# NVIDIA/flowtron

Measured on AMD Instinct MI355X. Metric: mel-frames/sec training (2-flow, 80-mel), higher is better.
Workload: dtype bf16; 1 GPU; BASELINE configs[1]: 2-flow LJS config.json model, per-GPU batch 32, T_max=862, L_max=157, attn-prior + CTC on, fwd+loss+bwd+clip+RAdam; global_batch=32, parallelism=dp1, mfma_operands=bf16, storage=fp32, skipped_steps=0

## Files before the change

flowtron_amd/_lib.py:

```python
from __future__ import annotations

import ctypes as C
import os

import torch

_HERE = os.path.dirname(os.path.abspath(__file__))
LIB_PATH = os.path.join(_HERE, "libflowtron_hip.so")

FT_F32, FT_BF16, FT_F16 = 0, 1, 2
GEMM_SPLITK = 1
GEMM_SPLITK_DET = 2
GEMM_C16 = 4
ACT_NONE, ACT_TANH, ACT_RELU, ACT_SIGMOID = 0, 1, 2, 3

_p, _i, _l, _f, _sz, _d = C.c_void_p, C.c_int, C.c_int64, C.c_float, C.c_size_t, C.c_double


class GemmArgs(C.Structure):
    _fields_ = [("A", _p), ("B", _p), ("C", _p), ("bias", _p),
                ("M", _i), ("N", _i), ("K", _i), ("batch", _i),
                ("sAm", _l), ("sAk", _l), ("sBk", _l), ("sBn", _l), ("ldc", _l),
                ("bsA", _l), ("bsB", _l), ("bsC", _l),
                ("alpha", _f), ("beta", _f), ("act", _i), ("mode", _i), ("flags", _i),
                ("work", _p), ("work_bytes", _sz)]


class GemmImgArgs(C.Structure):
    _fields_ = [("A", _p), ("B", _p), ("C", _p), ("bias", _p), ("M", _i), ("N", _i), ("K", _i),
                ("lda", _l), ("ldb", _l), ("ldc", _l), ("a_kmajor", _i), ("b_kmajor", _i),
                ("alpha", _f), ("beta", _f), ("act", _i), ("flags", _i),
                ("rowmap", _p), ("rows_dev", _p), ("compact", _i), ("k_shift", _i), ("r1_row", _p), ("r1_col", _p),
                ("split_work", _p), ("split_work_bytes", _sz), ("a_rows", _p)]


class LstmFwdRole(C.Structure):
    _fields_ = [("gx", _p), ("lens", _p), ("y", _p), ("ldy", _l), ("gates", _p), ("cell", _p), ("wimg", _p), ("state_h", _p), ("state_c", _p),
                ("B", C.c_int32), ("ldb", C.c_int32), ("t0", C.c_int32), ("t1", C.c_int32), ("gx16", C.c_int32)]


class LstmBwdRole(C.Structure):
    _fields_ = [("dy", _p), ("ldy", _l), ("lens", _p), ("gates", _p), ("cell", _p), ("dgx", _p), ("wimg", _p),
                ("dimg", _p), ("dimg_ld", _l), ("dimg_rows", _l), ("dbias", _p), ("state_da", _p), ("state_dc", _p),
                ("B", C.c_int32), ("ldb", C.c_int32), ("t0", C.c_int32), ("t1", C.c_int32), ("carry_in", C.c_int32)]


class ImgDesc(C.Structure):
    _fields_ = [("src", _p), ("ld", _l), ("rows", _l), ("cols", _l), ("dst", _p), ("kind", _i)]


class CummAttnArgs(C.Structure):
    _fields_ = [(n, _p) for n in ("text", "Q", "V", "w_key", "v", "w1", "b1", "w2", "b2", "in_lens", "ctx", "attn", "logprob",
                                  "cumm_all", "kproj_all", "work")] + [("work_bytes", _sz)] + [
        (n, _i) for n in ("T", "B", "L", "E", "A", "NF", "K1", "K2")] + [("temperature", _f), ("mode", _i), ("persist_status", _p)]


class DecodeArgs(C.Structure):
    _fields_ = [(n, _p) for n in (
        "att_w_ih", "att_w_hh", "att_b_ih", "att_b_hh", "w_query", "v", "K", "V",
        "l0_w_ih", "l0_w_hh", "l0_b_ih", "l0_b_hh", "l1_w_ih", "l1_w_hh", "l1_b_ih", "l1_b_hh",
        "d0_w", "d0_b", "d1_w", "d1_b", "conv_w", "conv_b", "gate_w", "gate_b",
        "residual", "mel_out", "attn_out", "n_done_dev", "work")] + [
        ("work_bytes", _sz), ("N", _i), ("L", _i), ("H", _i), ("A", _i), ("M", _i),
        ("temperature", _f), ("gate_threshold", _f), ("use_graph", _i)] + [
        (n, _p) for n in ("cond_w1", "cond_b1", "cond_w2", "cond_b2", "w_key", "enc")] + [("E", _i), ("prior", _p), ("forced", _p),
                                                                                         ("wimg", _p), ("wimg_bytes", _sz), ("persist_gran", _p), ("persist_status", _p),
                                                                                         ("n_layers", _i), ("extra_layers", _p)]


class DecodeBatchArgs(C.Structure):
    _fields_ = [("a", DecodeArgs), ("nb", _i), ("n_lim", _p), ("wimg_ready", _i)]


SUMSQ_PARTIALS = 1024
RESAMPLE_MAX_PHASES, RESAMPLE_MAX_TAPS = 2048, 20480

SIGNATURES = {
    "ft_abi_version": ([], _i),
    "ft_last_error": ([], C.c_char_p),
    "ft_debug_hold_cus": ([_i, _l, _p], _i),
    "ft_gemm": ([C.POINTER(GemmArgs), _p], _i),
    "ft_gemm_workspace_bytes": ([C.POINTER(GemmArgs)], _sz),
    "ft_bf16_image_bytes": ([_l, _l], _sz),
    "ft_bf16_image": ([_p, _l, _l, _l, _p, _p], _i),
    "ft_bf16_image_colsum": ([_p, _l, _l, _l, _p, _p, _p], _i),
    "ft_bf16_image_colsum_acc": ([_p, _l, _l, _l, _p, _p, _p], _i),
    "ft_gemm_img": ([C.POINTER(GemmImgArgs), _p], _i),
    "ft_gemm_img_split_work_bytes": ([_i, _i, _i], _sz),
    "ft_bf16_image_split3": ([_p, _l, _l, _l, _p, _i, _p], _i),
    "ft_bf16_image_split3_im2col": ([_p, _p, _i, _i, _i, _i, _p, _p], _i),
    "ft_bf16_image_split3_im2col_f16": ([_p, _p, _i, _i, _i, _i, _p, _p], _i),
    "ft_bf16_image_table": ([C.POINTER(ImgDesc), _i, _p], _i),
    "ft_bf16_image_table_f16": ([C.POINTER(ImgDesc), _i, _p], _i),
    "ft_bf16_image_split3_f16": ([_p, _l, _l, _l, _p, _i, _p], _i),
    "ft_rowmap_build": ([_p, _p, _p, _i, _i, _p], _i),
    "ft_chunk_gather_rows": ([_p, _p, _p, _i, _i, _i, _i, _p], _i),
    "ft_bf16_image_rows": ([_p, _l, _l, _l, _p, _p, _p, _p, _p], _i),
    "ft_bf16_image_rows_acc": ([_p, _l, _l, _l, _p, _p, _p, _p, _p], _i),
    "ft_bf16_image_rows_into": ([_p, _l, _l, _l, _p, _l, _l, _l, _p, _p, _p], _i),
    "ft_img_gemv_rows": ([_p, _l, _i, _p, _p, _p, _l, _p, _p, _p, _i, _i, _p], _i),
    "ft_img_gemv_rows_bwd": ([_p, _l, _i, _p, _l, _p, _p, _p, _p, _l, _p], _i),
    "ft_bf16_image_rows_act_bwd": ([_p, _l, _p, _l, _i, _l, _l, _p, _p, _p, _p, _p], _i),
    "ft_bf16_image_rows_act_bwd_acc": ([_p, _l, _p, _l, _i, _l, _l, _p, _p, _p, _p, _p], _i),
    "ft_pad_rows_fill": ([_p, _l, _i, _p, _i, _i, _i, _p], _i),
    "ft_embedding_fwd": ([_p, _p, _p, _i, _i, _l, _p], _i),
    "ft_embedding_bwd": ([_p, _p, _p, _i, _i, _l, _p], _i),
    "ft_embedding_bwd_runs": ([_p, _p, _p, _i, _i, _l, _i, _p], _i),
    "ft_im2col": ([_p, _p, _p, _i, _i, _i, _i, _p], _i),
    "ft_col2im": ([_p, _p, _p, _i, _i, _i, _i, _p], _i),
    "ft_instnorm_relu_fwd": ([_p] * 8 + [_i, _i, _i, _f, _p], _i),
    "ft_instnorm_relu_bwd": ([_p] * 11 + [_i, _i, _i, _p], _i),
    "ft_lstm_workspace_bytes": ([_i, _i], _sz),
    "ft_lstm_seq_fwd": ([_p, _p, _p, _p, _l, _p, _p, _p, _i, _i, _i, _i, _i, _p], _i),
    "ft_lstm_seq_bwd": ([_p, _l, _p, _p, _p, _p, _p, _p, _i, _i, _i, _i, _i, _p], _i),
    "ft_lstm_persist_supported": ([_i, _i], _i),
    "ft_lstm_persist_workspace_bytes": ([_i, _i], _sz),
    "ft_lstm_persist_debug_prof": ([_p], _i),
    "ft_lstm_persist_bwd": ([_p, _l, _p, _p, _p, _p, _p, _p, _p, _i, _i, _i, _i, _p], _i),
    "ft_bilstm_persist_supported": ([_i, _i], _i),
    "ft_bilstm_persist_workspace_bytes": ([_i, _i], C.c_size_t),
    "ft_bilstm_persist_fwd": ([_p, _p, _p, _p, _p, _p, _l, _p, _p, _p, _p, _p, _p, _i, _i, _i, _p], _i),
    "ft_bilstm_persist_bwd": ([_p, _l, _p, _p, _p, _p, _p, _p, _p, _p, _p, _p, _p, _i, _i, _i, _p], _i),
    "ft_lstm_persist_bwd_img": ([_p, _l, _p, _p, _p, _p, _p, _p, _p, _i, _i, _i, _i, _p, _l, _l, _p, _p], _i),
    "ft_lstm_roles_ctx_bytes": ([], _sz),
    "ft_lstm_roles_wimg_bytes": ([_i], _sz),
    "ft_lstm_roles_ctx_init": ([_p, _p], _i),
    "ft_lstm_roles_debug_prof": ([_p], _i),
    "ft_lstm_roles_prepare_fwd": ([_p, _p, _i, _p], _i),
    "ft_lstm_roles_prepare_bwd": ([_p, _p, _i, _p], _i),
    "ft_lstm_roles_fwd": ([C.POINTER(LstmFwdRole), _i, _i, _i, _p, _i, _p, _i, _p], _i),
    "ft_lstm_roles_bwd": ([C.POINTER(LstmBwdRole), _i, _i, _i, _p, _i, _p, _i, _p], _i),
    "ft_lstm2_supported": ([_i, _i], _i),
    "ft_lstm2_workspace_bytes": ([_i, _i], _sz),
    "ft_lstm2_seq_fwd": ([_p] * 13 + [_i, _i, _i, _p], _i),
    "ft_lstm2_seq_bwd": ([_p] * 12 + [_i, _i, _i, _p], _i),
    "ft_lstm_bidir_supported": ([_i, _i], _i),
    "ft_lstm_bidir_seq_fwd": ([_p] * 6 + [_l] + [_p] * 6 + [_i, _i, _i, _p], _i),
# ... 24 lines not shown
    "ft_decode_debug_prof": ([_p], _i),
    "ft_decode_flow": ([C.POINTER(DecodeArgs), _p], _i),
    "ft_decode_batch_max": ([], _i),
    "ft_decode_batch_gran_bytes": ([_i], _sz),
    "ft_decode_flow_batch": ([C.POINTER(DecodeBatchArgs), _p], _i),
    "ft_decode_flow_batch_keys": ([C.POINTER(DecodeBatchArgs), _p, _p], _i),
    "ft_stft_mel": ([_p, _p, _p, _p, _i, _i, _i, _i, _i, _p], _i),
    "ft_stft_r8": ([_p, _p, _p, _p, _p, _p, _p, _p, _i, _i, _i, _i, _p], _i),
    "ft_stft_r8_ragged": ([_p, _p, _p, _p, _p, _p, _p, _i, _i, _i, _i, _i, _p], _i),
    "ft_istft_r8": ([_p, _p, _p, _p, _i, _i, _i, _p], _i),
    "ft_stft_pow2": ([_p, _p, _p, _p, _p, _p, _p, _p, _i, _i, _i, _i, _i, _i, _p], _i),
    "ft_stft_pow2_ragged": ([_p, _p, _p, _p, _p, _p, _p, _i, _i, _i, _i, _i, _i, _i, _p], _i),
    "ft_istft_pow2": ([_p, _p, _p, _p, _i, _i, _i, _i, _i, _p], _i),
    "ft_stft_r8_ragged_phase": ([_p, _p, _p, _p, _p, _i, _i, _i, _p], _i),
    "ft_istft_r8_ragged": ([_p, _p, _p, _p, _p, _i, _i, _i, _p], _i),
    "ft_stft_pow2_ragged_phase": ([_p, _p, _p, _p, _p, _i, _i, _i, _i, _i, _p], _i),
    "ft_istft_pow2_ragged": ([_p, _p, _p, _p, _p, _i, _i, _i, _i, _i, _p], _i),
    "ft_resample_ragged": ([_p, _p, _p, _p, _p, _i, _i, _i, _i, _i, _i, _p], _i),
    "ft_resample_out_len": ([_l, _i, _i], _l),
    "ft_attn_ctc_workspace_floats":([_i, _i, _i], _sz),
    "ft_attn_ctc_fwd": ([_p, _p, _p, _f, _p, _p, _i, _i, _i, _i, _p], _i),
    "ft_attn_ctc_bwd": ([_p, _p, _p, _f, _p, _p, _p, _i, _i, _i, _i, _p], _i),
    "ft_attn_ctc_fwd_multi": ([_p, _p, _i, _p, _p, _f, _p, _p, _i, _i, _i, _i, _p], _i),
    "ft_attn_ctc_bwd_multi": ([_p, _p, _i, _p, _p, _f, _p, _p, _p, _i, _i, _i, _i, _p], _i),
    "ft_beta_binomial_prior": ([_p, _p, _p, _i, _i, _i, _f, _p], _i),
    "ft_sumsq": ([_p, _p, _l, _p, _p], _i),
    "ft_radam_step": ([_p, _p, _p, _p, _l, _p, _d, _d, _d, _d, _d, _d, _d, _i, _p, _p], _i),
    "ft_radam_step_dev": ([_p, _p, _p, _p, _l, _p, _d, _d, _d, _d, _d, _d, _i, _p, _p], _i),
    "ft_poison_if_nonzero": ([_p, _p, _p], _i),
}

OP16_TWINS = ("ft_gemm", "ft_bf16_image", "ft_bf16_image_colsum", "ft_bf16_image_colsum_acc", "ft_bf16_image_rows_acc", "ft_bf16_image_rows_act_bwd_acc", "ft_gemm_img", "ft_bf16_image_rows", "ft_bf16_image_rows_into", "ft_bf16_image_rows_act_bwd", "ft_img_gemv_rows", "ft_img_gemv_rows_bwd", "ft_lstm_seq_fwd", "ft_lstm_seq_bwd",
              "ft_lstm_persist_bwd", "ft_lstm_persist_bwd_img", "ft_lstm_roles_prepare_fwd", "ft_lstm_roles_prepare_bwd", "ft_lstm_roles_fwd", "ft_lstm_roles_bwd", "ft_lstm2_seq_fwd", "ft_lstm2_seq_bwd",
              "ft_lstm_bidir_seq_fwd", "ft_lstm_bidir_seq_bwd", "ft_bilstm_persist_fwd", "ft_bilstm_persist_bwd")
for _n in OP16_TWINS:
    SIGNATURES[_n + "_f16"] = SIGNATURES[_n]

_lib = None


def lib():
    global _lib
    if _lib is None:
        if not os.path.exists(LIB_PATH):
            raise RuntimeError(
                "libflowtron_hip.so is missing (%s). Build it with `python -m flowtron_amd.build` "
                "(hipcc --offload-arch=gfx950). There is no CPU/PyTorch fallback." % LIB_PATH)
        l = C.CDLL(LIB_PATH)
        for name, (argt, rest) in SIGNATURES.items():
            fn = getattr(l, name)
            fn.argtypes = argt
            fn.restype = rest
        if l.ft_abi_version() != 14:
            raise RuntimeError("libflowtron_hip.so ABI version mismatch")
        _lib = l
    return _lib


def check(rc: int, what: str):
    if rc != 0:
        raise RuntimeError("%s failed (%d): %s" % (what, rc, lib().ft_last_error().decode()))


def ptr(t):
    if t is None:
        return None
    return t.data_ptr()
# ... 41 lines not shown
```

flowtron_amd/csrc/bilstm_persist.hip:

```cpp
#include "common.h"
#include "lstm_images.h"

namespace {

typedef __attribute__((address_space(1))) unsigned long long gu64;
typedef __attribute__((ext_vector_type(4))) unsigned int u32x4;

constexpr int BH = 256;
constexpr int NWG = 256;
constexpr int GRAN_F = 4 * BH / 2;
constexpr int GRAN_B = 4 * 4 * BH / 2;

template <int N>
__device__ __forceinline__ unsigned row_shl(unsigned v) {
    if constexpr (N == 0) return v;
    else return (unsigned)__builtin_amdgcn_update_dpp(0, (int)v, 0x100 + N, 0xf, 0xf, true);
}
template <int N>
__device__ __forceinline__ float row_shl_f(float v) { return __uint_as_float(row_shl<N>(__float_as_uint(v))); }
template <int S>
__device__ __forceinline__ u32x4 shl4(u32x4 v) {
    return (u32x4){row_shl<S>(v[0]), row_shl<S>(v[1]), row_shl<S>(v[2]), row_shl<S>(v[3])};
}
__device__ __forceinline__ u32x4 member(u32x4 v, int j) {
// ... 284 lines not shown
    FT_CHECK_HIP(hipFuncSetAttribute(reinterpret_cast<const void*>(bilstm_persist_fwd_k), hipFuncAttributeMaxDynamicSharedMemorySize, (int)BI_LDS));
    hipLaunchKernelGGL(bilstm_persist_fwd_k, dim3(NWG), dim3(256), BI_LDS, st, p);
    FT_CHECK_LAUNCH();
    return FT_OK;
}

extern "C" int FT_OPNAME(ft_bilstm_persist_bwd)(const float* dy, int64_t ldy, const float* w_hh_f, const float* w_hh_r, const int32_t* lens,
                                             const float* gates_f, const float* gates_r, const float* cell_f, const float* cell_r,
                                             float* dgx_f, float* dgx_r, void* work, int32_t* status, int T, int B, int H,
                                             void* stream) {
    FT_CHECK_ARG(dy && w_hh_f && w_hh_r && lens && gates_f && gates_r && cell_f && cell_r && dgx_f && dgx_r && work && status);
    FT_CHECK_ARG(T >= 0 && ldy >= 2 * (int64_t)H && reinterpret_cast<uintptr_t>(work) % 256 == 0);
    if (!ft_bilstm_persist_supported(B, H))
        return ft_fail(FT_EUNSUPPORTED, "ft_bilstm_persist_bwd: needs H == 256, B <= 32 and a 256-CU device (H=%d B=%d)", H, B);
    if (T == 0) return FT_OK;
    hipStream_t st = reinterpret_cast<hipStream_t>(stream);
    char* base = reinterpret_cast<char*>(work);
    unsigned short* wf[2] = {reinterpret_cast<unsigned short*>(base), reinterpret_cast<unsigned short*>(base + al256b(BI_WFRAG))};
    unsigned long long* gran = reinterpret_cast<unsigned long long*>(base + 2 * al256b(BI_WFRAG));
    unsigned* census = reinterpret_cast<unsigned*>(base + 2 * al256b(BI_WFRAG) + al256b(BI_GRAN));
    FT_CHECK_HIP(hipMemsetAsync(dgx_f, 0, (size_t)T * B * 4 * H * 4, st));
    FT_CHECK_HIP(hipMemsetAsync(dgx_r, 0, (size_t)T * B * 4 * H * 4, st));
    static_assert(BI_GRAN % 16 == 0, "granule buffer in 16-byte pieces");
    const WfragAux aux{reinterpret_cast<uint4*>(gran), (unsigned long)(BI_GRAN / 16), 0u, census};
    hipLaunchKernelGGL(make_wfrag_bwd, dim3(256), dim3(256), 0, st, w_hh_f, wf[0], H, aux);
    hipLaunchKernelGGL(make_wfrag_bwd, dim3(256), dim3(256), 0, st, w_hh_r, wf[1], H, WfragAux{});
    BiBwdP p{dy, (long)ldy, lens, {gates_f, gates_r}, {cell_f, cell_r}, {dgx_f, dgx_r}, {wf[0], wf[1]}, gran, status, census, T, B,
             100000000L / 2};
    FT_CHECK_HIP(hipFuncSetAttribute(reinterpret_cast<const void*>(bilstm_persist_bwd_k), hipFuncAttributeMaxDynamicSharedMemorySize, (int)BI_LDS));
    hipLaunchKernelGGL(bilstm_persist_bwd_k, dim3(NWG), dim3(256), BI_LDS, st, p);
    FT_CHECK_LAUNCH();
    return FT_OK;
}
```

flowtron_amd/csrc/elementwise.hip:

```cpp
#include "common.h"

namespace {

constexpr int NT = 256;

__device__ __forceinline__ float block_sum(float v, float* red) {
    v = wave_sum(v);
    const int lane = threadIdx.x & 63, wave = threadIdx.x >> 6;
    __syncthreads();
    if (lane == 0) red[wave] = v;
    __syncthreads();
    float r = 0.f;
    const int nw = (blockDim.x + 63) >> 6;
    for (int i = 0; i < nw; ++i) r += red[i];
    return r;
}

inline int grid_for(int64_t n, int per_block = NT, int cap = 256 * 16) {
    int64_t g = (n + per_block - 1) / per_block;
    if (g < 1) g = 1;
    if (g > cap) g = cap;
    return (int)g;
}

// ... 60 lines not shown
    const long total = (long)L * B * C;
    const long CK = (long)C * KW;
    for (long i = blockIdx.x * (long)blockDim.x + threadIdx.x; i < total; i += (long)gridDim.x * blockDim.x) {
        const long row = i / C;
        const int c = (int)(i - row * C);
        const int l = (int)(row / B), b = (int)(row - (long)l * B);
        float v = 0.f;
        if (l < lens[b]) {
            for (int k = 0; k < KW; ++k) {
                const int lo = l - k + KW / 2;
                if (lo >= 0 && lo < L) v += dcol[((long)lo * B + b) * CK + (long)c * KW + k];
            }
        }
        dx[i] = v;
    }
}

__global__ void reverse_k(const float* __restrict__ x, float* __restrict__ y, const int* __restrict__ lens,
                          int T, int B, int C, int time_major) {
    const long total = (long)T * B * C;
    for (long i = blockIdx.x * (long)blockDim.x + threadIdx.x; i < total; i += (long)gridDim.x * blockDim.x) {
        const long row = i / C;
        const int c = (int)(i - row * C);
        int t, b;
        if (time_major) { t = (int)(row / B); b = (int)(row - (long)t * B); }
        else { b = (int)(row / T); t = (int)(row - (long)b * T); }
        const int len = lens[b];
        const int src = (t < len) ? (len - 1 - t) : (T - 1 + len - t);
        const long srow = time_major ? ((long)src * B + b) : ((long)b * T + src);
        y[i] = x[srow * C + c];
    }
}

__global__ void affine_fwd_k(const float* __restrict__ out, const float* __restrict__ x, float* __restrict__ z,
                             long n_rows, int M) {
    const long total = n_rows * M;
    for (long i = blockIdx.x * (long)blockDim.x + threadIdx.x; i < total; i += (long)gridDim.x * blockDim.x) {
        const long r = i / M;
        const int c = (int)(i - r * M);
        const float ls = out[r * 2 * M + c], bb = out[r * 2 * M + M + c];
        z[i] = expf(ls) * x[i] + bb;
    }
}
__global__ void affine_bwd_k(const float* __restrict__ out, const float* __restrict__ x, const float* __restrict__ dz,
                             const float* __restrict__ dls_ext, float* __restrict__ dout, float* __restrict__ dx,
                             long n_rows, int M) {
    const long total = n_rows * M;
    for (long i = blockIdx.x * (long)blockDim.x + threadIdx.x; i < total; i += (long)gridDim.x * blockDim.x) {
        const long r = i / M;
        const int c = (int)(i - r * M);
        const float s = expf(out[r * 2 * M + c]);
        const float g = dz[i];
        float dls = g * x[i] * s;
        if (dls_ext) dls += dls_ext[i];
        dout[r * 2 * M + c] = dls;
        dout[r * 2 * M + M + c] = g;
        if (dx) dx[i] = g * s;
    }
}
__global__ void affine_inv_k(const float* __restrict__ out, const float* __restrict__ z, float* __restrict__ x,
                             long n_rows, int M) {
    const long total = n_rows * M;
    for (long i = blockIdx.x * (long)blockDim.x + threadIdx.x; i < total; i += (long)gridDim.x * blockDim.x) {
        const long r = i / M;
        const int c = (int)(i - r * M);
        x[i] = (z[i] - out[r * 2 * M + M + c]) / expf(out[r * 2 * M + c]);
    }
}

__global__ void masked_sum_k(const float* __restrict__ x, long ld, const int* __restrict__ lens, float* __restrict__ acc,
                             int square, int T, int B, int M) {
    __shared__ float red[NT / 64];
    const long total = (long)T * B * M;
    float s = 0.f;
    for (long i = blockIdx.x * (long)blockDim.x + threadIdx.x; i < total; i += (long)gridDim.x * blockDim.x) {
        const long row = i / M;
        const int c = (int)(i - row * M);
        const int t = (int)(row / B), b = (int)(row - (long)t * B);
        if (t < lens[b]) {
            const float v = x[row * ld + c];
            s += square ? v * v : v;
        }
    }
    s = block_sum(s, red);
    if (threadIdx.x == 0) atomicAdd(acc, s);
}
__global__ void masked_sum_bwd_k(const float* __restrict__ x, long ld, const int* __restrict__ lens,
// ... 184 lines not shown
    float s = 0.f;
    for (int i = threadIdx.x; i < nb; i += blockDim.x) s += part[i];
    s = block_sum(s, red);
    if (threadIdx.x == 0) acc[0] += s;
}

__global__ void rowmap_k(const int* __restrict__ lens, int* __restrict__ rowmap, int* __restrict__ rows_dev, int T, int B) {
    const int b = blockIdx.x;
    int off = 0;
    for (int i = 0; i < b; ++i) { int l = lens[i]; l = l < 0 ? 0 : (l > T ? T : l); off += l + 1; }
    int len = lens[b];
    len = len < 0 ? 0 : (len > T ? T : len);
    for (int t = threadIdx.x; t < len; t += blockDim.x) rowmap[off + t] = t * B + b;
    if (threadIdx.x == 0) {
        rowmap[off + len] = len < T ? len * B + b : -1;
        if (b == B - 1) rows_dev[0] = off + len + 1;
    }
}

__global__ void chunk_rows_k(const int* __restrict__ lens, int* __restrict__ a_rows, int* __restrict__ rowmap, int T, int B, int t0, int t1) {
    const int b = blockIdx.x, w = t1 - t0;
    int off = 0, offc = 0, near = -1, off_b = 0, offc_b = 0, lk_b = 0;
    for (int i = 0; i < B; ++i) {
        int l = lens[i]; l = l < 0 ? 0 : (l > T ? T : l);
        int lk = l - t0; lk = lk < 0 ? 0 : (lk > w ? w : lk);
        if (i == b) { off_b = off; offc_b = offc; lk_b = lk; }
        if (lk > 0 && (i <= b || near < 0)) near = off + t0 + lk - 1;
        off += l + 1; offc += lk + 1;
    }
    for (int t = threadIdx.x; t < lk_b; t += blockDim.x) { a_rows[offc_b + t] = off_b + t0 + t; rowmap[offc_b + t] = t * B + b; }
    if (threadIdx.x == 0) { a_rows[offc_b + lk_b] = near < 0 ? 0 : near; rowmap[offc_b + lk_b] = -1; }
}

__global__ void pad_fill_k(float* __restrict__ y, long ld, int cols, const int* __restrict__ lens, int T, int B, int mode) {
    const int row = blockIdx.x, t = row / B, b = row % B;
    int len = lens[b];
    len = len < 0 ? 0 : len;
    if (t <= len) return;
    const float* src = y + (size_t)(len * B + b) * ld;
    float* dst = y + (size_t)row * ld;
    for (int c = blockIdx.y * blockDim.x + threadIdx.x; c < cols; c += gridDim.y * blockDim.x) dst[c] = mode ? src[c] : 0.f;
}

__global__ void poison_k(const int* __restrict__ status, float* __restrict__ dst) {
    if (status[0] != 0) dst[0] = __builtin_nanf("");
}

__global__ void radam_k(float* __restrict__ p, const float* __restrict__ g, float* __restrict__ m, float* __restrict__ v,
                        long n, const float* __restrict__ gnorm_sq, float clip, float wd_lr, float b1, float b2, float omb1,
                        float omb2, float eps, float step_size, int rectified, int* __restrict__ skipped) {
    float cs = 1.f;
    if (gnorm_sq) {
        const float sq = gnorm_sq[0];
        if (!(sq <= 3.0e38f)) {
            if (skipped && blockIdx.x == 0 && threadIdx.x == 0) atomicAdd(skipped, 1);
            return;
        }
        if (clip > 0.f) cs = fminf(1.f, clip / (sqrtf(sq) + 1e-6f));
    }
    for (long i = blockIdx.x * (long)blockDim.x + threadIdx.x; i < n; i += (long)gridDim.x * blockDim.x) {
        const float gi = g[i] * cs;
        const float vi = __fmaf_rn(omb2, __fmul_rn(gi, gi), __fmul_rn(b2, v[i]));
        const float mi = __fmaf_rn(omb1, gi, __fmul_rn(b1, m[i]));
        float pi = p[i];
        if (wd_lr != 0.f) pi = __fmaf_rn(-wd_lr, pi, pi);
        if (rectified) pi += -step_size * (mi / (sqrtf(vi) + eps));
        else pi += -step_size * mi;
        v[i] = vi; m[i] = mi; p[i] = pi;
    }
}

// ... 81 lines not shown
    hipLaunchKernelGGL(im2col_k, dim3(grid_for((int64_t)L * B * C * KW)), dim3(NT), 0, ST(stream), x, col, lens, L, B, C, KW);
    FT_CHECK_LAUNCH();
    return FT_OK;
}
extern "C" int ft_col2im(const float* dcol, float* dx, const int32_t* lens, int L, int B, int C, int KW, void* stream) {
    FT_CHECK_ARG(dcol && dx && lens && L >= 0 && B >= 1 && C >= 1 && KW >= 1 && (KW & 1));
    if (L == 0) return FT_OK;
    hipLaunchKernelGGL(col2im_k, dim3(grid_for((int64_t)L * B * C)), dim3(NT), 0, ST(stream), dcol, dx, lens, L, B, C, KW);
    FT_CHECK_LAUNCH();
    return FT_OK;
}
extern "C" int ft_reverse_by_length(const float* x, float* y, const int32_t* lens, int T, int B, int C, int time_major, void* stream) {
    FT_CHECK_ARG(x && y && lens && x != y && T >= 0 && B >= 1 && C >= 1);
    if (T == 0) return FT_OK;
    hipLaunchKernelGGL(reverse_k, dim3(grid_for((int64_t)T * B * C)), dim3(NT), 0, ST(stream), x, y, lens, T, B, C, time_major);
    FT_CHECK_LAUNCH();
    return FT_OK;
}
extern "C" int ft_affine_fwd(const float* out, const float* x, float* z, int64_t n_rows, int M, void* stream) {
    FT_CHECK_ARG(out && x && z && n_rows >= 0 && M >= 1);
    if (n_rows == 0) return FT_OK;
    hipLaunchKernelGGL(affine_fwd_k, dim3(grid_for(n_rows * M)), dim3(NT), 0, ST(stream), out, x, z, (long)n_rows, M);
    FT_CHECK_LAUNCH();
    return FT_OK;
}
extern "C" int ft_affine_bwd(const float* out, const float* x, const float* dz, const float* dlog_s_ext,
                             float* dout, float* dx, int64_t n_rows, int M, void* stream) {
    FT_CHECK_ARG(out && x && dz && dout && n_rows >= 0 && M >= 1);
    if (n_rows == 0) return FT_OK;
    hipLaunchKernelGGL(affine_bwd_k, dim3(grid_for(n_rows * M)), dim3(NT), 0, ST(stream), out, x, dz, dlog_s_ext, dout, dx, (long)n_rows, M);
    FT_CHECK_LAUNCH();
    return FT_OK;
}
extern "C" int ft_affine_inv(const float* out, const float* z, float* x, int64_t n_rows, int M, void* stream) {
    FT_CHECK_ARG(out && z && x && n_rows >= 0 && M >= 1);
    if (n_rows == 0) return FT_OK;
    hipLaunchKernelGGL(affine_inv_k, dim3(grid_for(n_rows * M)), dim3(NT), 0, ST(stream), out, z, x, (long)n_rows, M);
    FT_CHECK_LAUNCH();
    return FT_OK;
}
extern "C" int ft_masked_sum(const float* x, int64_t ld, const int32_t* lens, float* acc, int square,
                             int T, int B, int M, void* stream) {
    FT_CHECK_ARG(x && lens && acc && ld >= M && T >= 0 && B >= 1 && M >= 1);
    if (T == 0) return FT_OK;
    hipLaunchKernelGGL(masked_sum_k, dim3(grid_for((int64_t)T * B * M, NT, 1024)), dim3(NT), 0, ST(stream), x, (long)ld, lens, acc, square, T, B, M);
    FT_CHECK_LAUNCH();
    return FT_OK;
}
extern "C" int ft_masked_sum_bwd(const float* x, int64_t ld, const int32_t* lens, const float* scale_dev, float coef, int square,
                                 float* dx, int64_t ld_dx, int T, int B, int M, void* stream) {
    FT_CHECK_ARG(lens && scale_dev && dx && (x || !square) && ld_dx >= M && T >= 0 && B >= 1 && M >= 1);
    if (T == 0) return FT_OK;
    hipLaunchKernelGGL(masked_sum_bwd_k, dim3(grid_for((int64_t)T * B * M)), dim3(NT), 0, ST(stream), x, (long)ld, lens, scale_dev, coef, square, dx, (long)ld_dx, T, B, M);
    FT_CHECK_LAUNCH();
    return FT_OK;
}
extern "C" int ft_gate_bce_fwd(const float* gate, const float* target, const int32_t* lens, float* acc, int T, int B, void* stream) {
    FT_CHECK_ARG(gate && target && lens && acc && T >= 0 && B >= 1);
    if (T == 0) return FT_OK;
    hipLaunchKernelGGL(gate_bce_fwd_k, dim3(grid_for((int64_t)T * B, NT, 256)), dim3(NT), 0, ST(stream), gate, target, lens, acc, T, B);
    FT_CHECK_LAUNCH();
    return FT_OK;
}
extern "C" int ft_gate_bce_bwd(const float* gate, const float* target, const int32_t* lens, const float* scale_dev, float coef,
                               float* dgate, int T, int B, void* stream) {
    FT_CHECK_ARG(gate && target && lens && scale_dev && dgate && T >= 0 && B >= 1);
// ... 85 lines not shown
                             const float* gnorm_sq_dev, double clip, double lr, double beta1, double beta2, double eps,
                             double weight_decay, double step_size, int rectified, int32_t* skipped_dev, void* stream) {
    FT_CHECK_ARG(p && g && m && v && n >= 0);
    if (n == 0) return FT_OK;
    hipLaunchKernelGGL(radam_k, dim3(grid_for(n, NT, 4096)), dim3(NT), 0, ST(stream), p, g, m, v, (long)n, gnorm_sq_dev, (float)clip,
                       (float)(weight_decay * lr), (float)beta1, (float)beta2, (float)(1.0 - beta1), (float)(1.0 - beta2), (float)eps,
                       (float)step_size, rectified, skipped_dev);
    FT_CHECK_LAUNCH();
    return FT_OK;
}
extern "C" int ft_radam_step_dev(float* p, const float* g, float* m, float* v, int64_t n, const float* gnorm_sq_dev, double clip,
                                 double lr, double beta1, double beta2, double eps, double weight_decay, int calls,
                                 int32_t* skipped_dev, void* stream) {
    FT_CHECK_ARG(p && g && m && v && gnorm_sq_dev && skipped_dev && n >= 0 && calls >= 1);
    if (n == 0) return FT_OK;
    hipLaunchKernelGGL(radam_dev_k, dim3(grid_for(n, NT, 4096)), dim3(NT), 0, ST(stream), p, g, m, v, (long)n, gnorm_sq_dev, (float)clip,
                       (float)(weight_decay * lr), (float)beta1, (float)beta2, (float)(1.0 - beta1), (float)(1.0 - beta2), (float)eps,
                       lr, beta1, beta2, calls, skipped_dev);
    FT_CHECK_LAUNCH();
    return FT_OK;
}
extern "C" int ft_rowmap_build(const int32_t* lens, int32_t* rowmap, int32_t* rows_dev, int T, int B, void* stream) {
    FT_CHECK_ARG(lens && rowmap && rows_dev && T >= 1 && B >= 1 && (int64_t)T * B + B < (1ll << 31));
    hipLaunchKernelGGL(rowmap_k, dim3(B), dim3(256), 0, ST(stream), lens, rowmap, rows_dev, T, B);
    FT_CHECK_LAUNCH();
    return FT_OK;
}
extern "C" int ft_chunk_gather_rows(const int32_t* lens, int32_t* a_rows, int32_t* rowmap, int T, int B, int t0, int t1, void* stream) {
    FT_CHECK_ARG(lens && a_rows && rowmap && T >= 1 && B >= 1 && t0 >= 0 && t0 < t1 && t1 <= T && (int64_t)T * B + B < (1ll << 31));
    hipLaunchKernelGGL(chunk_rows_k, dim3(B), dim3(256), 0, ST(stream), lens, a_rows, rowmap, T, B, t0, t1);
    FT_CHECK_LAUNCH();
    return FT_OK;
}
extern "C" int ft_pad_rows_fill(float* y, int64_t ld, int cols, const int32_t* lens, int T, int B, int mode, void* stream) {
    FT_CHECK_ARG(y && lens && T >= 1 && B >= 1 && cols >= 1 && ld >= cols && (mode == 0 || mode == 1));
    hipLaunchKernelGGL(pad_fill_k, dim3(T * B, cols > 1024 ? 4 : 1), dim3(256), 0, ST(stream), y, (long)ld, cols, lens, T, B, mode);
    FT_CHECK_LAUNCH();
    return FT_OK;
}
extern "C" int ft_poison_if_nonzero(const int32_t* status_dev, float* dst, void* stream) {
    FT_CHECK_ARG(status_dev && dst);
    hipLaunchKernelGGL(poison_k, dim3(1), dim3(1), 0, ST(stream), status_dev, dst);
    FT_CHECK_LAUNCH();
    return FT_OK;
}
```

flowtron_amd/csrc/gemm_bf16.hip:

```cpp
#include "common.h"
#include <stdlib.h>

namespace {

constexpr int TB = 128;

inline size_t up(size_t v, size_t m) { return (v + m - 1) / m * m; }

__device__ __forceinline__ uint4 pack8(const float (&v)[8]) {
    uint4 o;
    o.x = pack_op16x2(v[0], v[1]); o.y = pack_op16x2(v[2], v[3]);
    o.z = pack_op16x2(v[4], v[5]); o.w = pack_op16x2(v[6], v[7]);
    return o;
}

__device__ __forceinline__ int mapped_rows(const int* rdev, int Rp, int& Rz) {
    const int R = *rdev;
    const int z = (R + 32 + 255) & ~255;
    Rz = z < Rp ? z : Rp;
    return R;
}

__device__ __forceinline__ void img_rows_body(const float* __restrict__ src, long sr, long sc, int R, int Cc,
                                              unsigned short* __restrict__ dst, int Rp, int Cp, int vec,
                                              const int* __restrict__ rowmap, const int* __restrict__ rdev, long dld,
                                              size_t first, size_t stride) {
    const int cq = Cp >> 3;
    int Rz = Rp;
    if (rdev) R = mapped_rows(rdev, Rp, Rz);
    const size_t total = (size_t)Rz * cq;
    for (size_t i = first; i < total; i += stride) {
        const int ri = (int)(i / cq), c = (int)(i % cq) * 8;
        int r = ri;
        if (rowmap) r = ri < R ? rowmap[ri] : -1;
        float v[8] = {0.f, 0.f, 0.f, 0.f, 0.f, 0.f, 0.f, 0.f};
        if (r >= 0 && (rowmap || r < R) && c < Cc) {
            const float* p = src + (size_t)r * sr + (size_t)c * sc;
            if (vec && c + 7 < Cc) {
                const float4 a = *reinterpret_cast<const float4*>(p), b = *reinterpret_cast<const float4*>(p + 4);
                v[0] = a.x; v[1] = a.y; v[2] = a.z; v[3] = a.w; v[4] = b.x; v[5] = b.y; v[6] = b.z; v[7] = b.w;
            } else {
#pragma unroll
                for (int e = 0; e < 8; ++e) if (c + e < Cc) v[e] = p[(size_t)e * sc];
            }
        }
        *reinterpret_cast<uint4*>(dst + (size_t)ri * dld + c) = pack8(v);
    }
}
__global__ __launch_bounds__(256) void img_rows_k(const float* __restrict__ src, long sr, long sc, int R, int Cc,
                                                  unsigned short* __restrict__ dst, int Rp, int Cp, int vec,
                                                  const int* __restrict__ rowmap, const int* __restrict__ rdev, long dld) {
    img_rows_body(src, sr, sc, R, Cc, dst, Rp, Cp, vec, rowmap, rdev, dld, blockIdx.x * (size_t)blockDim.x + threadIdx.x,
                  (size_t)gridDim.x * blockDim.x);
}

__device__ __forceinline__ void img_split3_body(const float* __restrict__ src, long sr, int R, int K, unsigned short* __restrict__ dst,
                                                int Rp, int Cp, int weight, size_t first, size_t stride) {
    const int kq = K >> 3, cq = Cp >> 3;
    const size_t total = (size_t)Rp * cq;
    for (size_t i = first; i < total; i += stride) {
        const int r = (int)(i / cq), q = (int)(i % cq);
        uint4 out = make_uint4(0u, 0u, 0u, 0u);
        if (r < R && q < 3 * kq) {
            const int blk = q / kq, c = (q - blk * kq) * 8;
            const float* p = src + (size_t)r * sr + c;
            float v[8], lo[8];
#pragma unroll
            for (int e = 0; e < 8; ++e) v[e] = p[e];
            const bool want_lo = weight ? blk == 2 : blk == 1;
            if (want_lo) {
#pragma unroll
                for (int e = 0; e < 8; ++e) lo[e] = v[e] - op16_to_f(f2op16(v[e]));
                out = pack8(lo);
            } else {
                out = pack8(v);
            }
        }
        *reinterpret_cast<uint4*>(dst + (size_t)r * Cp + (size_t)q * 8) = out;
    }
}
__global__ __launch_bounds__(256) void img_split3_k(const float* __restrict__ src, long sr, int R, int K, unsigned short* __restrict__ dst,
                                                    int Rp, int Cp, int weight) {
    img_split3_body(src, sr, R, K, dst, Rp, Cp, weight, blockIdx.x * (size_t)blockDim.x + threadIdx.x, (size_t)gridDim.x * blockDim.x);
}

__global__ __launch_bounds__(256) void img_split3_im2col_k(const float* __restrict__ x, const int* __restrict__ lens, int Lx, int B, int Cc, int KW,
                                                           unsigned short* __restrict__ dst, int Rp, int Cp) {
    const int R = Lx * B, K = Cc * KW;
    const int kq = K >> 3, cq = Cp >> 3;
    const size_t total = (size_t)Rp * cq;
    for (size_t i = blockIdx.x * (size_t)blockDim.x + threadIdx.x; i < total; i += (size_t)gridDim.x * blockDim.x) {
        const int r = (int)(i / cq), q = (int)(i % cq);
        uint4 out = make_uint4(0u, 0u, 0u, 0u);
        if (r < R && q < 3 * kq) {
            const int blk = q / kq, c0 = (q - blk * kq) * 8;
            const int l = r / B, b = r - l * B;
            const int len = lens[b];
            float v[8], lo[8];
#pragma unroll
            for (int e = 0; e < 8; ++e) {
                const int j = c0 + e, ch = j / KW, k = j - ch * KW;
                const int ls = l + k - KW / 2;
                v[e] = (ls >= 0 && ls < len) ? x[((size_t)ls * B + b) * Cc + ch] : 0.f;
            }
            if (blk == 1) {
#pragma unroll
                for (int e = 0; e < 8; ++e) lo[e] = v[e] - op16_to_f(f2op16(v[e]));
                out = pack8(lo);
            } else {
                out = pack8(v);
            }
        }
        *reinterpret_cast<uint4*>(dst + (size_t)r * Cp + (size_t)q * 8) = out;
    }
}

constexpr int IMG_TABLE_MAX = 32;
struct ImgTable {
    const float* src[IMG_TABLE_MAX];
    unsigned short* dst[IMG_TABLE_MAX];
    long sr[IMG_TABLE_MAX];
    int R[IMG_TABLE_MAX], Cc[IMG_TABLE_MAX], Rp[IMG_TABLE_MAX], Cp[IMG_TABLE_MAX], kind[IMG_TABLE_MAX], vec[IMG_TABLE_MAX];
    int blk0[IMG_TABLE_MAX + 1];
    int n;
};
__global__ __launch_bounds__(256) void img_table_k(ImgTable t) {
    int d = 0;
    while (d + 1 < t.n && (int)blockIdx.x >= t.blk0[d + 1]) ++d;
    const size_t first = (size_t)((int)blockIdx.x - t.blk0[d]) * blockDim.x + threadIdx.x;
    const size_t stride = (size_t)(t.blk0[d + 1] - t.blk0[d]) * blockDim.x;
    if (t.kind[d] == 0) img_rows_body(t.src[d], t.sr[d], 1, t.R[d], t.Cc[d], t.dst[d], t.Rp[d], t.Cp[d], t.vec[d], nullptr, nullptr, (long)t.Cp[d], first, stride);
    else img_split3_body(t.src[d], t.sr[d], t.R[d], t.Cc[d], t.dst[d], t.Rp[d], t.Cp[d], 1, first, stride);
}

constexpr int IMG_SUM_SLAB = 64;
__global__ __launch_bounds__(256) void img_rows_sum_k(const float* __restrict__ src, long sr, int R, int Cc,
                                                      unsigned short* __restrict__ dst, int Rp, int Cp, int vec,
                                                      float* __restrict__ colsum, const int* __restrict__ rowmap,
                                                      const int* __restrict__ rdev, const float* __restrict__ ysrc = nullptr,
                                                      long ysr = 0, int act = 0) {
    __shared__ float red[8][32][9];
    const int tx = threadIdx.x & 31, ty = threadIdx.x >> 5;
    const int c = (blockIdx.x * 32 + tx) * 8;
    const int r0 = blockIdx.y * IMG_SUM_SLAB;
    int Rz = Rp;
    if (rdev) R = mapped_rows(rdev, Rp, Rz);
    if (r0 >= Rz) return;
    float acc[8] = {0.f, 0.f, 0.f, 0.f, 0.f, 0.f, 0.f, 0.f};
    if (c < Cp) {
#pragma unroll 4
        for (int k = 0; k < IMG_SUM_SLAB / 8; ++k) {
            const int ri = r0 + ty + 8 * k;
            if (ri >= Rz) break;
            int r = ri;
            if (rowmap) r = ri < R ? rowmap[ri] : -1;
            float v[8] = {0.f, 0.f, 0.f, 0.f, 0.f, 0.f, 0.f, 0.f};
            if (r >= 0 && (rowmap || r < R) && c < Cc) {
                const float* p = src + (size_t)r * sr + c;
                if (vec && c + 7 < Cc) {
                    const float4 a = *reinterpret_cast<const float4*>(p), b = *reinterpret_cast<const float4*>(p + 4);
                    v[0] = a.x; v[1] = a.y; v[2] = a.z; v[3] = a.w; v[4] = b.x; v[5] = b.y; v[6] = b.z; v[7] = b.w;
                } else {
#pragma unroll
                    for (int e = 0; e < 8; ++e) if (c + e < Cc) v[e] = p[e];
// ... 3 lines not shown
                    float yv[8] = {0.f, 0.f, 0.f, 0.f, 0.f, 0.f, 0.f, 0.f};
                    if (vec && c + 7 < Cc) {
                        const float4 a = *reinterpret_cast<const float4*>(py), b = *reinterpret_cast<const float4*>(py + 4);
                        yv[0] = a.x; yv[1] = a.y; yv[2] = a.z; yv[3] = a.w; yv[4] = b.x; yv[5] = b.y; yv[6] = b.z; yv[7] = b.w;
                    } else {
#pragma unroll
                        for (int e = 0; e < 8; ++e) if (c + e < Cc) yv[e] = py[e];
                    }
#pragma unroll
                    for (int e = 0; e < 8; ++e) {
                        if (act == FT_ACT_TANH) v[e] = v[e] * (1.f - yv[e] * yv[e]);
                        else if (act == FT_ACT_RELU) v[e] = yv[e] > 0.f ? v[e] : 0.f;
                        else if (act == FT_ACT_SIGMOID) v[e] = v[e] * yv[e] * (1.f - yv[e]);
                    }
                }
            }
#pragma unroll
            for (int e = 0; e < 8; ++e) acc[e] += v[e];
            *reinterpret_cast<uint4*>(dst + (size_t)ri * Cp + c) = pack8(v);
        }
    }
#pragma unroll
    for (int e = 0; e < 8; ++e) red[ty][tx][e] = acc[e];
    __syncthreads();
    const int cx = threadIdx.x >> 3, e = threadIdx.x & 7;
    float s8 = 0.f;
#pragma unroll
    for (int y = 0; y < 8; ++y) s8 += red[y][cx][e];
    const int col = (blockIdx.x * 32 + cx) * 8 + e;
    if (col < Cc) atomicAdd(colsum + col, s8);
}

void make_image(const float* src, long sr, long sc, int R, int Cc, unsigned short* dst, int Rp, int Cp, hipStream_t st,
                const int* rowmap = nullptr, const int* rdev = nullptr, long dld = 0) {
    const bool vec = sc == 1 && reinterpret_cast<uintptr_t>(src) % 16 == 0 && sr % 4 == 0;
    const size_t chunks = (size_t)Rp * (Cp >> 3);
    const int blocks = (int)((chunks + 255) / 256 < 16384 ? (chunks + 255) / 256 : 16384);
    hipLaunchKernelGGL(img_rows_k, dim3(blocks), dim3(256), 0, st, src, sr, sc, R, Cc, dst, Rp, Cp, vec ? 1 : 0, rowmap, rdev,
                       dld ? dld : (long)Cp);
}

struct BfP {
    const unsigned short* A; const unsigned short* B; float* C; const float* bias;
    int M, N, nk;
    long lda, ldb, ldc;
    float alpha, beta;
    int act, gx, gy, splits, ksteps;
    int vec_c;
    const int* rowmap; const int* rows_dev; int compact, k_shift;
    int chunk_w;
    const float* r1row; const float* r1col;
    long c_slice;
    int c16;
    const int* a_rows;
};

typedef __attribute__((address_space(3))) void lds_void;
typedef const __attribute__((address_space(1))) void glb_void;
typedef __attribute__((ext_vector_type(4))) short bf16x4;

template <bool KM, int RT = 128>
struct Operand {
    static constexpr int NS = RT / 64;
    static constexpr int WT = RT / 32;
    const unsigned short* src[NS];
    size_t kstride;
    int dst[NS];
    int roff;
    __device__ __forceinline__ void init(const unsigned short* img, long ld, int r0, int wave, int lane, int wsel) {
        const int li = lane & 15, kg = lane >> 4;
        if constexpr (!KM) {
            const int srow = lane >> 2, skp = (lane & 3) ^ ((lane >> 4) & 2);
// ... 540 lines not shown
    unsigned short* Aimg = reinterpret_cast<unsigned short*>(a->work);
    unsigned short* Bimg = reinterpret_cast<unsigned short*>(reinterpret_cast<char*>(a->work) + ga.bytes);
    make_image(a->A, ga.sr, ga.sc, ga.rows, ga.cols, Aimg, ga.Rp, ga.Cp, st);
    make_image(a->B, gb.sr, gb.sc, gb.rows, gb.cols, Bimg, gb.Rp, gb.Cp, st);
    const int rc = run_images(Aimg, ga.Cp, ga.km, Bimg, gb.Cp, gb.km, a->C, a->ldc, a->bias, a->M, a->N, a->K, a->alpha, a->beta,
                              a->act, a->flags, st);
    return rc < 0 ? rc : 1;
}

#if FT_OPFMT == 0
extern "C" size_t ft_bf16_image_bytes(int64_t rows, int64_t cols) {
    if (rows < 1 || cols < 1) return 0;
    return up(up((size_t)rows + 32, 256) * up((size_t)cols, 256) * 2, 256);
}
#endif

extern "C" int FT_OPNAME(ft_bf16_image)(const float* src, int64_t ld, int64_t rows, int64_t cols, void* dst, void* stream) {
    FT_CHECK_ARG(src && dst && rows >= 1 && cols >= 1 && ld >= cols && rows < (1ll << 31) - 256 && cols < (1ll << 31) - 256);
    FT_CHECK_ARG(reinterpret_cast<uintptr_t>(dst) % 256 == 0);
    make_image(src, ld, 1, (int)rows, (int)cols, reinterpret_cast<unsigned short*>(dst), (int)up((size_t)rows + 32, 256),
               (int)up((size_t)cols, 256), reinterpret_cast<hipStream_t>(stream));
    FT_CHECK_LAUNCH();
    return FT_OK;
}

extern "C" int FT_OPNAME(ft_bf16_image_table)(const ft_img_desc* descs, int n, void* stream) {
    FT_CHECK_ARG(descs && n >= 1 && n <= IMG_TABLE_MAX);
    ImgTable t{};
    t.n = n;
    int blocks = 0;
    for (int i = 0; i < n; ++i) {
        const ft_img_desc& d = descs[i];
        FT_CHECK_ARG(d.src && d.dst && d.rows >= 1 && d.cols >= 1 && d.ld >= d.cols && d.rows < (1ll << 31) - 256 && 3 * d.cols < (1ll << 31) - 256);
        FT_CHECK_ARG(reinterpret_cast<uintptr_t>(d.dst) % 256 == 0 && (d.kind == 0 || (d.kind == 1 && d.cols % 8 == 0)));
        t.src[i] = d.src; t.dst[i] = reinterpret_cast<unsigned short*>(d.dst); t.sr[i] = (long)d.ld;
        t.R[i] = (int)d.rows; t.Cc[i] = (int)d.cols; t.kind[i] = d.kind;
        t.Rp[i] = (int)up((size_t)d.rows + 32, 256);
        t.Cp[i] = (int)up((size_t)(d.kind == 1 ? 3 * d.cols : d.cols), 256);
        t.vec[i] = (reinterpret_cast<uintptr_t>(d.src) % 16 == 0 && d.ld % 4 == 0) ? 1 : 0;
        const size_t chunks = (size_t)t.Rp[i] * (t.Cp[i] >> 3);
        const int nb = (int)((chunks + 255) / 256 < 2048 ? (chunks + 255) / 256 : 2048);
        t.blk0[i] = blocks;
        blocks += nb;
    }
    t.blk0[n] = blocks;
    hipLaunchKernelGGL(img_table_k, dim3(blocks), dim3(256), 0, reinterpret_cast<hipStream_t>(stream), t);
    FT_CHECK_LAUNCH();
    return FT_OK;
}

extern "C" int FT_OPNAME(ft_bf16_image_split3)(const float* src, int64_t ld, int64_t rows, int64_t cols, void* dst, int weight, void* stream) {
    FT_CHECK_ARG(src && dst && rows >= 1 && cols >= 8 && cols % 8 == 0 && ld >= cols && rows < (1ll << 31) - 256 && 3 * cols < (1ll << 31) - 256);
    FT_CHECK_ARG(reinterpret_cast<uintptr_t>(dst) % 256 == 0);
    const int Rp = (int)up((size_t)rows + 32, 256), Cp = (int)up((size_t)3 * cols, 256);
    const size_t chunks = (size_t)Rp * (Cp >> 3);
    const int blocks = (int)((chunks + 255) / 256 < 16384 ? (chunks + 255) / 256 : 16384);
    hipLaunchKernelGGL(img_split3_k, dim3(blocks), dim3(256), 0, reinterpret_cast<hipStream_t>(stream), src, (long)ld, (int)rows, (int)cols,
                       reinterpret_cast<unsigned short*>(dst), Rp, Cp, weight ? 1 : 0);
    FT_CHECK_LAUNCH();
    return FT_OK;
}

extern "C" int FT_OPNAME(ft_bf16_image_split3_im2col)(const float* x, const int32_t* lens, int L, int B, int C, int KW, void* dst, void* stream) {
    FT_CHECK_ARG(x && lens && dst && L >= 1 && B >= 1 && C >= 1 && KW >= 1 && (KW & 1) && ((int64_t)C * KW) % 8 == 0);
    FT_CHECK_ARG((int64_t)L * B < (1ll << 31) - 256 && 3ll * C * KW < (1ll << 31) - 256 && reinterpret_cast<uintptr_t>(dst) % 256 == 0);
    const int Rp = (int)up((size_t)L * B + 32, 256), Cp = (int)up((size_t)3 * C * KW, 256);
    const size_t chunks = (size_t)Rp * (Cp >> 3);
    const int blocks = (int)((chunks + 255) / 256 < 16384 ? (chunks + 255) / 256 : 16384);
    hipLaunchKernelGGL(img_split3_im2col_k, dim3(blocks), dim3(256), 0, reinterpret_cast<hipStream_t>(stream), x, lens, L, B, C, KW,
                       reinterpret_cast<unsigned short*>(dst), Rp, Cp);
    FT_CHECK_LAUNCH();
    return FT_OK;
}
// ... 66 lines not shown
    return image_rows_act_bwd_impl(dy, ld, y, ldy, act, cap_rows, cols, dst, colsum, rowmap, rows_dev, false, stream);
}

extern "C" int FT_OPNAME(ft_bf16_image_rows_into)(const float* src, int64_t ld, int64_t cap_rows, int64_t cols, void* dst, int64_t dst_ld,
                                                  int64_t col_off, int64_t fill_cols, const int32_t* rowmap, const int32_t* rows_dev,
                                                  void* stream) {
    FT_CHECK_ARG(src && dst && rowmap && rows_dev && cap_rows >= 1 && cols >= 1 && ld >= cols && cap_rows < (1ll << 31) - 512);
    FT_CHECK_ARG(col_off >= 0 && col_off % 8 == 0 && fill_cols >= cols && fill_cols % 8 == 0 && col_off + fill_cols <= dst_ld && dst_ld % 8 == 0);
    FT_CHECK_ARG(reinterpret_cast<uintptr_t>(dst) % 256 == 0);
    const int Rp = (int)up((size_t)cap_rows + 32, 256);
    make_image(src, ld, 1, (int)cap_rows, (int)cols, reinterpret_cast<unsigned short*>(dst) + col_off, Rp, (int)fill_cols,
               reinterpret_cast<hipStream_t>(stream), rowmap, rows_dev, (long)dst_ld);
    FT_CHECK_LAUNCH();
    return FT_OK;
}

static int image_rows_impl(const float* src, int64_t ld, int64_t cap_rows, int64_t cols, void* dst, float* colsum,
                           const int32_t* rowmap, const int32_t* rows_dev, bool clear, void* stream) {
    FT_CHECK_ARG(src && dst && rowmap && rows_dev && cap_rows >= 1 && cols >= 1 && ld >= cols && cap_rows < (1ll << 31) - 512 && cols < (1ll << 31) - 256);
    FT_CHECK_ARG(reinterpret_cast<uintptr_t>(dst) % 256 == 0);
    hipStream_t st = reinterpret_cast<hipStream_t>(stream);
    const int Rp = (int)up((size_t)cap_rows + 32, 256), Cp = (int)up((size_t)cols, 256);
    if (!colsum) {
        make_image(src, ld, 1, (int)cap_rows, (int)cols, reinterpret_cast<unsigned short*>(dst), Rp, Cp, st, rowmap, rows_dev);
    } else {
        const int vec = (reinterpret_cast<uintptr_t>(src) % 16 == 0 && ld % 4 == 0) ? 1 : 0;
        if (clear) FT_CHECK_HIP(hipMemsetAsync(colsum, 0, sizeof(float) * (size_t)cols, st));
        hipLaunchKernelGGL(img_rows_sum_k, dim3(cdiv(Cp, 256), cdiv(Rp, IMG_SUM_SLAB)), dim3(256), 0, st, src, (long)ld, (int)cap_rows, (int)cols,
                           reinterpret_cast<unsigned short*>(dst), Rp, Cp, vec, colsum, rowmap, rows_dev);
    }
    FT_CHECK_LAUNCH();
    return FT_OK;
}
extern "C" int FT_OPNAME(ft_bf16_image_rows)(const float* src, int64_t ld, int64_t cap_rows, int64_t cols, void* dst, float* colsum,
                                             const int32_t* rowmap, const int32_t* rows_dev, void* stream) {
    return image_rows_impl(src, ld, cap_rows, cols, dst, colsum, rowmap, rows_dev, true, stream);
}
extern "C" int FT_OPNAME(ft_bf16_image_rows_acc)(const float* src, int64_t ld, int64_t cap_rows, int64_t cols, void* dst, float* colsum,
                                                 const int32_t* rowmap, const int32_t* rows_dev, void* stream) {
    return image_rows_impl(src, ld, cap_rows, cols, dst, colsum, rowmap, rows_dev, false, stream);
}

extern "C" int FT_OPNAME(ft_img_gemv_rows)(const void* img, int64_t ld, int K, const float* w, const float* bias, float* y, int64_t ldy,
                                           const int32_t* rowmap, const int32_t* rows_dev, const int32_t* lens, int T, int B, void* stream) {
    FT_CHECK_ARG(img && w && y && rowmap && rows_dev && lens && K >= 1 && ld >= ((K + 7) & ~7) && ld % 8 == 0 && ldy >= 1 && T >= 1 && B >= 1);
    FT_CHECK_ARG(reinterpret_cast<uintptr_t>(img) % 16 == 0 && K <= 16384);
    const int blocks = cdiv(T * B + B, 4) < 2048 ? cdiv(T * B + B, 4) : 2048;
    hipLaunchKernelGGL(img_gemv_rows_k, dim3(blocks), dim3(256), sizeof(float) * ((K + 7) & ~7), reinterpret_cast<hipStream_t>(stream),
                       reinterpret_cast<const unsigned short*>(img), (long)ld, K, w, bias, y, (long)ldy, rowmap, rows_dev, lens, T, B);
    FT_CHECK_LAUNCH();
    return FT_OK;
}

extern "C" int FT_OPNAME(ft_img_gemv_rows_bwd)(const void* img, int64_t ld, int K, const float* dy, int64_t lddy, float* dw, float* db,
                                               const int32_t* rowmap, const int32_t* rows_dev, int64_t cap_rows, void* stream) {
    FT_CHECK_ARG(img && dy && dw && rowmap && rows_dev && K >= 1 && ld >= ((K + 7) & ~7) && ld % 8 == 0 && lddy >= 1 && cap_rows >= 1);
    FT_CHECK_ARG(reinterpret_cast<uintptr_t>(img) % 16 == 0 && cap_rows < (1ll << 31) - 512);
    hipLaunchKernelGGL((img_gemv_rows_bwd_k<256>), dim3(cdiv((int)cap_rows, 256)), dim3(256), 0, reinterpret_cast<hipStream_t>(stream),
                       reinterpret_cast<const unsigned short*>(img), (long)ld, K, dy, (long)lddy, dw, db, rowmap, rows_dev);
    FT_CHECK_LAUNCH();
    return FT_OK;
}
```

flowtron_amd/model.py:

```python
from __future__ import annotations

import ctypes as C
import numbers
import os
from typing import List, Optional

import torch
from torch import nn

from . import _lib as L
from . import ops



class LinearNorm(nn.Module):
    def __init__(self, in_dim, out_dim, bias=True, w_init_gain="linear"):
        super().__init__()
        self.linear_layer = nn.Linear(in_dim, out_dim, bias=bias)
        nn.init.xavier_uniform_(self.linear_layer.weight, gain=nn.init.calculate_gain(w_init_gain))

    def forward(self, x, act=L.ACT_NONE, rowmap=None, fill="y+dx"):
        return ops.linear(x, self.linear_layer.weight, self.linear_layer.bias, act, rowmap=rowmap, fill=fill)


# ... 120 lines not shown


class AR_Step(nn.Module):
    def __init__(self, n_mel_channels, n_speaker_dim, n_text_channels, n_in_channels, n_hidden, n_attn_channels,
                 n_lstm_layers, add_gate, use_cumm_attention):
        super().__init__()
        if n_lstm_layers < 1:
            raise ValueError("n_lstm_layers must be >= 1")
        self.n_lstm_layers = int(n_lstm_layers)
        self.use_cumm_attention = use_cumm_attention
        self.conv = nn.Conv1d(n_hidden, 2 * n_mel_channels, 1)
        self.conv.weight.data = 0.0 * self.conv.weight.data
        self.conv.bias.data = 0.0 * self.conv.bias.data
        self.lstm = nn.LSTM(n_hidden + n_attn_channels, n_hidden, n_lstm_layers)
        self.attention_lstm = nn.LSTM(n_mel_channels, n_hidden)
        self.attention_layer = Attention(n_hidden, n_speaker_dim, n_text_channels, n_attn_channels)
        if self.use_cumm_attention:
            self.attn_cond_layer = AttentionConditioningLayer(input_dim=2, attention_n_filters=32,
                                                              attention_kernel_sizes=[5, 3],
                                                              attention_dim=n_text_channels + n_speaker_dim)
        self.dense_layer = DenseLayer(in_dim=n_hidden, sizes=[n_hidden, n_hidden])
        if add_gate:
            self.gate_threshold = 0.5
            self.gate_layer = LinearNorm(n_hidden + n_attn_channels, 1, bias=True, w_init_gain="sigmoid")
        self._decode_work = None

    def __getstate__(self):
        d = self.__dict__.copy()
        for k in ("_decode_bufs", "_decode_wimg", "_decode_gran", "_decode_batch_bufs", "_decode_batch_gran"):
            d.pop(k, None)
        d["_decode_work"] = None
        return d

    def forward(self, mel, text, in_lens32, out_lens32, attn_prior=None, rowmap=None):
        T, B, M = mel.shape
        mode = L.mfma_mode()
        rm = rowmap
        mel0 = torch.cat([mel.new_zeros(1, B, M), mel[:-1]], 0)
        a = self.attention_lstm
        h_att = ops.lstm_layer(mel0, out_lens32, a.weight_ih_l0, a.weight_hh_l0, a.bias_ih_l0, a.bias_hh_l0, mode=mode, rowmap=rm,
                               fill="dx")
        if self.use_cumm_attention:
            ctx, attn, logprob = self.run_cumm_attn_sequence(h_att, text, in_lens32)
        else:
            ctx, attn, logprob = self.attention_layer(h_att, text, text, in_lens32, attn_prior, rowmap=rm)
        gates = None
        p = self.lstm
        g = self.gate_layer.linear_layer if hasattr(self, "gate_layer") else None
        persist = (ops.lstm_persist_groups(B, p.weight_hh_l0.shape[1], False, mode, mel.device)
                   or bool(ops.lstm_persist_slices(B, p.weight_hh_l0.shape[1], False, mode, mel.device))
                   or ops.lstm_pad_width(B, p.weight_hh_l0.shape[1], False, mode, mel.device, T))
        fuse_gate = g is not None and (self.n_lstm_layers != 2 or persist or not ops.lstm2_supported(B, p.weight_hh_l0.shape[1], mode))
        if g is not None and not fuse_gate:
            gates = ops.linear([h_att, ctx], g.weight, g.bias, mode=mode)

        def first_layer():
            r = ops.lstm_layer(h_att, out_lens32, p.weight_ih_l0, p.weight_hh_l0, p.bias_ih_l0, p.bias_hh_l0, mode=mode,
                               xs_extra=[ctx], rowmap=rm, fill="dx", gate=(g.weight, g.bias) if fuse_gate else None)
            return r if fuse_gate else (r, gates)
        if self.n_lstm_layers != 2:
            h, gates = first_layer()
            for l in range(1, self.n_lstm_layers):
                h = ops.lstm_layer(h, out_lens32, getattr(p, "weight_ih_l%d" % l), getattr(p, "weight_hh_l%d" % l),
                                   getattr(p, "bias_ih_l%d" % l), getattr(p, "bias_hh_l%d" % l), mode=mode, rowmap=rm)
        elif persist and rm is not None and ops.decoder_pair_chunks(B, p.weight_hh_l0.shape[1], mode, mel.device, T):
            h, gates_f = ops.decoder_pair(h_att, out_lens32, p, mode, [ctx], rm, "dx", (g.weight, g.bias) if fuse_gate else None,
                                          ops.decoder_pair_chunks(B, p.weight_hh_l0.shape[1], mode, mel.device, T))
            if fuse_gate:
                gates = gates_f
        elif persist:
            h, gates = first_layer()
            h = ops.lstm_layer(h, out_lens32, p.weight_ih_l1, p.weight_hh_l1, p.bias_ih_l1, p.bias_hh_l1, mode=mode, rowmap=rm)
        elif ops.lstm2_supported(B, p.weight_hh_l0.shape[1], mode):
            gx0 = ops.LinearFn.apply(p.weight_ih_l0, p.bias_ih_l0 + p.bias_hh_l0, L.ACT_NONE, mode, None, "", h_att, ctx)
            h = ops.LSTM2SeqFn.apply(gx0, p.weight_hh_l0, p.weight_ih_l1, p.bias_ih_l1, p.bias_hh_l1, p.weight_hh_l1, out_lens32, mode)
        else:
            h, gates = first_layer()
            h = ops.lstm_layer(h, out_lens32, p.weight_ih_l1, p.weight_hh_l1, p.bias_ih_l1, p.bias_hh_l1, mode=mode, rowmap=rm)
        h = self.dense_layer(h, rowmap=rm)
        out = ops.linear(h, self.conv.weight.reshape(self.conv.weight.shape[0], -1), self.conv.bias, mode=mode, rowmap=rm, fill="y")
        z = ops.AffineFn.apply(out, mel)
        log_s = out[..., :M]
        return z, log_s, gates, attn, logprob

    def run_cumm_attn_sequence(self, h_att, text, in_lens32):
        mode = L.mfma_mode()
        att = self.attention_layer
        V = ops.linear(text, att.value.linear_layer.weight, None, mode=mode)
        Q = ops.linear(h_att, att.query.linear_layer.weight, None, mode=mode)
        if os.environ.get("FLOWTRON_CUMM_LOOP", "fused") != "python":
            c = self.attn_cond_layer
            return ops.CummAttnSeqFn.apply(Q, V, text, att.key.linear_layer.weight, att.v.linear_layer.weight,
                                           c.location_conv_hidden.conv.weight, c.location_conv_hidden.conv.bias,
                                           c.location_conv_out.conv.weight, c.location_conv_out.conv.bias,
                                           in_lens32, float(att.temperature), mode)
        T, B, _ = h_att.shape
        Lk = text.shape[0]
        full = torch.full((B,), Lk, dtype=torch.int32, device=text.device)
        cumm = text.new_zeros(Lk, B)
        prev = text.new_zeros(Lk, B)
        ctxs, attns, lps = [], [], []
        for i in range(T):
            cond = self.attn_cond_layer(torch.stack([cumm, prev], 2), full)
            K = ops.linear(ops.MulFn.apply(text, cond), att.key.linear_layer.weight, None, mode=mode)
            a, lp = ops.AttentionScoresFn.apply(Q[i:i + 1], K, att.v.linear_layer.weight, in_lens32, None, att.temperature)
            ctxs.append(ops.ContextFn.apply(a, V, mode))
            attns.append(a)
            lps.append(lp)
            prev = a[:, 0, :].t()
            cumm = ops.AddFn.apply(cumm, prev)
        return torch.cat(ctxs, 0), torch.cat(attns, 1), torch.cat(lps, 1)

    def infer(self, residual, text, attns=None, attn_prior=None, use_graph=None):
        N, B, M = residual.shape
        if B != 1:
# ... 186 lines not shown
                L.check(L.lib().ft_decode_flow_batch_keys(C.byref(bargs), L.ptr(keys_all[g0:g0 + nb]), L.stream()),
                        "ft_decode_flow_batch_keys")
            else:
                L.check(L.lib().ft_decode_flow_batch(C.byref(bargs), L.stream()), "ft_decode_flow_batch")
            out[:Ng, g0:g0 + nb] = mel_out.transpose(0, 1)
            attn[:Ng, g0:g0 + nb, 0] = attn_out.transpose(0, 1)
            n_done_all[g0:g0 + nb] = n_done
        n = list(lens)
        if batched:
            ok = ops.check_persist_status(raise_on_failure=False)
            if has_gate and ok:
                n = n_done_all.tolist()
            if not ok:
                singles = sorted(singles + [b for g in batched for b in g])
        for b in singles:
            m_, rows = self.infer(x[:lens[b], b:b + 1].contiguous(), text[:il[b], b:b + 1].contiguous())
            n[b] = m_.shape[0]
            out[:, b] = 0.0
            attn[:, b] = 0.0
            out[:n[b], b] = m_[:, 0]
            if rows:
                attn[:n[b], b, :, :il[b]] = torch.cat(rows, 0)
        return out, attn, n


class AR_Back_Step(nn.Module):
    def __init__(self, n_mel_channels, n_speaker_dim, n_text_dim, n_in_channels, n_hidden, n_attn_channels,
                 n_lstm_layers, add_gate, use_cumm_attention):
        super().__init__()
        self.ar_step = AR_Step(n_mel_channels, n_speaker_dim, n_text_dim, n_mel_channels + n_speaker_dim, n_hidden,
                               n_attn_channels, n_lstm_layers, add_gate, use_cumm_attention)
        self.ar_step._time_reversed = True

    def forward(self, mel, text, in_lens32, out_lens32, attn_prior=None, rowmap=None):
        mel = ops.reverse_by_length(mel, out_lens32, True)
        if attn_prior is not None:
            attn_prior = ops.reverse_by_length(attn_prior, out_lens32, False)
        z, log_s, gates, attn, logprob = self.ar_step(mel, text, in_lens32, out_lens32, attn_prior, rowmap=rowmap)
        z = ops.reverse_by_length(z, out_lens32, True)
        return z, log_s, gates, attn, logprob

    def infer(self, residual, text, attns=None, attn_prior=None):
        if attn_prior is not None:
            attn_prior = torch.flip(attn_prior, (1,))
        out, attn = self.ar_step.infer(torch.flip(residual, (0,)), text, attns, attn_prior=attn_prior)
        return torch.flip(out, (0,)), attn


def lengths_arg(v, name, B, hi):
    if v is None:
        return None
    if torch.is_tensor(v):
        if v.dtype.is_floating_point or v.dtype.is_complex or v.dtype == torch.bool:
            raise ValueError("%s must hold integers, got a %s tensor" % (name, v.dtype))
        if v.dim() != 1:
            raise ValueError("%s must be one-dimensional [B], got shape %s" % (name, tuple(v.shape)))
        vals = v.tolist()
    else:
        if not isinstance(v, (list, tuple)):
            raise ValueError("%s must be a list, tuple or tensor of integers, got %s" % (name, type(v).__name__))
        if any(isinstance(x, bool) or not isinstance(x, numbers.Integral) for x in v):
            raise ValueError("%s must hold integers, got %r" % (name, list(v)))
        vals = [int(x) for x in v]
    if len(vals) != B:
        raise ValueError("%s has %d entries for a batch of %d" % (name, len(vals), B))
    if any(not 1 <= x <= hi for x in vals):
        raise ValueError("%s must lie in 1 ..= %d, got %r" % (name, hi, vals))
    return vals


class Flowtron(nn.Module):
    def __init__(self, n_speakers, n_speaker_dim, n_text, n_text_dim, n_flows, n_mel_channels, n_hidden,
# ... 31 lines not shown
        return torch.cat([enc, spk], 2), lens

    def forward(self, mel, speaker_ids, text, in_lens, out_lens, attn_prior=None):
        L.require_cuda(mel, text, in_lens, out_lens, attn_prior)
        ops.weight_images_begin(self)
        ops.bias_sums_begin(self._lstm_bias_pairs())
        try:
            return self._forward(mel, speaker_ids, text, in_lens, out_lens, attn_prior)
        finally:
            ops.bias_sums_end()
            ops.weight_images_end(self)

    def _lstm_bias_pairs(self):
        groups = {}
        for mname, m in self.named_modules():
            if isinstance(m, torch.nn.LSTM):
                key = ".".join(mname.split(".")[:2]) if mname.startswith("flows.") else mname.split(".")[0]
                for name, p in m.named_parameters(recurse=False):
                    if name.startswith("bias_ih"):
                        groups.setdefault(key, []).append((p, getattr(m, "bias_hh" + name[len("bias_ih"):])))
        return list(groups.values())

    def _forward(self, mel, speaker_ids, text, in_lens, out_lens, attn_prior=None):
        enc, in32 = self._encode(speaker_ids, text, in_lens)
        out32 = ops.lens32(out_lens)
        x = mel.permute(2, 0, 1).contiguous().float()
        if attn_prior is not None:
            attn_prior = attn_prior.float()
        rm = ops.row_map(out32, x.shape[0], x.shape[1]) if L.is16(L.mfma_mode()) else None

        def run_flows(x, enc):
            log_s_list, attns_list, attns_logprob_list = [], [], []
            gate = None
            for flow in self.flows:
                x, log_s, gate, attn, logprob = flow(x, enc, in32, out32, attn_prior, rowmap=rm)
                log_s_list.append(log_s)
                attns_list.append(attn)
                attns_logprob_list.append(logprob)
            return x, log_s_list, gate, attns_list, attns_logprob_list

        x0 = x
        x, log_s_list, gate, attns_list, attns_logprob_list = run_flows(x0, enc)
        if not torch.is_grad_enabled() and ops.PERSIST_LAUNCHES:
            if not ops.check_persist_status(raise_on_failure=False):
                enc, in32 = self._encode(speaker_ids, text, in_lens)
                x, log_s_list, gate, attns_list, attns_logprob_list = run_flows(x0, enc)
        return x, log_s_list, gate, attns_list, attns_logprob_list, None, None, None

    def infer(self, residual, speaker_ids, text, temperature=1.0, gate_threshold=0.5, attns=None, attn_prior=None,
              in_lens=None, out_lens=None, return_lengths=False):
        L.require_cuda(residual, text)
        B = residual.shape[0]
        if residual.dim() != 3 or text.dim() != 2 or text.shape[0] != B:
            raise ValueError("residual must be [B, M, N] and text [B, L] with the same B, got %s and %s"
                             % (tuple(residual.shape), tuple(text.shape)))
        Lt, N = text.shape[1], residual.shape[2]
        il = lengths_arg(in_lens, "in_lens", B, Lt) or [Lt] * B
        ol = lengths_arg(out_lens, "out_lens", B, N) or [N] * B
        if B > 1 and attns is not None:
            raise ValueError("forced alignments (attns=) are taken one utterance at a time")
        if B == 1:
            if attns is not None and (il[0] < Lt or ol[0] < N):
                attns = [(torch.stack([r.reshape(-1) for r in a]) if isinstance(a, (list, tuple)) else a.reshape(-1, Lt))[:ol[0], :il[0]]
                         for a in attns]
            mel, aws = self._infer_one(residual[:, :, :ol[0]], speaker_ids, text[:, :il[0]], temperature, gate_threshold, attns,
                                       None if attn_prior is None else attn_prior[:, :ol[0], :il[0]])
            if il[0] < Lt:
                aws = [[torch.nn.functional.pad(r, (0, Lt - il[0])) for r in rows] for rows in aws]
# ... 135 lines not shown
```

flowtron_amd/ops.py:

```python
from __future__ import annotations

import ctypes as C
from typing import List, Optional, Sequence

import torch

from . import _lib as L



def _c(t: torch.Tensor) -> torch.Tensor:
    return t if t.is_contiguous() else t.contiguous()


import os as _os
_BF16_IMAGES = True


def gemm_raw(A, B, Cm, M, N, K, sAm, sAk, sBk, sBn, ldc, bias=None, act=L.ACT_NONE, alpha=1.0, beta=0.0,
             batch=1, bsA=0, bsB=0, bsC=0, mode=None, splitk=False):
    L.require_cuda(A, B, Cm, bias)
    a = L.GemmArgs(L.ptr(A), L.ptr(B), L.ptr(Cm), L.ptr(bias), M, N, K, batch,
                   sAm, sAk, sBk, sBn, ldc, bsA, bsB, bsC, alpha, beta, act,
                   L.mfma_mode() if mode is None else mode, L.GEMM_SPLITK if splitk else 0,
                   None, 0)
    if _BF16_IMAGES:
        need = L.lib().ft_gemm_workspace_bytes(C.byref(a))
        if need:
            work = torch.empty(need, device=Cm.device, dtype=torch.uint8)
            a.work, a.work_bytes = L.ptr(work), need
    L.check(L.lib().ft_gemm(C.byref(a), L.stream()), "ft_gemm")


class RowMap:
    __slots__ = ("T", "B", "cap", "lens", "map", "rows", "gather")

    def __init__(self, lens32, T, B):
        L.require_cuda(lens32)
        self.T, self.B, self.cap, self.lens = int(T), int(B), int(T) * int(B) + int(B), lens32
        self.map = torch.empty(self.cap, device=lens32.device, dtype=torch.int32)
        self.rows = torch.empty(1, device=lens32.device, dtype=torch.int32)
        L.check(L.lib().ft_rowmap_build(L.ptr(lens32), L.ptr(self.map), L.ptr(self.rows), self.T, self.B, L.stream()), "ft_rowmap_build")

    def fill(self, y2d, ncols, copy_separator):
        L.check(L.lib().ft_pad_rows_fill(L.ptr(y2d), int(y2d.stride(0)), int(ncols), L.ptr(self.lens), self.T, self.B,
                                         1 if copy_separator else 0, L.stream()), "ft_pad_rows_fill")


_COMPACT = _os.environ.get("FLOWTRON_GEMM_COMPACT", "1") != "0"
_FUSE_ACT_BWD = True
_ENC_SPLITK = "det"
_CAT_IMAGES = True
_PERSIST_IMG = _os.environ.get("FLOWTRON_LSTM_PERSIST_IMG", "1")


def row_map(lens32, T, B):
    return RowMap(lens32, T, B) if (_COMPACT and _BF16_IMAGES) else None


class Bf16Image:
    __slots__ = ("buf", "rows", "cols", "ld", "colsum", "fmt", "rowmap")

    def __init__(self, t2d, colsum=False, mode=None, rowmap=None):
        assert t2d.dim() == 2 and t2d.stride(1) == 1 and t2d.dtype == torch.float32
        L.require_cuda(t2d)
        self.rows, self.cols = int(t2d.shape[0]), int(t2d.shape[1])
        self.fmt = L.mfma_mode() if mode is None else mode
        self.ld = (self.cols + 255) // 256 * 256
        self.rowmap = rowmap
        self.colsum = zeroed((self.cols,), t2d.device) if colsum else None
        if rowmap is not None:
            assert self.rows == rowmap.T * rowmap.B, "row map built for another [T, B]"
            self.rows = rowmap.cap
            self.buf = torch.empty(L.lib().ft_bf16_image_bytes(self.rows, self.cols), device=t2d.device, dtype=torch.uint8)
            L.check(L.op16("ft_bf16_image_rows_acc", self.fmt)(L.ptr(t2d), int(t2d.stride(0)), self.rows, self.cols, L.ptr(self.buf), L.ptr(self.colsum),
                                                                L.ptr(rowmap.map), L.ptr(rowmap.rows), L.stream()), "ft_bf16_image_rows_acc")
            return
        self.buf = torch.empty(L.lib().ft_bf16_image_bytes(self.rows, self.cols), device=t2d.device, dtype=torch.uint8)
        if colsum:
            L.check(L.op16("ft_bf16_image_colsum_acc", self.fmt)(L.ptr(t2d), int(t2d.stride(0)), self.rows, self.cols, L.ptr(self.buf), L.ptr(self.colsum),
                                                     L.stream()), "ft_bf16_image_colsum_acc")
        else:
            L.check(L.op16("ft_bf16_image", self.fmt)(L.ptr(t2d), int(t2d.stride(0)), self.rows, self.cols, L.ptr(self.buf), L.stream()), "ft_bf16_image")

    def ptr(self, row_off=0, col_off=0):
        assert col_off % 8 == 0
        return self.buf.data_ptr() + 2 * (row_off * self.ld + col_off)

    def view_cols(self, cols):
        v = Bf16Image.__new__(Bf16Image)
        v.buf, v.rows, v.cols, v.ld, v.colsum, v.fmt, v.rowmap = self.buf, self.rows, int(cols), self.ld, None, self.fmt, self.rowmap
        return v

    @classmethod
    def split3(cls, t2d, mode, weight):
        assert t2d.dim() == 2 and t2d.stride(1) == 1 and t2d.dtype == torch.float32 and t2d.shape[1] % 8 == 0
        self = cls.__new__(cls)
        self.rows, self.cols, self.fmt, self.rowmap, self.colsum = int(t2d.shape[0]), 3 * int(t2d.shape[1]), mode, None, None
        self.ld = (self.cols + 255) // 256 * 256
        self.buf = torch.empty(L.lib().ft_bf16_image_bytes(self.rows, self.cols), device=t2d.device, dtype=torch.uint8)
        L.check(L.op16("ft_bf16_image_split3", mode)(L.ptr(t2d), int(t2d.stride(0)), self.rows, int(t2d.shape[1]), L.ptr(self.buf),
                                                     1 if weight else 0, L.stream()), "ft_bf16_image_split3")
        return self

    @classmethod
    def split3_im2col(cls, x, lens, KW, mode):
        Lx, B, Cc = x.shape
        self = cls.__new__(cls)
        self.rows, self.cols, self.fmt, self.rowmap, self.colsum = int(Lx * B), 3 * int(Cc * KW), mode, None, None
        self.ld = (self.cols + 255) // 256 * 256
        self.buf = torch.empty(L.lib().ft_bf16_image_bytes(self.rows, self.cols), device=x.device, dtype=torch.uint8)
        L.check(L.op16("ft_bf16_image_split3_im2col", mode)(L.ptr(x), L.ptr(lens), int(Lx), int(B), int(Cc), int(KW), L.ptr(self.buf), L.stream()),
                "ft_bf16_image_split3_im2col")
        return self

    @classmethod
    def _blank(cls, rows, cols, mode, device):
        self = cls.__new__(cls)
        self.rows, self.cols, self.fmt, self.rowmap, self.colsum = int(rows), int(cols), mode, None, None
        self.ld = (self.cols + 255) // 256 * 256
        self.buf = torch.empty(L.lib().ft_bf16_image_bytes(self.rows, self.cols), device=device, dtype=torch.uint8)
        return self

    @classmethod
    def of_weight(cls, W, mode, split=False):
        w = _WIMG
        key = (W.data_ptr(), tuple(W.shape), mode, bool(split))
        if w["plan_next"] is not None:
            w["plan_next"][key] = W
        if w["armed"]:
            w["armed"] = False
            plan = [(k, t) for k, t in w["plan"].items() if t.is_cuda and t.device == W.device and t.dtype == torch.float32 and t.is_contiguous()
                    and t.data_ptr() == k[0] and tuple(t.shape) == k[1]]
            for lo in range(0, len(plan), 32):
                part = plan[lo:lo + 32]
                by_fmt = {}
                for k, t in part:
                    by_fmt.setdefault(k[2], []).append((k, t))
                for fmt, items in by_fmt.items():
                    descs = (L.ImgDesc * len(items))()
                    for i, (k, t) in enumerate(items):
                        img = cls._blank(t.shape[0], (3 if k[3] else 1) * t.shape[1], fmt, t.device)
                        descs[i] = L.ImgDesc(t.data_ptr(), int(t.stride(0)), int(t.shape[0]), int(t.shape[1]), img.buf.data_ptr(), 1 if k[3] else 0)
                        w["cache"][k] = img
                    L.check(L.op16("ft_bf16_image_table", fmt)(descs, len(items), L.stream()), "ft_bf16_image_table")
        img = w["cache"].get(key)
        if img is not None:
            return img
        return cls.split3(W, mode, True) if split else cls(W, mode=mode)

    @classmethod
    def cat_rows(cls, xs2d, mode, rowmap):
        self = cls.__new__(cls)
        self.rows, self.cols, self.fmt, self.rowmap, self.colsum = rowmap.cap, int(sum(x.shape[1] for x in xs2d)), mode, rowmap, None
        self.ld = (self.cols + 255) // 256 * 256
        self.buf = torch.empty(L.lib().ft_bf16_image_bytes(self.rows, self.cols), device=xs2d[0].device, dtype=torch.uint8)
        off = 0
        for i, x in enumerate(xs2d):
            assert x.dim() == 2 and x.stride(1) == 1 and x.dtype == torch.float32 and x.shape[0] == rowmap.T * rowmap.B
            K = int(x.shape[1])
            last = i == len(xs2d) - 1
            assert last or K % 8 == 0
            L.check(L.op16("ft_bf16_image_rows_into", mode)(L.ptr(x), int(x.stride(0)), self.rows, K, L.ptr(self.buf), self.ld, off,
                                                            (self.ld - off) if last else K, L.ptr(rowmap.map), L.ptr(rowmap.rows), L.stream()),
                    "ft_bf16_image_rows_into")
            off += K
        return self

    @classmethod
    def empty_rows(cls, cols, rowmap, mode, device):
        self = cls.__new__(cls)
        self.rows, self.cols, self.fmt, self.rowmap = rowmap.cap, int(cols), mode, rowmap
        self.ld = (self.cols + 255) // 256 * 256
        self.buf = torch.empty(L.lib().ft_bf16_image_bytes(self.rows, self.cols), device=device, dtype=torch.uint8)
        self.colsum = zeroed((self.cols,), device)
        return self


_WIMG_ON = True
_WIMG = {"plan": {}, "plan_next": None, "cache": {}, "armed": False, "plans": None}


def weight_images_begin(model):
    if not _WIMG_ON:
        return
    w = _WIMG
    if w["plans"] is None:
        w["plans"] = _weakref.WeakKeyDictionary()
    w["plan"] = w["plans"].get(model, {})
    w["plan_next"], w["cache"], w["armed"] = {}, {}, bool(w["plan"])


def weight_images_end(model):
    w = _WIMG
    if w["plan_next"] is not None and w["plans"] is not None:
        w["plans"][model] = w["plan_next"]
    w["plan"], w["plan_next"], w["cache"], w["armed"] = {}, None, {}, False


import weakref as _weakref
_IMG_CACHE = {}


def shared_image(t, rows, cols, mode, rowmap=None):
    key = id(t)
    hit = _IMG_CACHE.get(key)
    want_rows = rows if rowmap is None else rowmap.cap
    if hit is not None:
        ref, ver, img = hit
        if ref() is t and ver == t._version and img.rows == want_rows and img.cols == cols and img.fmt == mode and img.rowmap is rowmap:
            return img
    img = Bf16Image(t.reshape(rows, cols), mode=mode, rowmap=rowmap)
    if len(_IMG_CACHE) > 64:
# ... 187 lines not shown


def colsum(x2d: torch.Tensor, rows: int, N: int, ld: int) -> torch.Tensor:
    out = torch.empty(N, device=x2d.device, dtype=torch.float32)
    L.check(L.lib().ft_colsum(L.ptr(x2d), L.ptr(out), rows, N, ld, L.stream()), "ft_colsum")
    return out


_LENS_CACHE = {}


def _lens_entry(lens: torch.Tensor):
    key = (lens.data_ptr(), lens._version, lens.numel(), lens.dtype, lens.device)
    e = _LENS_CACHE.get(key)
    if e is None or e[0]() is not lens:
        import weakref
        if len(_LENS_CACHE) > 64:
            _LENS_CACHE.clear()
        i32 = lens if (lens.dtype == torch.int32 and lens.is_contiguous()) else lens.to(dtype=torch.int32).contiguous()
        e = _LENS_CACHE[key] = (weakref.ref(lens), i32, {})
    return e


def lens32(lens: torch.Tensor) -> torch.Tensor:
    return _lens_entry(lens)[1]


def lens_total(lens: torch.Tensor, scale: float = 1.0) -> torch.Tensor:
    e = _lens_entry(lens)
    t = e[2].get(scale)
    if t is None:
        t = e[2][scale] = e[1].sum().to(torch.float32) * scale if scale != 1.0 else e[1].sum().to(torch.float32)
    return t


def linear_uses_images(mode, rows, N, xs):
    return all(images_apply(mode, rows, N, x.shape[-1]) for x in xs) and all((x.shape[-1] % 8 == 0) for x in xs[:-1])


class LinearFn(torch.autograd.Function):

    @staticmethod
    def forward(ctx, W, bias, act, mode, rowmap, fill, *xs):
        xs = [_c(x) for x in xs]
        L.require_cuda(W, *xs)
        W = _c(W)
        N, Ktot = W.shape
        rows = xs[0].numel() // xs[0].shape[-1]
        c16 = "c16" in fill
        y = torch.empty(xs[0].shape[:-1] + (N,), device=W.device, dtype=op16_dtype(mode) if c16 else torch.float32)
        mode_dx = mode_dw = mode
        if isinstance(mode, tuple):
            mode, mode_dx, mode_dw = mode
        split_fwd = mode == "split3"
        if split_fwd:
            assert len(xs) == 1 and act == L.ACT_NONE and L.is16(mode_dx) and mode_dx == mode_dw
            x2d = xs[0].reshape(rows, Ktot)
            split_imgs = lazy = None
            if Ktot % 32 == 0 and images_apply(mode_dx, rows, N, Ktot):
                lazy = _LAZY_COLS.pop(xs[0].data_ptr(), None)
                xi = Bf16Image.split3_im2col(*lazy, mode_dx) if lazy is not None else Bf16Image.split3(x2d, mode_dx, False)
                wi = Bf16Image.of_weight(W, mode_dx, split=True)
                gemm_img(xi, 0, xi.ptr(), wi, 0, wi.ptr(), y, rows, N, 3 * Ktot, N, bias=bias, splitk=_ENC_SPLITK)
                split_imgs = (wi.view_cols(Ktot), [xi.view_cols(Ktot)])
            else:
                _materialize_col(xs[0])
                gemm_raw(x2d, W, y, rows, N, Ktot, Ktot, 1, 1, Ktot, N, bias=bias, mode=L.FT_F32)
            mode = L.FT_F32
        mixed = not (mode == mode_dx == mode_dw)
        ctx.mode_dx, ctx.mode_dw = mode_dx, mode_dw
        use_img = (not mixed) and linear_uses_images(mode, rows, N, xs)
        ctx.lazy_img_mode = mode_dx if (mixed and mode_dx == mode_dw and linear_uses_images(mode_dx, rows, N, xs)) else None
        if rowmap is not None and (not use_img or rows != rowmap.T * rowmap.B):
            rowmap = None
        ctx.imgs = split_imgs if split_fwd else None
        ctx.cat = False
        ctx.img_kind = ("split3" if split_imgs is not None else None) if split_fwd else ("images" if use_img else None)
        ctx.lazy_src = lazy if split_fwd else None
        if use_img:
            w_img = Bf16Image.of_weight(W, mode)
            if len(xs) > 1 and rowmap is not None and _CAT_IMAGES:
                x_cat = Bf16Image.cat_rows([x.reshape(rows, x.shape[-1]) for x in xs], mode, rowmap)
                ctx.imgs, ctx.cat = (w_img, [x_cat]), True
                gemm_img(x_cat, 0, x_cat.ptr(), w_img, 0, w_img.ptr(), y, rowmap.cap, N, Ktot, N, bias=bias, act=act, rowmap=rowmap, compact=1, c16=c16)
            else:
                x_imgs = [shared_image(x, rows, x.shape[-1], mode, rowmap) for x in xs]
                ctx.imgs = (w_img, x_imgs)
        off = 0
        for i, x in enumerate(xs):
            if ctx.cat or split_fwd:
                off = Ktot
                break
            K = x.shape[-1]
            last = i == len(xs) - 1
            if use_img:
                assert not c16 or len(xs) == 1
                gemm_img(x_imgs[i], 0, x_imgs[i].ptr(), w_img, 0, w_img.ptr(0, off), y, rows if rowmap is None else rowmap.cap, N, K, N,
                         bias=bias if last else None, act=act if last else L.ACT_NONE, beta=0.0 if i == 0 else 1.0,
                         rowmap=rowmap, compact=1, c16=c16)
            else:
                assert not c16, "16-bit output rows come from the image GEMMs only"
                gemm_raw(x, W[:, off:], y, rows, N, K, K, 1, 1, Ktot, N,
                         bias=bias if last else None, act=act if last else L.ACT_NONE,
                         beta=0.0 if i == 0 else 1.0, mode=mode)
            off += K
        assert off == Ktot
        if rowmap is not None and "y" in fill:
            rowmap.fill(y.reshape(rows, N), N, copy_separator=True)
        ctx.save_for_backward(W, y if act != L.ACT_NONE else None, *xs)
        ctx.act, ctx.mode, ctx.has_bias, ctx.rowmap, ctx.fill = act, mode, bias is not None, rowmap, fill
        return y

    @staticmethod
    def backward(ctx, dy):
        W, y, *xs = ctx.saved_tensors
        N, Ktot = W.shape
        rows = dy.numel() // N
        rowmap = ctx.rowmap
        if ctx.imgs is None and ctx.img_kind is not None:
# ... 9 lines not shown
            _require_written(dy)
            dy = _c(dy.float())
        fuse_act = ctx.act != L.ACT_NONE and ctx.imgs is not None and rowmap is not None and _FUSE_ACT_BWD
        if ctx.act != L.ACT_NONE and not fuse_act:
            dpre = torch.empty_like(dy)
            L.check(L.lib().ft_act_bwd(L.ptr(y), L.ptr(dy), L.ptr(dpre), dy.numel(), ctx.act, L.stream()), "ft_act_bwd")
        else:
            dpre = dy
        dW = None
        if ctx.needs_input_grad[0]:
            dW = weight_grad_out(W) if ctx.imgs is not None else torch.empty_like(W)
        want_db = ctx.has_bias and ctx.needs_input_grad[1]
        db = None
        dxs = []
        off = 0
        imgs = ctx.imgs
        if imgs is not None:
            w_img, x_imgs = imgs
            d_img = d_img_in
            if d_img is None and fuse_act:
                d_img = Bf16Image.empty_rows(N, rowmap, w_img.fmt, dy.device)
                L.check(L.op16("ft_bf16_image_rows_act_bwd_acc", w_img.fmt)(L.ptr(dy), N, L.ptr(y), N, ctx.act, d_img.rows, N, L.ptr(d_img.buf),
                                                                             L.ptr(d_img.colsum), L.ptr(rowmap.map), L.ptr(rowmap.rows), L.stream()),
                        "ft_bf16_image_rows_act_bwd_acc")
            elif d_img is None:
                d_img = Bf16Image(dpre.reshape(rows, N), colsum=want_db, mode=w_img.fmt, rowmap=rowmap)
            db = d_img.colsum if want_db else None
        if want_db and db is None:
            db = colsum(dpre, rows, N, N)
        mrows = rows if rowmap is None else rowmap.cap
        for i, x in enumerate(xs):
            K = x.shape[-1]
            if ctx.needs_input_grad[6 + i]:
                if imgs is not None:
                    dx, acc = _dx_buffer(x)
                    gemm_img(d_img, 0, d_img.ptr(), w_img, 1, w_img.ptr(0, off), dx, mrows, K, N, K, beta=1.0 if acc else 0.0,
                             rowmap=rowmap, compact=1)
                    if rowmap is not None and "dx" in ctx.fill:
                        rowmap.fill(dx.reshape(rows, K), K, copy_separator=False)
                    if acc:
                        dx = None
                else:
                    dx = torch.empty_like(x)
                    gemm_raw(dpre, W[:, off:], dx, rows, K, N, N, 1, Ktot, 1, K, mode=ctx.mode_dx)
                dxs.append(dx)
            else:
                dxs.append(None)
            if dW is not None and ctx.cat:
                if i == 0:
                    gemm_img(d_img, 1, d_img.ptr(), x_imgs[0], 1, x_imgs[0].ptr(), dW, N, Ktot, mrows, Ktot, beta=1.0, splitk=True, rowmap=rowmap, compact=2)
            elif dW is not None:
                if imgs is not None:
                    gemm_img(d_img, 1, d_img.ptr(), x_imgs[i], 1, x_imgs[i].ptr(), dW[:, off:], N, K, mrows, Ktot, beta=1.0, splitk=True,
                             rowmap=rowmap, compact=2)
                    if rowmap is not None:
                        _handoff_put_x(x, x_imgs[i])
                else:
                    gemm_raw(dpre, x, dW[:, off:], N, K, rows, 1, N, K, 1, Ktot, mode=ctx.mode_dw, splitk=True)
            off += K
        ctx.imgs = None
        return (dW, db, None, None, None, None, *dxs)


def _linear_images_again(ctx, W, xs, rows):
    Ktot = W.shape[1]
    if ctx.img_kind == "split3":
        m = ctx.mode_dx
        xi = Bf16Image.split3_im2col(*ctx.lazy_src, m) if ctx.lazy_src is not None else Bf16Image.split3(xs[0].reshape(rows, Ktot), m, False)
        return Bf16Image.of_weight(W, m, split=True).view_cols(Ktot), [xi.view_cols(Ktot)]
    w_img = Bf16Image.of_weight(W, ctx.mode)
    if ctx.cat:
        return w_img, [Bf16Image.cat_rows([x.reshape(rows, x.shape[-1]) for x in xs], ctx.mode, ctx.rowmap)]
    return w_img, [shared_image(x, rows, x.shape[-1], ctx.mode, ctx.rowmap) for x in xs]


_GATE_ON_CAT = True


def linear_gate_fusable(mode, rowmap, xs, N):
    if not (_GATE_ON_CAT and _CAT_IMAGES and rowmap is not None and len(xs) == 2):
        return False
    rows = xs[0].numel() // xs[0].shape[-1]
    return rows == rowmap.T * rowmap.B and linear_uses_images(mode, rows, N, xs)


class LinearGateFn(torch.autograd.Function):

    @staticmethod
    def forward(ctx, W, bias, Wg, bg, mode, rowmap, fill, x0, x1):
        xs = [_c(x0), _c(x1)]
        L.require_cuda(W, Wg, *xs)
        W, Wg = _c(W), _c(Wg)
        N, Ktot = W.shape
        assert Wg.shape == (1, Ktot) and xs[0].shape[-1] + xs[1].shape[-1] == Ktot
        rows = rowmap.T * rowmap.B
        c16 = "c16" in fill
        y = torch.empty(xs[0].shape[:-1] + (N,), device=W.device, dtype=op16_dtype(mode) if c16 else torch.float32)
        gate = torch.empty(xs[0].shape[:-1] + (1,), device=W.device, dtype=torch.float32)
        w_img = Bf16Image.of_weight(W, mode)
        x_cat = Bf16Image.cat_rows([x.reshape(rows, x.shape[-1]) for x in xs], mode, rowmap)
        gemm_img(x_cat, 0, x_cat.ptr(), w_img, 0, w_img.ptr(), y, rowmap.cap, N, Ktot, N, bias=bias, rowmap=rowmap, compact=1, c16=c16)
        L.check(L.op16("ft_img_gemv_rows", mode)(L.ptr(x_cat.buf), x_cat.ld, Ktot, L.ptr(Wg), L.ptr(bg), L.ptr(gate), 1, L.ptr(rowmap.map),
                                                 L.ptr(rowmap.rows), L.ptr(rowmap.lens), rowmap.T, rowmap.B, L.stream()), "ft_img_gemv_rows")
        if "y" in fill:
            rowmap.fill(y.reshape(rows, N), N, copy_separator=True)
# ... 299 lines not shown
def persist_usable(device):
    if not L.lib().ft_lstm_persist_supported(8, 1024):
        return False
    st = _persist_state(torch.device(device))
    if st.usable is None:
        st.usable = _persist_selftest(torch.device(device), int(_os.environ.get("FLOWTRON_LSTM_PERSIST", "1")) or 1)
    return bool(st.usable)


def lstm_persist_groups(B, H, reverse, mode, device=None):
    ng = int(_os.environ.get("FLOWTRON_LSTM_PERSIST", "1"))
    if ng not in (0, 1):
        raise ValueError("FLOWTRON_LSTM_PERSIST must be 0 or 1 (the transport variants were removed in round 6)")
    if not ng or reverse or not L.is16(mode) or not L.lib().ft_lstm_persist_supported(B, H):
        return 0
    if device is not None:
        st = _persist_state(device)
        if st.usable is None:
            st.usable = _persist_selftest(device, ng)
        if not st.usable:
            return 0
    return 1


def lstm_persist_slices(B, H, reverse, mode, device=None):
    if B <= 32:
        return False
    return bool(lstm_persist_groups(32, H, reverse, mode, device))


_BIAS_SUMS = {}


class _BiasSumsFn(torch.autograd.Function):
    @staticmethod
    def forward(ctx, *flat):
        n = len(flat) // 2
        return tuple(torch._foreach_add(list(flat[:n]), list(flat[n:])))

    @staticmethod
    def backward(ctx, *gs):
        return tuple(gs) + tuple(gs)


def bias_sums_begin(groups):
    _BIAS_SUMS.clear()
    for pairs in groups:
        pairs = [(a, b) for a, b in pairs if a.is_cuda and b.is_cuda and a.shape == b.shape]
        if len(pairs) < 2:
            continue
        group = {"pairs": pairs, "outs": None}
        for a, b in pairs:
            _BIAS_SUMS[(id(a), id(b))] = group


def bias_sums_end():
    _BIAS_SUMS.clear()


def bias_sum(a, b):
    g = _BIAS_SUMS.get((id(a), id(b)))
    if g is None:
        return a + b
    if g["outs"] is None:
        g["outs"] = _BiasSumsFn.apply(*[x for x, _ in g["pairs"]], *[y for _, y in g["pairs"]])
    for (x, y), o in zip(g["pairs"], g["outs"]):
        if x is a and y is b:
            return o
    return a + b

# ... 18 lines not shown
def bilstm_persist_ok(B, H, mode, device):
    if int(_os.environ.get("FLOWTRON_LSTM_PERSIST", "1")) != 1:
        return False
    if not L.is16(mode) or not L.lib().ft_bilstm_persist_supported(B, H):
        return False
    st = _persist_state(device)
    if st.usable is None:
        st.usable = _persist_selftest(device, int(_os.environ.get("FLOWTRON_LSTM_PERSIST", "1")))
    return bool(st.usable)


class RolesCtx:

    def __init__(self, device):
        self.buf = torch.empty(L.lib().ft_lstm_roles_ctx_bytes(), device=device, dtype=torch.uint8)
        L.check(L.lib().ft_lstm_roles_ctx_init(L.ptr(self.buf), L.stream()), "ft_lstm_roles_ctx_init")
        self.phase = [0, 0]
        self.reset_rows = 8


_ROLES_CTX = {}


def roles_ctx(device):
    device = torch.device(device)
    if device.index is None:
        device = torch.device("cuda", torch.cuda.current_device())
    c = _ROLES_CTX.get(device)
    if c is None:
        c = _ROLES_CTX[device] = RolesCtx(device)
    return c


def roles_wimg(w_hh, mode, backward):
    img = torch.empty(L.lib().ft_lstm_roles_wimg_bytes(w_hh.shape[1]), device=w_hh.device, dtype=torch.uint8)
    fn = L.op16("ft_lstm_roles_prepare_bwd" if backward else "ft_lstm_roles_prepare_fwd", mode)
    w = _c(w_hh)
    L.check(fn(L.ptr(w), L.ptr(img), w.shape[1], L.stream()), "ft_lstm_roles_prepare")
    return img


def fwd_role(gx, lens, y, gates, cell, wimg, t0=0, t1=None, state=None, b0=0, nb=None):
    T, LB, H = gx.shape[0], gx.shape[1], y.shape[2]
    nb = LB - b0 if nb is None else nb
    return L.LstmFwdRole(gx.data_ptr() + gx.element_size() * 4 * H * b0, lens.data_ptr() + 4 * b0, y.data_ptr() + 4 * y.stride(1) * b0, y.stride(1),
                         gates.data_ptr() + 16 * H * b0 if gates is not None else None, cell.data_ptr() + 4 * H * b0 if cell is not None else None,
                         L.ptr(wimg), L.ptr(state[0]) if state is not None else None, L.ptr(state[1]) if state is not None else None,
                         nb, LB, t0, T if t1 is None else t1, int(gx.dtype != torch.float32))


def bwd_role(dy, lens, gates, cell, dgx, wimg, t0=0, t1=None, state=None, carry_in=False, dimg=None, b0=0, nb=None):
    T, LB, H = gates.shape[0], gates.shape[1], cell.shape[2]
    nb = LB - b0 if nb is None else nb
    return L.LstmBwdRole(dy.data_ptr() + 4 * dy.stride(1) * b0, dy.stride(1), lens.data_ptr() + 4 * b0, gates.data_ptr() + 16 * H * b0,
                         cell.data_ptr() + 4 * H * b0, dgx.data_ptr() + 16 * H * b0 if dgx is not None else None, L.ptr(wimg),
                         L.ptr(dimg.buf) if dimg is not None else None, dimg.ld if dimg is not None else 0,
                         dimg.buf.numel() // (2 * dimg.ld) if dimg is not None else 0, L.ptr(dimg.colsum) if dimg is not None else None,
                         L.ptr(state[0]) if state is not None else None, L.ptr(state[1]) if state is not None else None,
                         nb, LB, t0, T if t1 is None else t1, int(bool(carry_in)))


def roles_launch(roles, R, mode, device, backward=False, H=1024):
    if all(r.t1 <= r.t0 for r in roles):
        return
    c = roles_ctx(device)
    if R > c.reset_rows:
        L.check(L.lib().ft_lstm_roles_ctx_init(L.ptr(c.buf), L.stream()), "ft_lstm_roles_ctx_init")
        c.phase, c.reset_rows = [0, 0], R
    st = _persist_watch(c.buf.device)
    k = 1 if backward else 0
# ... 1 lines not shown
    fn = L.op16("ft_lstm_roles_bwd" if backward else "ft_lstm_roles_fwd", mode)
    L.check(fn(arr, len(roles), R, c.reset_rows, L.ptr(c.buf), c.phase[k], L.ptr(st.status), H, L.stream()), "ft_lstm_roles")
    c.phase[k] += 1
    _persist_arm(st)


def roles_plan(B, backward):
    cap = 64 if backward else 128
    out = []
    for b0 in range(0, B, cap):
        nb = min(cap, B - b0)
        out.append((b0, nb, 4 if nb <= 32 else 8 if nb <= 64 else 16))
    return out


_PAIR_CHUNKS_BWD = int(_os.environ.get("FLOWTRON_LSTM_PAIR_BWD", "3"))
_PAIR_CHUNKS = int(_os.environ.get("FLOWTRON_LSTM_PAIR", "6"))


def decoder_pair_chunks(B, H, mode, device, T):
    if _PAIR_CHUNKS <= 0 or B > 32 or T < 4 * _PAIR_CHUNKS or not lstm_persist_groups(B, H, False, mode, device):
        return 0
    return _PAIR_CHUNKS


def _chunk_edges(T, n):
    return [(k * T + n // 2) // n for k in range(n + 1)]


_EDGE_CACHE = {}


def _chunk_rowmaps(lens, edges, B):
    key = (tuple(edges), lens.device)
    ev = _EDGE_CACHE.get(key)
    if ev is None:
        T, n = edges[-1], len(edges) - 1
        k = torch.arange(n + 1, device=lens.device, dtype=torch.int64)
        e = torch.div(k * T + n // 2, n, rounding_mode="floor").to(torch.int32)
        if len(_EDGE_CACHE) > 64:
            _EDGE_CACHE.clear()
        ev = _EDGE_CACHE[key] = (e[:-1].contiguous(), (e[1:] - e[:-1]).contiguous())
    ck = (lens.data_ptr(), lens._version, key)
    if _EDGE_CACHE.get("last_key") == ck and _EDGE_CACHE["last_lens"]() is lens:
        return _EDGE_CACHE["last_maps"]
    lk = torch.minimum((lens[None, :] - ev[0][:, None]).clamp_(min=0), ev[1][:, None])
    maps = [RowMap(lk[k], edges[k + 1] - edges[k], B) for k in range(len(edges) - 1)]
    _EDGE_CACHE["last_key"], _EDGE_CACHE["last_lens"], _EDGE_CACHE["last_maps"] = ck, _weakref.ref(lens), maps
    return maps


def _gather_gemm_on():
    def num(name, default):
        try:
            return int(_os.environ.get(name, default))
        except ValueError:
            return 0
    return num("FT_GEMM_BF16_WIDE", "1") != 0 and num("FT_GEMM_BF16_TILE", "0") != 256


def _chunk_gathers(maps, lens, edges):
    for k, m in enumerate(maps):
        if getattr(m, "gather", None) is None:
            m.gather = ChunkGather(lens, m, edges[-1], edges[k], edges[k + 1])
    return [m.gather for m in maps]

# ... 13 lines not shown

    @staticmethod
    def forward(ctx, gx0, w_hh0, w_ih1, b_ih1, b_hh1, w_hh1, lens, mode, rowmap, gx_private, nchunks):
        gx0, w_hh0, w_ih1, w_hh1 = _c(gx0), _c(w_hh0), _c(w_ih1), _c(w_hh1)
        L.require_cuda(gx0, w_hh0, w_ih1, w_hh1, lens)
        T, B, H4 = gx0.shape
        H = H4 // 4
        dev = gx0.device
        f = dict(device=dev, dtype=torch.float32)
        y0, g0, c0 = torch.empty(T, B, H, **f), torch.empty(T, B, H4, **f), torch.empty(T, B, H, **f)
        y1, g1, c1 = torch.empty(T, B, H, **f), torch.empty(T, B, H4, **f), torch.empty(T, B, H, **f)
        g16 = gx0.dtype != torch.float32
        gx1 = torch.empty(T, B, H4, device=dev, dtype=gx0.dtype)
        st0, st1 = torch.empty(2, B, H, **f), torch.empty(2, B, H, **f)
        wi0, wi1 = roles_wimg(w_hh0, mode, False), roles_wimg(w_hh1, mode, False)
        w_img = Bf16Image.of_weight(w_ih1, mode)
        b1 = bias_sum(b_ih1, b_hh1).detach()
        edges = _chunk_edges(T, nchunks)
        rms = _chunk_rowmaps(lens, edges, B)
        for k in range(nchunks + 1):
            roles = []
            if k < nchunks:
                roles.append(fwd_role(gx0, lens, y0, g0, c0, wi0, edges[k], edges[k + 1], st0))
            if k > 0:
                roles.append(fwd_role(gx1, lens, y1, g1, c1, wi1, edges[k - 1], edges[k], st1))
            roles_launch(roles, 8 if len(roles) == 2 else 4, mode, dev)
            if k < nchunks:
                a, b = edges[k], edges[k + 1]
                x_img = Bf16Image(y0[a:b].reshape((b - a) * B, H), mode=mode, rowmap=rms[k])
                gemm_img(x_img, 0, x_img.ptr(), w_img, 0, w_img.ptr(), gx1[a:b], rms[k].cap, H4, H, H4, bias=b1, rowmap=rms[k], compact=1, c16=g16)
        ctx.save_for_backward(w_hh0, w_ih1, w_hh1, lens, y0, g0, c0, y1, g1, c1)
        ctx.mode, ctx.rowmap, ctx.gx_private, ctx.nchunks = mode, rowmap, bool(gx_private), nchunks
        ctx.chunk_maps, ctx.w_img, ctx.gx_dtype = (edges, rms), w_img, gx0.dtype
        return y1

    @staticmethod
    def backward(ctx, dy1):
        w_hh0, w_ih1, w_hh1, lens, y0, g0, c0, y1, g1, c1 = ctx.saved_tensors
        dy1 = _c(dy1)
        T, B, H = y1.shape
        H4, mode, rm, n = 4 * H, ctx.mode, ctx.rowmap, ctx.nchunks
        dev = dy1.device
        f = dict(device=dev, dtype=torch.float32)
        edges, rms = ctx.chunk_maps
        img_ok = rm is not None and _PERSIST_IMG != "0" and images_apply(mode, H4, H, (T - 1) * B) and (ctx.gx_private or _PERSIST_IMG == "both")
        img_only = img_ok and _PERSIST_IMG != "both" and not torch.is_anomaly_enabled()
        w_img = ctx.w_img if ctx.w_img is not None else Bf16Image.of_weight(w_ih1, mode)
        ctx.w_img = None
        nb = min(_PAIR_CHUNKS_BWD, T) if _PAIR_CHUNKS_BWD >= 0 else n
        if nb == 0 and rm is not None and img_ok and ctx.needs_input_grad[1] and ctx.needs_input_grad[5]:
            return DecoderPairFn._backward_sequential(ctx, dy1, w_img, img_only)
        if nb != n and nb > 0:
            n = nb
            edges = _chunk_edges(T, n)
            rms = _chunk_rowmaps(lens, edges, B)
        assert all(a < b for a, b in zip(edges, edges[1:])), "empty time window in the pair's backward pipeline"
        if rm is not None and img_only and ctx.needs_input_grad[1] and ctx.needs_input_grad[5] and T > 1 and _gather_gemm_on():
            return DecoderPairFn._backward_pipeline_img(ctx, dy1, w_img, n, edges, rms)
        dgx1 = torch.empty(T, B, H4, **f)
        dy0 = torch.empty(T, B, H, **f)
        d_img0 = Bf16Image.empty_rows(H4, rm, mode, dev) if img_ok else None
        dgx0 = None if img_only else torch.empty(T, B, H4, **f)
        sb1 = (torch.zeros(B, H4, **f), torch.zeros(B, H, **f))
        sb0 = (torch.zeros(B, H4, **f), torch.zeros(B, H, **f))
        wb0, wb1 = roles_wimg(w_hh0, mode, True), roles_wimg(w_hh1, mode, True)
        for j in range(n + 1):
            c = n - 1 - j
            roles = []
            if j < n:
                roles.append(bwd_role(dy1, lens, g1, c1, dgx1, wb1, edges[c], edges[c + 1], sb1, carry_in=c < n - 1))
            if j > 0:
                roles.append(bwd_role(dy0, lens, g0, c0, dgx0, wb0, edges[c + 1], edges[c + 2], sb0, carry_in=c + 1 < n - 1, dimg=d_img0))
            roles_launch(roles, 8 if len(roles) == 2 else 4, mode, dev, backward=True)
            if j < n:
                a, b = edges[c], edges[c + 1]
                d_img = Bf16Image(dgx1[a:b].reshape((b - a) * B, H4), mode=mode, rowmap=rms[c])
                gemm_img(d_img, 0, d_img.ptr(), w_img, 1, w_img.ptr(), dy0[a:b], rms[c].cap, H, H4, H, rowmap=rms[c], compact=1)
        dW_hh0 = dW_ih1 = dW_hh1 = db1 = None
        need = ctx.needs_input_grad
        compact_ok = rm is not None and T > 1 and images_apply(mode, H4, H, (T - 1) * B)
        if need[1] or need[2] or need[3] or need[4] or need[5]:
            if compact_ok:
                d_img1 = Bf16Image(dgx1.reshape(T * B, H4), colsum=True, mode=mode, rowmap=rm)
                db1 = d_img1.colsum
                y0_img, y1_img = shared_image(y0, T * B, H, mode, rm), shared_image(y1, T * B, H, mode, rm)
                if need[5]:
                    dW_hh1 = weight_grad_out(w_hh1)
                    gemm_img(d_img1, 1, d_img1.ptr(1), y1_img, 1, y1_img.ptr(0), dW_hh1, H4, H, rm.cap, H, beta=1.0, splitk=True, rowmap=rm, compact=2, k_shift=1)
                if need[2]:
                    dW_ih1 = weight_grad_out(w_ih1)
                    gemm_img(d_img1, 1, d_img1.ptr(), y0_img, 1, y0_img.ptr(), dW_ih1, H4, H, rm.cap, H, beta=1.0, splitk=True, rowmap=rm, compact=2)
                if need[1]:
                    d0 = d_img0 if d_img0 is not None else Bf16Image(dgx0.reshape(T * B, H4), colsum=True, mode=mode, rowmap=rm)
                    dW_hh0 = weight_grad_out(w_hh0)
                    gemm_img(d0, 1, d0.ptr(1), y0_img, 1, y0_img.ptr(0), dW_hh0, H4, H, rm.cap, H, beta=1.0, splitk=True, rowmap=rm, compact=2, k_shift=1)
                    d_img0 = d0
            else:
                rows = (T - 1) * B
# ... 35 lines not shown
    dW_hh1, dW_ih1, dW_hh0 = weight_grad_out(w_hh1), weight_grad_out(w_ih1), weight_grad_out(w_hh0)
    gemm_img(d_img1, 1, d_img1.ptr(1), y1_img, 1, y1_img.ptr(0), dW_hh1, H4, H, rm.cap, H, beta=1.0, splitk=True, rowmap=rm, compact=2, k_shift=1)
    dy0 = torch.empty(T, B, H, device=dev, dtype=torch.float32)
    gemm_img(d_img1, 0, d_img1.ptr(), w_img, 1, w_img.ptr(), dy0, rm.cap, H, H4, H, rowmap=rm, compact=1)
    gemm_img(d_img1, 1, d_img1.ptr(), y0_img, 1, y0_img.ptr(), dW_ih1, H4, H, rm.cap, H, beta=1.0, splitk=True, rowmap=rm, compact=2)
    dgx0 = None if img_only else torch.empty(T, B, H4, device=dev, dtype=torch.float32)
    d_img0 = recurrence(dy0, g0, c0, w_hh0, dgx0)
    gemm_img(d_img0, 1, d_img0.ptr(1), y0_img, 1, y0_img.ptr(0), dW_hh0, H4, H, rm.cap, H, beta=1.0, splitk=True, rowmap=rm, compact=2, k_shift=1)
    if img_only:
        dgx0 = image_only_gradient((T, B, H4), dev, ctx.gx_dtype)
        _handoff_put_image_only(dgx0, d_img0)
    else:
        if ctx.gx_dtype != torch.float32:
            dgx0 = dgx0.to(ctx.gx_dtype)
        _handoff_put(dgx0, d_img0)
    db1 = d_img1.colsum
    return dgx0, dW_hh0, dW_ih1, db1, db1, dW_hh1, None, None, None, None, None


DecoderPairFn._backward_sequential = staticmethod(_pair_backward_sequential)


def _pair_backward_pipeline_img(ctx, dy1, w_img, n, edges, rms):
    w_hh0, w_ih1, w_hh1, lens, y0, g0, c0, y1, g1, c1 = ctx.saved_tensors
    T, B, H = y1.shape
    H4, mode, rm = 4 * H, ctx.mode, ctx.rowmap
    dev = dy1.device
    f = dict(device=dev, dtype=torch.float32)
    gr = _chunk_gathers(rms, lens, edges)
    d_img1, d_img0 = Bf16Image.empty_rows(H4, rm, mode, dev), Bf16Image.empty_rows(H4, rm, mode, dev)
    dy0 = torch.empty(T, B, H, **f)
    st = torch.empty(2, B * (H4 + H), **f)
    sb1, sb0 = (st[0, :B * H4], st[0, B * H4:]), (st[1, :B * H4], st[1, B * H4:])
    wb0, wb1 = roles_wimg(w_hh0, mode, True), roles_wimg(w_hh1, mode, True)
    for j in range(n + 1):
        c = n - 1 - j
        roles = []
        if j < n:
            roles.append(bwd_role(dy1, lens, g1, c1, None, wb1, edges[c], edges[c + 1], sb1, carry_in=c < n - 1, dimg=d_img1))
        if j > 0:
            roles.append(bwd_role(dy0, lens, g0, c0, None, wb0, edges[c + 1], edges[c + 2], sb0, carry_in=c + 1 < n - 1, dimg=d_img0))
        roles_launch(roles, 8 if len(roles) == 2 else 4, mode, dev, backward=True)
        if j < n:
            a, b = edges[c], edges[c + 1]
            gemm_img(d_img1, 0, d_img1.ptr(), w_img, 1, w_img.ptr(), dy0[a:b], gr[c].cap, H, H4, H, rowmap=gr[c], compact=1, a_rows=gr[c].a_rows)
    y0_img, y1_img = y_image(y0, T * B, H, mode, rm), y_image(y1, T * B, H, mode, rm)
    dW_hh1, dW_ih1, dW_hh0 = weight_grad_out(w_hh1), weight_grad_out(w_ih1), weight_grad_out(w_hh0)
    gemm_img(d_img1, 1, d_img1.ptr(1), y1_img, 1, y1_img.ptr(0), dW_hh1, H4, H, rm.cap, H, beta=1.0, splitk=True, rowmap=rm, compact=2, k_shift=1)
    gemm_img(d_img1, 1, d_img1.ptr(), y0_img, 1, y0_img.ptr(), dW_ih1, H4, H, rm.cap, H, beta=1.0, splitk=True, rowmap=rm, compact=2)
    gemm_img(d_img0, 1, d_img0.ptr(1), y0_img, 1, y0_img.ptr(0), dW_hh0, H4, H, rm.cap, H, beta=1.0, splitk=True, rowmap=rm, compact=2, k_shift=1)
    dgx0 = image_only_gradient((T, B, H4), dev, ctx.gx_dtype)
    _handoff_put_image_only(dgx0, d_img0)
    db1 = d_img1.colsum
    return dgx0, dW_hh0, dW_ih1, db1, db1, dW_hh1, None, None, None, None, None


DecoderPairFn._backward_pipeline_img = staticmethod(_pair_backward_pipeline_img)


def decoder_pair(x, lens, p, mode, xs_extra, rowmap, fill, gate, nchunks):
    xs = [x] + list(xs_extra)
    T, B = x.shape[0], x.shape[1]
    gates = None
    if gx16_ok(mode, rowmap, T, B, p.weight_hh_l0.shape[1], False, xs, p.weight_ih_l0.shape[0], x.device):
        fill = fill + "|c16"
    if gate is not None and linear_gate_fusable(mode, rowmap, xs, p.weight_ih_l0.shape[0]):
        gx, gates = LinearGateFn.apply(p.weight_ih_l0, bias_sum(p.bias_ih_l0, p.bias_hh_l0), gate[0], gate[1], mode, rowmap, fill, *xs)
# ... 312 lines not shown

    @staticmethod
    def _args(Q, V, text, w_key, v, w1, b1, w2, b2, in_lens, out_ctx, attn, logprob, cumm_all, kproj_all, work, temperature, mode):
        T, B, A = Q.shape
        Lk, _, E = text.shape
        base = (work.data_ptr() + 255) // 256 * 256
        return L.CummAttnArgs(L.ptr(text), L.ptr(Q), L.ptr(V), L.ptr(w_key), L.ptr(v), L.ptr(w1), L.ptr(b1), L.ptr(w2), L.ptr(b2),
                              L.ptr(in_lens), L.ptr(out_ctx), L.ptr(attn), L.ptr(logprob), L.ptr(cumm_all), L.ptr(kproj_all),
                              base, work.numel() - (base - work.data_ptr()), T, B, Lk, E, A, w1.shape[0], w1.shape[2], w2.shape[2],
                              float(temperature), int(mode), None)

    @staticmethod
    def backward(ctx, dctx, dattn, dlogprob):
        Q, V, text, w_key, v, w1, b1, w2, b2, in_lens, attn, cumm_all, kproj_all = ctx.saved_tensors
        T, B, A = Q.shape
        Lk, _, E = text.shape
        NF, _, K1 = w1.shape
        K2 = w2.shape[2]
        f = dict(device=Q.device, dtype=torch.float32)
        dctx = _c(dctx) if dctx is not None else torch.zeros(T, B, A, **f)
        dattn = _c(dattn) if dattn is not None else None
        dlogprob = _c(dlogprob) if dlogprob is not None else None
        dQ, dV, dtext = torch.empty_like(Q), torch.empty_like(V), torch.empty_like(text)
        dwk, dv, dw1, db1, dw2, db2 = (torch.empty_like(t) for t in (w_key, v, w1, b1, w2, b2))
        work = torch.empty(L.lib().ft_cumm_attn_workspace_bytes(T, Lk, B, E, A, NF, K1, K2, int(ctx.mode), 1) + 256, device=Q.device, dtype=torch.uint8)
        scratch = torch.empty(1, **f)
        args = CummAttnSeqFn._args(Q, V, text, w_key, v, w1, b1, w2, b2, in_lens, scratch, attn, scratch, cumm_all, kproj_all, work,
                                   ctx.temperature, ctx.mode)
        L.check(L.lib().ft_cumm_attn_bwd(C.byref(args), L.ptr(dctx), L.ptr(dattn), L.ptr(dlogprob), L.ptr(dQ), L.ptr(dV), L.ptr(dtext),
                                         L.ptr(dwk), L.ptr(dv), L.ptr(dw1), L.ptr(db1), L.ptr(dw2), L.ptr(db2), L.stream()), "ft_cumm_attn_bwd")
        return dQ, dV, dtext, dwk, dv.reshape(1, -1), dw1, db1, dw2, db2, None, None, None


class AffineFn(torch.autograd.Function):
    @staticmethod
    def forward(ctx, out, x):
        out, x = _c(out), _c(x)
        L.require_cuda(out, x)
        M = x.shape[-1]
        rows = x.numel() // M
        z = torch.empty_like(x)
        L.check(L.lib().ft_affine_fwd(L.ptr(out), L.ptr(x), L.ptr(z), rows, M, L.stream()), "ft_affine_fwd")
        ctx.save_for_backward(out, x)
        return z

    @staticmethod
    def backward(ctx, dz):
        out, x = ctx.saved_tensors
        dz = _c(dz)
        M = x.shape[-1]
        rows = x.numel() // M
        dout = torch.empty_like(out)
        dx = torch.empty_like(x)
        L.check(L.lib().ft_affine_bwd(L.ptr(out), L.ptr(x), L.ptr(dz), None, L.ptr(dout), L.ptr(dx), rows, M, L.stream()),
                "ft_affine_bwd")
        return dout, dx


class ReverseByLengthFn(torch.autograd.Function):

    @staticmethod
    def forward(ctx, x, lens, time_major):
        x = _c(x)
        L.require_cuda(x, lens)
        if time_major:
            T, B, Cc = x.shape
        else:
            B, T, Cc = x.shape
        y = torch.empty_like(x)
        L.check(L.lib().ft_reverse_by_length(L.ptr(x), L.ptr(y), L.ptr(lens), T, B, Cc, int(time_major), L.stream()),
                "ft_reverse_by_length")
        ctx.save_for_backward(lens)
        ctx.time_major = time_major
        return y

    @staticmethod
    def backward(ctx, dy):
        (lens,) = ctx.saved_tensors
        return ReverseByLengthFn.apply(_c(dy), lens, ctx.time_major), None, None


def reverse_by_length(x, lens, time_major=True):
    return ReverseByLengthFn.apply(x, lens, time_major)


class NLLFn(torch.autograd.Function):

    @staticmethod
    def forward(ctx, z, lens, sigma, *log_s):
# ... 276 lines not shown
```

include/flowtron_hip.h:

```cpp
#ifndef FLOWTRON_HIP_H
#define FLOWTRON_HIP_H

#include <stddef.h>
#include <stdint.h>

#ifdef __cplusplus
extern "C" {
#endif

#define FT_ABI_VERSION 14

enum { FT_OK = 0, FT_EINVAL = -1, FT_EHIP = -2, FT_EUNSUPPORTED = -3 };
enum { FT_F32 = 0, FT_BF16 = 1, FT_F16 = 2 };
enum { FT_ACT_NONE = 0, FT_ACT_TANH = 1, FT_ACT_RELU = 2, FT_ACT_SIGMOID = 3 };
enum { FT_GEMM_SPLITK = 1, FT_GEMM_SPLITK_DET = 2, FT_GEMM_C16 = 4 };

int ft_abi_version(void);
const char* ft_last_error(void);
int ft_debug_hold_cus(int n_wg, int64_t ticks, void* stream);

typedef struct {
    const float* A; const float* B; float* C; const float* bias;
    int M, N, K, batch;
    int64_t sAm, sAk, sBk, sBn, ldc;
// ... 12 lines not shown
    int M, N, K;
    int64_t lda, ldb, ldc;
    int a_kmajor, b_kmajor;
    float alpha, beta;
    int act, flags;
    const int32_t* rowmap; const int32_t* rows_dev;
    int compact, k_shift;
    const float* r1_row; const float* r1_col;
    void* split_work; size_t split_work_bytes;
    const int32_t* a_rows;
} ft_gemm_img_args;
size_t ft_gemm_img_split_work_bytes(int M, int N, int K);
size_t ft_bf16_image_bytes(int64_t rows, int64_t cols);
int ft_bf16_image(const float* src, int64_t ld, int64_t rows, int64_t cols, void* dst, void* stream);
int ft_bf16_image_colsum(const float* src, int64_t ld, int64_t rows, int64_t cols, void* dst, float* colsum, void* stream);
int ft_gemm_img(const ft_gemm_img_args* a, void* stream);
int ft_bf16_image_colsum_acc(const float* src, int64_t ld, int64_t rows, int64_t cols, void* dst, float* colsum, void* stream);
int ft_bf16_image_rows_acc(const float* src, int64_t ld, int64_t cap_rows, int64_t cols, void* dst, float* colsum,
                           const int32_t* rowmap, const int32_t* rows_dev, void* stream);
int ft_bf16_image_rows_act_bwd_acc(const float* dy, int64_t ld, const float* y, int64_t ldy, int act, int64_t cap_rows, int64_t cols,
                                   void* dst, float* colsum, const int32_t* rowmap, const int32_t* rows_dev, void* stream);
int ft_bf16_image_colsum_acc_f16(const float* src, int64_t ld, int64_t rows, int64_t cols, void* dst, float* colsum, void* stream);
int ft_bf16_image_rows_acc_f16(const float* src, int64_t ld, int64_t cap_rows, int64_t cols, void* dst, float* colsum,
                               const int32_t* rowmap, const int32_t* rows_dev, void* stream);
int ft_bf16_image_rows_act_bwd_acc_f16(const float* dy, int64_t ld, const float* y, int64_t ldy, int act, int64_t cap_rows, int64_t cols,
                                       void* dst, float* colsum, const int32_t* rowmap, const int32_t* rows_dev, void* stream);
int ft_bf16_image_split3(const float* src, int64_t ld, int64_t rows, int64_t cols, void* dst, int weight, void* stream);
int ft_bf16_image_split3_f16(const float* src, int64_t ld, int64_t rows, int64_t cols, void* dst, int weight, void* stream);
int ft_bf16_image_split3_im2col(const float* x, const int32_t* lens, int L, int B, int C, int KW, void* dst, void* stream);
int ft_bf16_image_split3_im2col_f16(const float* x, const int32_t* lens, int L, int B, int C, int KW, void* dst, void* stream);
typedef struct { const float* src; int64_t ld; int64_t rows; int64_t cols; void* dst; int kind; } ft_img_desc;
int ft_bf16_image_table(const ft_img_desc* descs, int n, void* stream);
int ft_bf16_image_table_f16(const ft_img_desc* descs, int n, void* stream);
int ft_rowmap_build(const int32_t* lens, int32_t* rowmap, int32_t* rows_dev, int T, int B, void* stream);
int ft_chunk_gather_rows(const int32_t* lens, int32_t* a_rows, int32_t* rowmap, int T, int B, int t0, int t1, void* stream);
int ft_bf16_image_rows(const float* src, int64_t ld, int64_t cap_rows, int64_t cols, void* dst, float* colsum,
                       const int32_t* rowmap, const int32_t* rows_dev, void* stream);
int ft_bf16_image_rows_act_bwd(const float* dy, int64_t ld, const float* y, int64_t ldy, int act, int64_t cap_rows, int64_t cols,
                               void* dst, float* colsum, const int32_t* rowmap, const int32_t* rows_dev, void* stream);
int ft_bf16_image_rows_act_bwd_f16(const float* dy, int64_t ld, const float* y, int64_t ldy, int act, int64_t cap_rows, int64_t cols,
                                   void* dst, float* colsum, const int32_t* rowmap, const int32_t* rows_dev, void* stream);
int ft_bf16_image_rows_into(const float* src, int64_t ld, int64_t cap_rows, int64_t cols, void* dst, int64_t dst_ld, int64_t col_off,
                            int64_t fill_cols, const int32_t* rowmap, const int32_t* rows_dev, void* stream);
int ft_bf16_image_rows_into_f16(const float* src, int64_t ld, int64_t cap_rows, int64_t cols, void* dst, int64_t dst_ld, int64_t col_off,
                                int64_t fill_cols, const int32_t* rowmap, const int32_t* rows_dev, void* stream);
int ft_img_gemv_rows(const void* img, int64_t ld, int K, const float* w, const float* bias, float* y, int64_t ldy,
                     const int32_t* rowmap, const int32_t* rows_dev, const int32_t* lens, int T, int B, void* stream);
int ft_img_gemv_rows_f16(const void* img, int64_t ld, int K, const float* w, const float* bias, float* y, int64_t ldy,
                         const int32_t* rowmap, const int32_t* rows_dev, const int32_t* lens, int T, int B, void* stream);
int ft_img_gemv_rows_bwd(const void* img, int64_t ld, int K, const float* dy, int64_t lddy, float* dw, float* db,
                         const int32_t* rowmap, const int32_t* rows_dev, int64_t cap_rows, void* stream);
int ft_img_gemv_rows_bwd_f16(const void* img, int64_t ld, int K, const float* dy, int64_t lddy, float* dw, float* db,
                             const int32_t* rowmap, const int32_t* rows_dev, int64_t cap_rows, void* stream);
int ft_pad_rows_fill(float* y, int64_t ld, int cols, const int32_t* lens, int T, int B, int mode, void* stream);

int ft_embedding_fwd(const int64_t* ids, const float* W, float* out, int n, int dim, int64_t ld_out, void* stream);
int ft_embedding_bwd(const int64_t* ids, const float* dout, float* dW, int n, int dim, int64_t ld_dout, void* stream);
int ft_embedding_bwd_runs(const int64_t* ids, const float* dout, float* dW, int n, int dim, int64_t ld_dout, int stride, void* stream);

int ft_im2col(const float* x, float* col, const int32_t* lens, int L, int B, int C, int KW, void* stream);
int ft_col2im(const float* dcol, float* dx, const int32_t* lens, int L, int B, int C, int KW, void* stream);

int ft_instnorm_relu_fwd(const float* x, const float* gamma, const float* beta, const float* keep,
                         const int32_t* lens, float* y, float* mean, float* rstd,
                         int L, int B, int C, float eps, void* stream);
int ft_instnorm_relu_bwd(const float* x, const float* y, const float* dy, const float* gamma, const float* keep,
                         const int32_t* lens, const float* mean, const float* rstd,
                         float* dx, float* dgamma, float* dbeta, int L, int B, int C, void* stream);

size_t ft_lstm_workspace_bytes(int B, int H);
int ft_lstm_seq_fwd(const float* gx, const float* w_hh, const int32_t* lens,
                    float* y, int64_t ldy, float* gates, float* cell, void* work,
                    int T, int B, int H, int reverse, int mode, void* stream);
int ft_lstm_seq_bwd(const float* dy, int64_t ldy, const float* w_hh, const int32_t* lens,
                    const float* gates, const float* cell, float* dgx, void* work,
                    int T, int B, int H, int reverse, int mode, void* stream);

int ft_lstm_persist_supported(int B, int H);
size_t ft_lstm_persist_workspace_bytes(int B, int H);
int ft_lstm_persist_debug_prof(void* dev_buf);
int ft_lstm_persist_bwd(const float* dy, int64_t ldy, const float* w_hh, const int32_t* lens, const float* gates,
                        const float* cell, float* dgx, void* work, int32_t* status, int T, int B, int H, int ng, void* stream);
int ft_lstm_persist_bwd_img(const float* dy, int64_t ldy, const float* w_hh, const int32_t* lens, const float* gates,
                            const float* cell, float* dgx, void* work, int32_t* status, int T, int B, int H, int ng,
                            void* dimg, int64_t dimg_ld, int64_t dimg_rows, float* dbias, void* stream);

typedef struct {
// ... 29 lines not shown
                     void* work, int T, int B, int H, void* stream);
int ft_lstm2_seq_bwd(const float* dy1, const float* w_hh0, const float* w_ih1, const float* w_hh1, const int32_t* lens,
                     const float* gates0, const float* cell0, const float* gates1, const float* cell1,
                     float* dgx0, float* dgx1, void* work, int T, int B, int H, void* stream);

int ft_lstm_bidir_supported(int B, int H);
int ft_lstm_bidir_seq_fwd(const float* gx_f, const float* gx_r, const float* w_hh_f, const float* w_hh_r,
                          const int32_t* lens, float* y, int64_t ldy, float* gates_f, float* gates_r,
                          float* cell_f, float* cell_r, void* work_f, void* work_r, int T, int B, int H, void* stream);
int ft_lstm_bidir_seq_bwd(const float* dy, int64_t ldy, const float* w_hh_f, const float* w_hh_r, const int32_t* lens,
                          const float* gates_f, const float* gates_r, const float* cell_f, const float* cell_r,
                          float* dgx_f, float* dgx_r, void* work_f, void* work_r, int T, int B, int H, void* stream);

int ft_bilstm_persist_supported(int B, int H);
size_t ft_bilstm_persist_workspace_bytes(int B, int H);
int ft_bilstm_persist_fwd(const float* gx_f, const float* gx_r, const float* w_hh_f, const float* w_hh_r, const int32_t* lens,
                          float* y, int64_t ldy, float* gates_f, float* gates_r, float* cell_f, float* cell_r,
                          void* work, int32_t* status, int T, int B, int H, void* stream);
int ft_bilstm_persist_bwd(const float* dy, int64_t ldy, const float* w_hh_f, const float* w_hh_r, const int32_t* lens,
                          const float* gates_f, const float* gates_r, const float* cell_f, const float* cell_r,
                          float* dgx_f, float* dgx_r, void* work, int32_t* status, int T, int B, int H, void* stream);

int ft_attention_fwd(const float* Q, const float* K, const float* v, const int32_t* in_lens, const float* prior,
                     float* attn, float* logprob, float* p_save,
                     int T, int B, int L, int A, float temperature, void* stream);
int ft_attention_bwd(const float* Q, const float* K, const float* v, const int32_t* in_lens, const float* prior,
                     const float* attn, const float* p_save, const float* dattn, const float* dlogprob,
                     float* de_work, float* dQ, float* dK, float* dv,
                     int T, int B, int L, int A, float temperature, void* stream);

int ft_affine_fwd(const float* out, const float* x, float* z, int64_t n_rows, int M, void* stream);
int ft_affine_bwd(const float* out, const float* x, const float* dz, const float* dlog_s_ext,
                  float* dout, float* dx, int64_t n_rows, int M, void* stream);
int ft_affine_inv(const float* out, const float* z, float* x, int64_t n_rows, int M, void* stream);

int ft_masked_sum(const float* x, int64_t ld, const int32_t* lens, float* acc, int square,
                  int T, int B, int M, void* stream);
int ft_masked_sum_bwd(const float* x, int64_t ld, const int32_t* lens, const float* scale_dev, float coef, int square,
                      float* dx, int64_t ld_dx, int T, int B, int M, void* stream);

int ft_gate_bce_fwd(const float* gate, const float* target, const int32_t* lens, float* acc, int T, int B, void* stream);
int ft_gate_bce_bwd(const float* gate, const float* target, const int32_t* lens, const float* scale_dev, float coef,
                    float* dgate, int T, int B, void* stream);

int ft_flowtron_loss_fwd(const float* z, const float* const* log_s, int n_ls, int64_t ld_ls, const float* gate,
                         const float* gate_target, const int32_t* out_lens, float sigma, float* acc, float* nll_out,
                         float* gate_out, int T, int B, int M, void* stream);
int ft_flowtron_loss_bwd(const float* z, const float* gate, const float* gate_target, const int32_t* out_lens, float sigma,
                         const float* acc, const float* g_nll, const float* g_gate, float* dz, float* dls, float* dgate,
                         int T, int B, int M, void* stream);

int ft_reverse_by_length(const float* x, float* y, const int32_t* lens, int T, int B, int C, int time_major, void* stream);

int ft_act_bwd(const float* y, const float* dy, float* dpre, int64_t n, int act, void* stream);

int ft_eltwise(const float* a, const float* b, float* out, int64_t n, int op, void* stream);

int ft_colsum(const float* x, float* out, int64_t rows, int N, int64_t ld, void* stream);

typedef struct {
      const float *att_w_ih, *att_w_hh, *att_b_ih, *att_b_hh;
       const float *w_query, *v, *K, *V;
       const float *l0_w_ih, *l0_w_hh, *l0_b_ih, *l0_b_hh, *l1_w_ih, *l1_w_hh, *l1_b_ih, *l1_b_hh;
       const float *d0_w, *d0_b, *d1_w, *d1_b, *conv_w, *conv_b;
       const float *gate_w, *gate_b;
    const float* residual;
// ... 150 lines not shown
```

Before: 705,300 mel-frames/s.

## Batch step-map construction, fuse affine with reversal, and prebuild LSTM weight images

```diff
diff --git a/flowtron_amd/_lib.py b/flowtron_amd/_lib.py
--- a/flowtron_amd/_lib.py
+++ b/flowtron_amd/_lib.py
@@ -47,6 +47,14 @@
 
 class ImgDesc(C.Structure):
     _fields_ = [("src", _p), ("ld", _l), ("rows", _l), ("cols", _l), ("dst", _p), ("kind", _i)]
+
+
+class StepMapJob(C.Structure):
+    _fields_ = [("kind", C.c_int32), ("t0", C.c_int32), ("t1", C.c_int32)]
+
+
+IMG_TABLE_MAX = 48
+IMG_PLAIN, IMG_SPLIT, IMG_FRAG_ROLES_FWD, IMG_FRAG_ROLES_BWD, IMG_FRAG_BILSTM_FWD, IMG_FRAG_BILSTM_BWD = range(6)
 
 
 class CummAttnArgs(C.Structure):
@@ -94,6 +102,9 @@
     "ft_bf16_image_table_f16": ([C.POINTER(ImgDesc), _i, _p], _i),
     "ft_bf16_image_split3_f16": ([_p, _l, _l, _l, _p, _i, _p], _i),
     "ft_rowmap_build": ([_p, _p, _p, _i, _i, _p], _i),
+    "ft_step_maps_plan": ([_i, _i, C.POINTER(StepMapJob), _i, C.POINTER(_l)], _l),
+    "ft_step_maps": ([_p, _p, _l, _i, _i, C.POINTER(StepMapJob), _i, _p], _i),
+    "ft_bilstm_wimg_prepare": ([_p, _p, _i, _i, _p], _i),
     "ft_chunk_gather_rows": ([_p, _p, _p, _i, _i, _i, _i, _p], _i),
     "ft_bf16_image_rows": ([_p, _l, _l, _l, _p, _p, _p, _p, _p], _i),
     "ft_bf16_image_rows_acc": ([_p, _l, _l, _l, _p, _p, _p, _p, _p], _i),
@@ -103,6 +114,10 @@
     "ft_bf16_image_rows_act_bwd": ([_p, _l, _p, _l, _i, _l, _l, _p, _p, _p, _p, _p], _i),
     "ft_bf16_image_rows_act_bwd_acc": ([_p, _l, _p, _l, _i, _l, _l, _p, _p, _p, _p, _p], _i),
     "ft_pad_rows_fill": ([_p, _l, _i, _p, _i, _i, _i, _p], _i),
+    "ft_pad_rows_fill_tail": ([_p, _l, _i, _p, _i, _i, _p], _i),
+    "ft_bf16_image_rows_shift": ([_p, _l, _l, _l, _p, _p, _p, _i, _p], _i),
+    "ft_affine_fwd_rev": ([_p, _p, _p, _p, _i, _i, _i, _p], _i),
+    "ft_affine_bwd_rev": ([_p, _p, _p, _p, _p, _p, _p, _i, _i, _i, _p], _i),
     "ft_embedding_fwd": ([_p, _p, _p, _i, _i, _l, _p], _i),
     "ft_embedding_bwd": ([_p, _p, _p, _i, _i, _l, _p], _i),
     "ft_embedding_bwd_runs": ([_p, _p, _p, _i, _i, _l, _i, _p], _i),
@@ -193,7 +208,7 @@
 
 OP16_TWINS = ("ft_gemm", "ft_bf16_image", "ft_bf16_image_colsum", "ft_bf16_image_colsum_acc", "ft_bf16_image_rows_acc", "ft_bf16_image_rows_act_bwd_acc", "ft_gemm_img", "ft_bf16_image_rows", "ft_bf16_image_rows_into", "ft_bf16_image_rows_act_bwd", "ft_img_gemv_rows", "ft_img_gemv_rows_bwd", "ft_lstm_seq_fwd", "ft_lstm_seq_bwd",
               "ft_lstm_persist_bwd", "ft_lstm_persist_bwd_img", "ft_lstm_roles_prepare_fwd", "ft_lstm_roles_prepare_bwd", "ft_lstm_roles_fwd", "ft_lstm_roles_bwd", "ft_lstm2_seq_fwd", "ft_lstm2_seq_bwd",
-              "ft_lstm_bidir_seq_fwd", "ft_lstm_bidir_seq_bwd", "ft_bilstm_persist_fwd", "ft_bilstm_persist_bwd")
+              "ft_lstm_bidir_seq_fwd", "ft_lstm_bidir_seq_bwd", "ft_bilstm_persist_fwd", "ft_bilstm_persist_bwd", "ft_bilstm_wimg_prepare", "ft_bf16_image_rows_shift")
 for _n in OP16_TWINS:
     SIGNATURES[_n + "_f16"] = SIGNATURES[_n]
 
diff --git a/flowtron_amd/csrc/bilstm_persist.hip b/flowtron_amd/csrc/bilstm_persist.hip
--- a/flowtron_amd/csrc/bilstm_persist.hip
+++ b/flowtron_amd/csrc/bilstm_persist.hip
@@ -340,3 +340,12 @@
     FT_CHECK_LAUNCH();
     return FT_OK;
 }
+
+extern "C" int FT_OPNAME(ft_bilstm_wimg_prepare)(const float* w_hh, void* wimg, int H, int backward, void* stream) {
+    FT_CHECK_ARG(w_hh && wimg && H == BH && reinterpret_cast<uintptr_t>(wimg) % 256 == 0);
+    hipStream_t st = reinterpret_cast<hipStream_t>(stream);
+    if (backward) hipLaunchKernelGGL(make_wfrag_bwd, dim3(256), dim3(256), 0, st, w_hh, reinterpret_cast<unsigned short*>(wimg), H, WfragAux{});
+    else hipLaunchKernelGGL(make_wfrag_fwd, dim3(256), dim3(256), 0, st, w_hh, reinterpret_cast<unsigned short*>(wimg), H, WfragAux{});
+    FT_CHECK_LAUNCH();
+    return FT_OK;
+}
diff --git a/flowtron_amd/csrc/elementwise.hip b/flowtron_amd/csrc/elementwise.hip
--- a/flowtron_amd/csrc/elementwise.hip
+++ b/flowtron_amd/csrc/elementwise.hip
@@ -116,27 +116,35 @@
     }
 }
 
+__device__ __forceinline__ long rev_row(long r, const int* __restrict__ lens, int T, int B) {
+    const int t = (int)(r / B), b = (int)(r - (long)t * B);
+    int len = lens[b];
+    len = len < 0 ? 0 : (len > T ? T : len);
+    const int d = (t < len) ? (len - 1 - t) : (T - 1 + len - t);
+    return (long)d * B + b;
+}
 __global__ void affine_fwd_k(const float* __restrict__ out, const float* __restrict__ x, float* __restrict__ z,
-                             long n_rows, int M) {
+                             long n_rows, int M, const int* __restrict__ rev_lens = nullptr, int T = 0, int B = 0) {
     const long total = n_rows * M;
     for (long i = blockIdx.x * (long)blockDim.x + threadIdx.x; i < total; i += (long)gridDim.x * blockDim.x) {
         const long r = i / M;
         const int c = (int)(i - r * M);
         const float ls = out[r * 2 * M + c], bb = out[r * 2 * M + M + c];
-        z[i] = expf(ls) * x[i] + bb;
+        const long o = rev_lens ? rev_row(r, rev_lens, T, B) * M + c : i;
+        z[o] = expf(ls) * x[i] + bb;
     }
 }
 __global__ void affine_bwd_k(const float* __restrict__ out, const float* __restrict__ x, const float* __restrict__ dz,
                              const float* __restrict__ dls_ext, float* __restrict__ dout, float* __restrict__ dx,
-                             long n_rows, int M) {
+                             long n_rows, int M, const int* __restrict__ rev_lens = nullptr, int T = 0, int B = 0) {
     const long total = n_rows * M;
     for (long i = blockIdx.x * (long)blockDim.x + threadIdx.x; i < total; i += (long)gridDim.x * blockDim.x) {
         const long r = i / M;
         const int c = (int)(i - r * M);
         const float s = expf(out[r * 2 * M + c]);
-        const float g = dz[i];
+        const float g = dz[rev_lens ? rev_row(r, rev_lens, T, B) * M + c : i];
         float dls = g * x[i] * s;
-        if (dls_ext) dls += dls_ext[i];
+        if (dls_ext) dls = __fadd_rn(dls, dls_ext[i]);
         dout[r * 2 * M + c] = dls;
         dout[r * 2 * M + M + c] = g;
         if (dx) dx[i] = g * s;
@@ -387,11 +395,51 @@
     if (threadIdx.x == 0) { a_rows[offc_b + lk_b] = near < 0 ? 0 : near; rowmap[offc_b + lk_b] = -1; }
 }
 
+constexpr int STEP_MAPS_MAX_JOBS = 56;
+struct StepMapsArgs {
+    const int* lens;
+    int* out;
+    int T, B;
+    int kind[STEP_MAPS_MAX_JOBS], t0[STEP_MAPS_MAX_JOBS], t1[STEP_MAPS_MAX_JOBS];
+    int o_lens[STEP_MAPS_MAX_JOBS], o_map[STEP_MAPS_MAX_JOBS], o_rows[STEP_MAPS_MAX_JOBS], o_arows[STEP_MAPS_MAX_JOBS];
+};
+__global__ void step_maps_k(StepMapsArgs a) {
+    const int j = blockIdx.y, b = blockIdx.x, T = a.T, B = a.B;
+    const int t0 = a.t0[j], w = a.t1[j] - t0;
+    const int* __restrict__ lens = a.lens;
+    if (a.kind[j] == 2) {
+        int* __restrict__ a_rows = a.out + a.o_arows[j];
+        int* __restrict__ rowmap = a.out + a.o_map[j];
+        int off = 0, offc = 0, near = -1, off_b = 0, offc_b = 0, lk_b = 0;
+        for (int i = 0; i < B; ++i) {
+            int l = lens[i]; l = l < 0 ? 0 : (l > T ? T : l);
+            int lk = l - t0; lk = lk < 0 ? 0 : (lk > w ? w : lk);
+            if (i == b) { off_b = off; offc_b = offc; lk_b = lk; }
+            if (lk > 0 && (i <= b || near < 0)) near = off + t0 + lk - 1;
+            off += l + 1; offc += lk + 1;
+        }
+        for (int t = threadIdx.x; t < lk_b; t += blockDim.x) { a_rows[offc_b + t] = off_b + t0 + t; rowmap[offc_b + t] = t * B + b; }
+        if (threadIdx.x == 0) { a_rows[offc_b + lk_b] = near < 0 ? 0 : near; rowmap[offc_b + lk_b] = -1; }
+        return;
+    }
+    int* __restrict__ rowmap = a.out + a.o_map[j];
+    int off = 0;
+    for (int i = 0; i < b; ++i) { int l = lens[i] - t0; l = l < 0 ? 0 : (l > w ? w : l); off += l + 1; }
+    int len = lens[b] - t0;
+    len = len < 0 ? 0 : (len > w ? w : len);
+    for (int t = threadIdx.x; t < len; t += blockDim.x) rowmap[off + t] = t * B + b;
+    if (threadIdx.x == 0) {
+        rowmap[off + len] = len < w ? len * B + b : -1;
+        if (b == B - 1) a.out[a.o_rows[j]] = off + len + 1;
+        if (a.kind[j] == 1) a.out[a.o_lens[j] + b] = len;
+    }
+}
+
 __global__ void pad_fill_k(float* __restrict__ y, long ld, int cols, const int* __restrict__ lens, int T, int B, int mode) {
     const int row = blockIdx.x, t = row / B, b = row % B;
     int len = lens[b];
     len = len < 0 ? 0 : len;
-    if (t <= len) return;
+    if (t <= len && t < T) return;
     const float* src = y + (size_t)(len * B + b) * ld;
     float* dst = y + (size_t)row * ld;
     for (int c = blockIdx.y * blockDim.x + threadIdx.x; c < cols; c += gridDim.y * blockDim.x) dst[c] = mode ? src[c] : 0.f;
@@ -539,6 +587,23 @@
     FT_CHECK_LAUNCH();
     return FT_OK;
 }
+extern "C" int ft_affine_fwd_rev(const float* out, const float* x, float* z, const int32_t* lens, int T, int B, int M, void* stream) {
+    FT_CHECK_ARG(out && x && z && lens && T >= 0 && B >= 1 && M >= 1);
+    if (T == 0) return FT_OK;
+    const long n_rows = (long)T * B;
+    hipLaunchKernelGGL(affine_fwd_k, dim3(grid_for(n_rows * M)), dim3(NT), 0, ST(stream), out, x, z, n_rows, M, lens, T, B);
+    FT_CHECK_LAUNCH();
+    return FT_OK;
+}
+extern "C" int ft_affine_bwd_rev(const float* out, const float* x, const float* dz, const float* dlog_s_ext, float* dout, float* dx,
+                                 const int32_t* lens, int T, int B, int M, void* stream) {
+    FT_CHECK_ARG(out && x && dz && dout && lens && T >= 0 && B >= 1 && M >= 1);
+    if (T == 0) return FT_OK;
+    const long n_rows = (long)T * B;
+    hipLaunchKernelGGL(affine_bwd_k, dim3(grid_for(n_rows * M)), dim3(NT), 0, ST(stream), out, x, dz, dlog_s_ext, dout, dx, n_rows, M, lens, T, B);
+    FT_CHECK_LAUNCH();
+    return FT_OK;
+}
 extern "C" int ft_affine_inv(const float* out, const float* z, float* x, int64_t n_rows, int M, void* stream) {
     FT_CHECK_ARG(out && z && x && n_rows >= 0 && M >= 1);
     if (n_rows == 0) return FT_OK;
@@ -690,12 +755,53 @@
     FT_CHECK_LAUNCH();
     return FT_OK;
 }
+static int64_t step_maps_layout(int T, int B, const ft_step_map_job* jobs, int n, int64_t* off) {
+    if (!jobs || n < 1 || n > STEP_MAPS_MAX_JOBS || T < 1 || B < 1 || (int64_t)T * B + B >= (1ll << 31)) return -1;
+    auto up64 = [](int64_t v) { return (v + 63) / 64 * 64; };
+    int64_t at = 0;
+    for (int j = 0; j < n; ++j) {
+        const ft_step_map_job& q = jobs[j];
+        if (q.kind < 0 || q.kind > 2 || q.t0 < 0 || q.t0 >= q.t1 || q.t1 > T || (q.kind == 0 && (q.t0 != 0 || q.t1 != T))) return -1;
+        const int64_t cap = (int64_t)(q.t1 - q.t0) * B + B;
+        int64_t o[4] = {-1, -1, -1, -1};
+        if (q.kind == 1) { o[0] = at; at += up64(B); }
+        if (q.kind == 2) { o[3] = at; at += cap; }
+        o[1] = at; at += up64(cap);
+        if (q.kind != 2) { o[2] = at; at += 64; }
+        if (off) for (int e = 0; e < 4; ++e) off[4 * j + e] = o[e];
+    }
+    return at < (1ll << 31) ? at : -1;
+}
+extern "C" int64_t ft_step_maps_plan(int T, int B, const ft_step_map_job* jobs, int n_jobs, int64_t* offsets) {
+    return step_maps_layout(T, B, jobs, n_jobs, offsets);
+}
+extern "C" int ft_step_maps(const int32_t* lens, int32_t* out, int64_t out_ints, int T, int B, const ft_step_map_job* jobs, int n_jobs,
+                            void* stream) {
+    int64_t off[4 * STEP_MAPS_MAX_JOBS];
+    const int64_t need = step_maps_layout(T, B, jobs, n_jobs, off);
+    FT_CHECK_ARG(lens && out && need > 0 && need <= out_ints);
+    StepMapsArgs a{};
+    a.lens = lens; a.out = out; a.T = T; a.B = B;
+    for (int j = 0; j < n_jobs; ++j) {
+        a.kind[j] = jobs[j].kind; a.t0[j] = jobs[j].t0; a.t1[j] = jobs[j].t1;
+        a.o_lens[j] = (int)off[4 * j]; a.o_map[j] = (int)off[4 * j + 1]; a.o_rows[j] = (int)off[4 * j + 2]; a.o_arows[j] = (int)off[4 * j + 3];
+    }
+    hipLaunchKernelGGL(step_maps_k, dim3(B, n_jobs), dim3(256), 0, ST(stream), a);
+    FT_CHECK_LAUNCH();
+    return FT_OK;
+}
 extern "C" int ft_pad_rows_fill(float* y, int64_t ld, int cols, const int32_t* lens, int T, int B, int mode, void* stream) {
     FT_CHECK_ARG(y && lens && T >= 1 && B >= 1 && cols >= 1 && ld >= cols && (mode == 0 || mode == 1));
     hipLaunchKernelGGL(pad_fill_k, dim3(T * B, cols > 1024 ? 4 : 1), dim3(256), 0, ST(stream), y, (long)ld, cols, lens, T, B, mode);
     FT_CHECK_LAUNCH();
     return FT_OK;
 }
+extern "C" int ft_pad_rows_fill_tail(float* y, int64_t ld, int cols, const int32_t* lens, int T, int B, void* stream) {
+    FT_CHECK_ARG(y && lens && T >= 1 && B >= 1 && cols >= 1 && ld >= cols && (int64_t)(T + 1) * B < (1ll << 31));
+    hipLaunchKernelGGL(pad_fill_k, dim3((T + 1) * B, cols > 1024 ? 4 : 1), dim3(256), 0, ST(stream), y, (long)ld, cols, lens, T, B, 0);
+    FT_CHECK_LAUNCH();
+    return FT_OK;
+}
 extern "C" int ft_poison_if_nonzero(const int32_t* status_dev, float* dst, void* stream) {
     FT_CHECK_ARG(status_dev && dst);
     hipLaunchKernelGGL(poison_k, dim3(1), dim3(1), 0, ST(stream), status_dev, dst);
diff --git a/flowtron_amd/csrc/gemm_bf16.hip b/flowtron_amd/csrc/gemm_bf16.hip
--- a/flowtron_amd/csrc/gemm_bf16.hip
+++ b/flowtron_amd/csrc/gemm_bf16.hip
@@ -24,7 +24,7 @@
 __device__ __forceinline__ void img_rows_body(const float* __restrict__ src, long sr, long sc, int R, int Cc,
                                               unsigned short* __restrict__ dst, int Rp, int Cp, int vec,
                                               const int* __restrict__ rowmap, const int* __restrict__ rdev, long dld,
-                                              size_t first, size_t stride) {
+                                              size_t first, size_t stride, int rshift = 0) {
     const int cq = Cp >> 3;
     int Rz = Rp;
     if (rdev) R = mapped_rows(rdev, Rp, Rz);
@@ -33,6 +33,7 @@
         const int ri = (int)(i / cq), c = (int)(i % cq) * 8;
         int r = ri;
         if (rowmap) r = ri < R ? rowmap[ri] : -1;
+        if (rshift && r >= 0) r -= rshift;
         float v[8] = {0.f, 0.f, 0.f, 0.f, 0.f, 0.f, 0.f, 0.f};
         if (r >= 0 && (rowmap || r < R) && c < Cc) {
             const float* p = src + (size_t)r * sr + (size_t)c * sc;
@@ -49,9 +50,9 @@
 }
 __global__ __launch_bounds__(256) void img_rows_k(const float* __restrict__ src, long sr, long sc, int R, int Cc,
                                                   unsigned short* __restrict__ dst, int Rp, int Cp, int vec,
-                                                  const int* __restrict__ rowmap, const int* __restrict__ rdev, long dld) {
+                                                  const int* __restrict__ rowmap, const int* __restrict__ rdev, long dld, int rshift) {
     img_rows_body(src, sr, sc, R, Cc, dst, Rp, Cp, vec, rowmap, rdev, dld, blockIdx.x * (size_t)blockDim.x + threadIdx.x,
-                  (size_t)gridDim.x * blockDim.x);
+                  (size_t)gridDim.x * blockDim.x, rshift);
 }
 
 __device__ __forceinline__ void img_split3_body(const float* __restrict__ src, long sr, int R, int K, unsigned short* __restrict__ dst,
@@ -115,7 +116,39 @@
     }
 }
 
-constexpr int IMG_TABLE_MAX = 32;
+__device__ __forceinline__ void img_wfrag_body(const float* __restrict__ w, unsigned short* __restrict__ out, int H, int kind,
+                                               size_t first, size_t stride) {
+    const size_t total = (size_t)H * H >> 1;
+    for (size_t i8 = first; i8 < total; i8 += stride) {
+        const int lane = (int)(i8 & 63), li = lane & 15, kg = lane >> 4;
+        const size_t rest = i8 >> 6;
+        float v[8];
+        if (kind == 2 || kind == 4) {
+            const int nchunk = H >> 5;
+            const int c = (int)(rest % nchunk), jb = (int)(rest / nchunk);
+            const size_t row = kind == 2 ? (size_t)(li & 3) * H + jb * 4 + (li >> 2) : (size_t)(li >> 2) * H + jb * 4 + (li & 3);
+            const float* p = w + row * H + c * 32 + kg * 8;
+            const float4 a = *reinterpret_cast<const float4*>(p), b = *reinterpret_cast<const float4*>(p + 4);
+            v[0] = a.x; v[1] = a.y; v[2] = a.z; v[3] = a.w; v[4] = b.x; v[5] = b.y; v[6] = b.z; v[7] = b.w;
+        } else {
+            size_t r, col;
+            if (kind == 3) {
+                const int ntile = H >> 4;
+                const int g = (int)(rest & 3), jt = (int)((rest >> 2) % ntile), q = (int)((rest >> 2) / ntile);
+                r = (size_t)g * H + q * 32 + kg * 8; col = (size_t)jt * 16 + li;
+            } else {
+                const int nchunk = (4 * H) >> 5;
+                const int c = (int)(rest % nchunk), jt = (int)(rest / nchunk);
+                r = (size_t)c * 32 + kg * 8; col = (size_t)jt * 16 + li;
+            }
+#pragma unroll
+            for (int e = 0; e < 8; ++e) v[e] = w[(r + e) * H + col];
+        }
+        *reinterpret_cast<uint4*>(out + i8 * 8) = pack8(v);
+    }
+}
+
+constexpr int IMG_TABLE_MAX = 48;
 struct ImgTable {
     const float* src[IMG_TABLE_MAX];
     unsigned short* dst[IMG_TABLE_MAX];
@@ -130,6 +163,7 @@
     const size_t first = (size_t)((int)blockIdx.x - t.blk0[d]) * blockDim.x + threadIdx.x;
     const size_t stride = (size_t)(t.blk0[d + 1] - t.blk0[d]) * blockDim.x;
     if (t.kind[d] == 0) img_rows_body(t.src[d], t.sr[d], 1, t.R[d], t.Cc[d], t.dst[d], t.Rp[d], t.Cp[d], t.vec[d], nullptr, nullptr, (long)t.Cp[d], first, stride);
+    else if (t.kind[d] >= 2) img_wfrag_body(t.src[d], t.dst[d], t.Cc[d], t.kind[d], first, stride);
     else img_split3_body(t.src[d], t.sr[d], t.R[d], t.Cc[d], t.dst[d], t.Rp[d], t.Cp[d], 1, first, stride);
 }
 
@@ -199,12 +233,12 @@
 }
 
 void make_image(const float* src, long sr, long sc, int R, int Cc, unsigned short* dst, int Rp, int Cp, hipStream_t st,
-                const int* rowmap = nullptr, const int* rdev = nullptr, long dld = 0) {
+                const int* rowmap = nullptr, const int* rdev = nullptr, long dld = 0, int rshift = 0) {
     const bool vec = sc == 1 && reinterpret_cast<uintptr_t>(src) % 16 == 0 && sr % 4 == 0;
     const size_t chunks = (size_t)Rp * (Cp >> 3);
     const int blocks = (int)((chunks + 255) / 256 < 16384 ? (chunks + 255) / 256 : 16384);
     hipLaunchKernelGGL(img_rows_k, dim3(blocks), dim3(256), 0, st, src, sr, sc, R, Cc, dst, Rp, Cp, vec ? 1 : 0, rowmap, rdev,
-                       dld ? dld : (long)Cp);
+                       dld ? dld : (long)Cp, rshift);
 }
 
 struct BfP {
@@ -811,13 +845,15 @@
     for (int i = 0; i < n; ++i) {
         const ft_img_desc& d = descs[i];
         FT_CHECK_ARG(d.src && d.dst && d.rows >= 1 && d.cols >= 1 && d.ld >= d.cols && d.rows < (1ll << 31) - 256 && 3 * d.cols < (1ll << 31) - 256);
-        FT_CHECK_ARG(reinterpret_cast<uintptr_t>(d.dst) % 256 == 0 && (d.kind == 0 || (d.kind == 1 && d.cols % 8 == 0)));
+        FT_CHECK_ARG(reinterpret_cast<uintptr_t>(d.dst) % 256 == 0 && d.kind >= 0 && d.kind <= 5 && (d.kind != 1 || d.cols % 8 == 0));
+        FT_CHECK_ARG(d.kind < 2 || (d.rows == 4 * d.cols && d.ld == d.cols && d.cols % 32 == 0 && d.cols <= 16384 &&
+                                    reinterpret_cast<uintptr_t>(d.src) % 16 == 0));
         t.src[i] = d.src; t.dst[i] = reinterpret_cast<unsigned short*>(d.dst); t.sr[i] = (long)d.ld;
         t.R[i] = (int)d.rows; t.Cc[i] = (int)d.cols; t.kind[i] = d.kind;
         t.Rp[i] = (int)up((size_t)d.rows + 32, 256);
         t.Cp[i] = (int)up((size_t)(d.kind == 1 ? 3 * d.cols : d.cols), 256);
         t.vec[i] = (reinterpret_cast<uintptr_t>(d.src) % 16 == 0 && d.ld % 4 == 0) ? 1 : 0;
-        const size_t chunks = (size_t)t.Rp[i] * (t.Cp[i] >> 3);
+        const size_t chunks = d.kind >= 2 ? (size_t)d.cols * d.cols / 2 : (size_t)t.Rp[i] * (t.Cp[i] >> 3);
         const int nb = (int)((chunks + 255) / 256 < 2048 ? (chunks + 255) / 256 : 2048);
         t.blk0[i] = blocks;
         blocks += nb;
@@ -950,6 +986,15 @@
     FT_CHECK_LAUNCH();
     return FT_OK;
 }
+extern "C" int FT_OPNAME(ft_bf16_image_rows_shift)(const float* src, int64_t ld, int64_t cap_rows, int64_t cols, void* dst,
+                                                   const int32_t* rowmap, const int32_t* rows_dev, int row_shift, void* stream) {
+    FT_CHECK_ARG(src && dst && rowmap && rows_dev && cap_rows >= 1 && cols >= 1 && ld >= cols && cap_rows < (1ll << 31) - 512 && cols < (1ll << 31) - 256);
+    FT_CHECK_ARG(reinterpret_cast<uintptr_t>(dst) % 256 == 0 && row_shift >= 0);
+    make_image(src, ld, 1, (int)cap_rows, (int)cols, reinterpret_cast<unsigned short*>(dst), (int)up((size_t)cap_rows + 32, 256),
+               (int)up((size_t)cols, 256), reinterpret_cast<hipStream_t>(stream), rowmap, rows_dev, 0, row_shift);
+    FT_CHECK_LAUNCH();
+    return FT_OK;
+}
 extern "C" int FT_OPNAME(ft_bf16_image_rows)(const float* src, int64_t ld, int64_t cap_rows, int64_t cols, void* dst, float* colsum,
                                              const int32_t* rowmap, const int32_t* rows_dev, void* stream) {
     return image_rows_impl(src, ld, cap_rows, cols, dst, colsum, rowmap, rows_dev, true, stream);
diff --git a/flowtron_amd/model.py b/flowtron_amd/model.py
--- a/flowtron_amd/model.py
+++ b/flowtron_amd/model.py
@@ -176,14 +176,15 @@
         d["_decode_work"] = None
         return d
 
-    def forward(self, mel, text, in_lens32, out_lens32, attn_prior=None, rowmap=None):
+    def forward(self, mel, text, in_lens32, out_lens32, attn_prior=None, rowmap=None, z_rev=False):
         T, B, M = mel.shape
         mode = L.mfma_mode()
         rm = rowmap
-        mel0 = torch.cat([mel.new_zeros(1, B, M), mel[:-1]], 0)
         a = self.attention_lstm
+        shift = ops.linear_shift_fusable(mode, rm, mel, a.weight_ih_l0.shape[0]) and not ops.lstm_pad_width(B, a.weight_hh_l0.shape[1], False, mode, mel.device, T)
+        mel0 = mel if shift else torch.cat([mel.new_zeros(1, B, M), mel[:-1]], 0)
         h_att = ops.lstm_layer(mel0, out_lens32, a.weight_ih_l0, a.weight_hh_l0, a.bias_ih_l0, a.bias_hh_l0, mode=mode, rowmap=rm,
-                               fill="dx")
+                               fill="dx|shift" if shift else "dx")
         if self.use_cumm_attention:
             ctx, attn, logprob = self.run_cumm_attn_sequence(h_att, text, in_lens32)
         else:
@@ -223,8 +224,12 @@
             h = ops.lstm_layer(h, out_lens32, p.weight_ih_l1, p.weight_hh_l1, p.bias_ih_l1, p.bias_hh_l1, mode=mode, rowmap=rm)
         h = self.dense_layer(h, rowmap=rm)
         out = ops.linear(h, self.conv.weight.reshape(self.conv.weight.shape[0], -1), self.conv.bias, mode=mode, rowmap=rm, fill="y")
-        z = ops.AffineFn.apply(out, mel)
-        log_s = out[..., :M]
+        rev = out_lens32 if z_rev else None
+        if ops._AFFINE_LOGS:
+            z, log_s = ops.AffineFn.apply(out, mel, True, rev)
+        else:
+            z = ops.AffineFn.apply(out, mel, False, rev)
+            log_s = out[..., :M]
         return z, log_s, gates, attn, logprob
 
     def run_cumm_attn_sequence(self, h_att, text, in_lens32):
@@ -477,12 +482,15 @@
                                n_attn_channels, n_lstm_layers, add_gate, use_cumm_attention)
         self.ar_step._time_reversed = True
 
-    def forward(self, mel, text, in_lens32, out_lens32, attn_prior=None, rowmap=None):
-        mel = ops.reverse_by_length(mel, out_lens32, True)
+    def forward(self, mel, text, in_lens32, out_lens32, attn_prior=None, rowmap=None, z_rev=False, mel_reversed=False):
+        if not mel_reversed:
+            mel = ops.reverse_by_length(mel, out_lens32, True)
         if attn_prior is not None:
             attn_prior = ops.reverse_by_length(attn_prior, out_lens32, False)
-        z, log_s, gates, attn, logprob = self.ar_step(mel, text, in_lens32, out_lens32, attn_prior, rowmap=rowmap)
-        z = ops.reverse_by_length(z, out_lens32, True)
+        fold = ops._AFFINE_REVERSE and not z_rev
+        z, log_s, gates, attn, logprob = self.ar_step(mel, text, in_lens32, out_lens32, attn_prior, rowmap=rowmap, z_rev=fold)
+        if not fold and not z_rev:
+            z = ops.reverse_by_length(z, out_lens32, True)
         return z, log_s, gates, attn, logprob
 
     def infer(self, residual, text, attns=None, attn_prior=None):
@@ -580,8 +588,14 @@
         def run_flows(x, enc):
             log_s_list, attns_list, attns_logprob_list = [], [], []
             gate = None
-            for flow in self.flows:
-                x, log_s, gate, attn, logprob = flow(x, enc, in32, out32, attn_prior, rowmap=rm)
+            reversed_x = False
+            for i, flow in enumerate(self.flows):
+                nxt = self.flows[i + 1] if i + 1 < len(self.flows) else None
+                want = ops._AFFINE_REVERSE and isinstance(nxt, AR_Back_Step)
+                kw = dict(mel_reversed=reversed_x) if isinstance(flow, AR_Back_Step) else {}
+                assert not reversed_x or kw
+                x, log_s, gate, attn, logprob = flow(x, enc, in32, out32, attn_prior, rowmap=rm, z_rev=want, **kw)
+                reversed_x = want
                 log_s_list.append(log_s)
                 attns_list.append(attn)
                 attns_logprob_list.append(logprob)
diff --git a/flowtron_amd/ops.py b/flowtron_amd/ops.py
--- a/flowtron_amd/ops.py
+++ b/flowtron_amd/ops.py
@@ -47,6 +47,62 @@
                                          1 if copy_separator else 0, L.stream()), "ft_pad_rows_fill")
 
 
+_STEP_MAPS = _os.environ.get("FLOWTRON_STEP_MAPS", "1") != "0"
+_STEP_MAPS_LAST = {"sm": None}
+
+
+class StepMaps:
+
+    def __init__(self, lens32, T, B, edge_sets=(), gather_edges=None):
+        L.require_cuda(lens32)
+        T, B = int(T), int(B)
+        sets = []
+        for e in edge_sets:
+            if e is not None and tuple(e) not in sets:
+                sets.append(tuple(e))
+        gather_edges = tuple(gather_edges) if gather_edges is not None else None
+        assert gather_edges is None or gather_edges in sets
+        jobs = [(0, 0, T)] + [(1, e[k], e[k + 1]) for e in sets for k in range(len(e) - 1)]
+        if gather_edges is not None:
+            jobs += [(2, gather_edges[k], gather_edges[k + 1]) for k in range(len(gather_edges) - 1)]
+        arr = (L.StepMapJob * len(jobs))(*[L.StepMapJob(*j) for j in jobs])
+        off = (C.c_int64 * (4 * len(jobs)))()
+        total = L.lib().ft_step_maps_plan(T, B, arr, len(jobs), off)
+        if total < 0:
+            raise RuntimeError("ft_step_maps_plan: invalid jobs (T=%d B=%d, %d jobs)" % (T, B, len(jobs)))
+        buf = torch.empty(total, device=lens32.device, dtype=torch.int32)
+        L.check(L.lib().ft_step_maps(L.ptr(lens32), L.ptr(buf), total, T, B, arr, len(jobs), L.stream()), "ft_step_maps")
+        self.buf, self.T, self.B, self.version, self.lens_ref = buf, T, B, lens32._version, _weakref.ref(lens32)
+
+        def rowmap(j, lens, w):
+            m = RowMap.__new__(RowMap)
+            m.T, m.B, m.cap, m.lens, m.gather = w, B, w * B + B, lens, None
+            m.map, m.rows = buf[off[4 * j + 1]:off[4 * j + 1] + m.cap], buf[off[4 * j + 2]:off[4 * j + 2] + 1]
+            return m
+        self.whole = rowmap(0, lens32, T)
+        self.chunks, j = {}, 1
+        for e in sets:
+            self.chunks[e] = []
+            for k in range(len(e) - 1):
+                self.chunks[e].append(rowmap(j, buf[off[4 * j]:off[4 * j] + B], e[k + 1] - e[k]))
+                j += 1
+        if gather_edges is not None:
+            for m in self.chunks[gather_edges]:
+                g = ChunkGather.__new__(ChunkGather)
+                g.cap, g.rows = m.cap, m.rows
+                g.a_rows, g.map = buf[off[4 * j + 3]:off[4 * j + 3] + m.cap], buf[off[4 * j + 1]:off[4 * j + 1] + m.cap]
+                m.gather = g
+                j += 1
+
+
+def _step_edge_sets(T, B):
+    nf = _PAIR_CHUNKS if (_PAIR_CHUNKS > 0 and B <= 32 and T >= 4 * _PAIR_CHUNKS) else 0
+    if nf <= 0 or nf > 16:
+        return None, None
+    nb = min(_PAIR_CHUNKS_BWD, T) if _PAIR_CHUNKS_BWD >= 0 else nf
+    return _chunk_edges(T, nf), (_chunk_edges(T, nb) if 0 < nb <= 16 else None)
+
+
 _COMPACT = _os.environ.get("FLOWTRON_GEMM_COMPACT", "1") != "0"
 _FUSE_ACT_BWD = True
 _ENC_SPLITK = "det"
@@ -55,13 +111,19 @@
 
 
 def row_map(lens32, T, B):
-    return RowMap(lens32, T, B) if (_COMPACT and _BF16_IMAGES) else None
+    if not (_COMPACT and _BF16_IMAGES):
+        return None
+    if _STEP_MAPS:
+        ef, eb = _step_edge_sets(int(T), int(B))
+        sm = _STEP_MAPS_LAST["sm"] = StepMaps(lens32, T, B, (ef, eb), eb if eb is not None else ef)
+        return sm.whole
+    return RowMap(lens32, T, B)
 
 
 class Bf16Image:
     __slots__ = ("buf", "rows", "cols", "ld", "colsum", "fmt", "rowmap")
 
-    def __init__(self, t2d, colsum=False, mode=None, rowmap=None):
+    def __init__(self, t2d, colsum=False, mode=None, rowmap=None, row_shift=0):
         assert t2d.dim() == 2 and t2d.stride(1) == 1 and t2d.dtype == torch.float32
         L.require_cuda(t2d)
         self.rows, self.cols = int(t2d.shape[0]), int(t2d.shape[1])
@@ -73,9 +135,16 @@
             assert self.rows == rowmap.T * rowmap.B, "row map built for another [T, B]"
             self.rows = rowmap.cap
             self.buf = torch.empty(L.lib().ft_bf16_image_bytes(self.rows, self.cols), device=t2d.device, dtype=torch.uint8)
+            if row_shift:
+                assert not colsum
+                L.check(L.op16("ft_bf16_image_rows_shift", self.fmt)(L.ptr(t2d), int(t2d.stride(0)), self.rows, self.cols, L.ptr(self.buf),
+                                                                      L.ptr(rowmap.map), L.ptr(rowmap.rows), int(row_shift), L.stream()),
+                        "ft_bf16_image_rows_shift")
+                return
             L.check(L.op16("ft_bf16_image_rows_acc", self.fmt)(L.ptr(t2d), int(t2d.stride(0)), self.rows, self.cols, L.ptr(self.buf), L.ptr(self.colsum),
                                                                 L.ptr(rowmap.map), L.ptr(rowmap.rows), L.stream()), "ft_bf16_image_rows_acc")
             return
+        assert not row_shift
         self.buf = torch.empty(L.lib().ft_bf16_image_bytes(self.rows, self.cols), device=t2d.device, dtype=torch.uint8)
         if colsum:
             L.check(L.op16("ft_bf16_image_colsum_acc", self.fmt)(L.ptr(t2d), int(t2d.stride(0)), self.rows, self.cols, L.ptr(self.buf), L.ptr(self.colsum),
@@ -124,27 +193,7 @@
 
     @classmethod
     def of_weight(cls, W, mode, split=False):
-        w = _WIMG
-        key = (W.data_ptr(), tuple(W.shape), mode, bool(split))
-        if w["plan_next"] is not None:
-            w["plan_next"][key] = W
-        if w["armed"]:
-            w["armed"] = False
-            plan = [(k, t) for k, t in w["plan"].items() if t.is_cuda and t.device == W.device and t.dtype == torch.float32 and t.is_contiguous()
-                    and t.data_ptr() == k[0] and tuple(t.shape) == k[1]]
-            for lo in range(0, len(plan), 32):
-                part = plan[lo:lo + 32]
-                by_fmt = {}
-                for k, t in part:
-                    by_fmt.setdefault(k[2], []).append((k, t))
-                for fmt, items in by_fmt.items():
-                    descs = (L.ImgDesc * len(items))()
-                    for i, (k, t) in enumerate(items):
-                        img = cls._blank(t.shape[0], (3 if k[3] else 1) * t.shape[1], fmt, t.device)
-                        descs[i] = L.ImgDesc(t.data_ptr(), int(t.stride(0)), int(t.shape[0]), int(t.shape[1]), img.buf.data_ptr(), 1 if k[3] else 0)
-                        w["cache"][k] = img
-                    L.check(L.op16("ft_bf16_image_table", fmt)(descs, len(items), L.stream()), "ft_bf16_image_table")
-        img = w["cache"].get(key)
+        img = _wimg_request(W, mode, bool(split))
         if img is not None:
             return img
         return cls.split3(W, mode, True) if split else cls(W, mode=mode)
@@ -179,6 +228,38 @@
 
 _WIMG_ON = True
 _WIMG = {"plan": {}, "plan_next": None, "cache": {}, "armed": False, "plans": None}
+
+
+def _wimg_request(W, mode, kind):
+    w = _WIMG
+    key = (W.data_ptr(), tuple(W.shape), mode, kind)
+    if w["plan_next"] is not None:
+        w["plan_next"][key] = W
+    if w["armed"]:
+        w["armed"] = False
+        plan = [(k, t) for k, t in w["plan"].items() if t.is_cuda and t.device == W.device and t.dtype == torch.float32 and t.is_contiguous()
+                and t.data_ptr() == k[0] and tuple(t.shape) == k[1] and (int(k[3]) < 2 or _wfrag_ok(t))]
+        for lo in range(0, len(plan), L.IMG_TABLE_MAX):
+            part = plan[lo:lo + L.IMG_TABLE_MAX]
+            by_fmt = {}
+            for k, t in part:
+                by_fmt.setdefault(k[2], []).append((k, t))
+            for fmt, items in by_fmt.items():
+                descs = (L.ImgDesc * len(items))()
+                for i, (k, t) in enumerate(items):
+                    if int(k[3]) >= 2:
+                        img = dst = torch.empty(L.lib().ft_lstm_roles_wimg_bytes(t.shape[1]), device=t.device, dtype=torch.uint8)
+                    else:
+                        img = Bf16Image._blank(t.shape[0], (3 if k[3] else 1) * t.shape[1], fmt, t.device)
+                        dst = img.buf
+                    descs[i] = L.ImgDesc(t.data_ptr(), int(t.stride(0)), int(t.shape[0]), int(t.shape[1]), dst.data_ptr(), int(k[3]))
+                    w["cache"][k] = img
+                L.check(L.op16("ft_bf16_image_table", fmt)(descs, len(items), L.stream()), "ft_bf16_image_table")
+    return w["cache"].get(key)
+
+
+def _wfrag_ok(t):
+    return t.dim() == 2 and t.shape[0] == 4 * t.shape[1] and t.shape[1] % 32 == 0 and t.data_ptr() % 16 == 0 and t.is_contiguous()
 
 
 def weight_images_begin(model):
@@ -432,6 +513,16 @@
     if t is None:
         t = e[2][scale] = e[1].sum().to(torch.float32) * scale if scale != 1.0 else e[1].sum().to(torch.float32)
     return t
+
+
+_SHIFT_IMAGE = _os.environ.get("FLOWTRON_SHIFT_IMAGE", "1") != "0"
+
+
+def linear_shift_fusable(mode, rowmap, x, N):
+    if not _SHIFT_IMAGE or rowmap is None or isinstance(mode, tuple) or x.dim() != 3 or x.dtype != torch.float32:
+        return False
+    T, B, K = x.shape
+    return rowmap.T == T and rowmap.B == B and K % 4 == 0 and linear_uses_images(mode, T * B, N, [x])
 
 
 def linear_uses_images(mode, rows, N, xs):
@@ -475,6 +566,8 @@
             rowmap = None
         ctx.imgs = split_imgs if split_fwd else None
         ctx.cat = False
+        ctx.shift = "shift" in fill
+        assert not ctx.shift or (use_img and rowmap is not None and len(xs) == 1 and "dx" in fill)
         ctx.img_kind = ("split3" if split_imgs is not None else None) if split_fwd else ("images" if use_img else None)
         ctx.lazy_src = lazy if split_fwd else None
         if use_img:
@@ -484,7 +577,8 @@
                 ctx.imgs, ctx.cat = (w_img, [x_cat]), True
                 gemm_img(x_cat, 0, x_cat.ptr(), w_img, 0, w_img.ptr(), y, rowmap.cap, N, Ktot, N, bias=bias, act=act, rowmap=rowmap, compact=1, c16=c16)
             else:
-                x_imgs = [shared_image(x, rows, x.shape[-1], mode, rowmap) for x in xs]
+                x_imgs = ([Bf16Image(xs[0].reshape(rows, Ktot), mode=mode, rowmap=rowmap, row_shift=rowmap.B)] if ctx.shift else
+                          [shared_image(x, rows, x.shape[-1], mode, rowmap) for x in xs])
                 ctx.imgs = (w_img, x_imgs)
         off = 0
         for i, x in enumerate(xs):
@@ -560,7 +654,13 @@
         for i, x in enumerate(xs):
             K = x.shape[-1]
             if ctx.needs_input_grad[6 + i]:
-                if imgs is not None:
+                if imgs is not None and ctx.shift:
+                    Ts, Bs = rowmap.T, rowmap.B
+                    buf = torch.empty((Ts + 1) * Bs, K, device=x.device, dtype=torch.float32)
+                    gemm_img(d_img, 0, d_img.ptr(), w_img, 1, w_img.ptr(0, off), buf, mrows, K, N, K, rowmap=rowmap, compact=1)
+                    L.check(L.lib().ft_pad_rows_fill_tail(L.ptr(buf), K, K, L.ptr(rowmap.lens), Ts, Bs, L.stream()), "ft_pad_rows_fill_tail")
+                    dx = buf[Bs:].view(x.shape)
+                elif imgs is not None:
                     dx, acc = _dx_buffer(x)
                     gemm_img(d_img, 0, d_img.ptr(), w_img, 1, w_img.ptr(0, off), dx, mrows, K, N, K, beta=1.0 if acc else 0.0,
                              rowmap=rowmap, compact=1)
@@ -581,7 +681,7 @@
                 if imgs is not None:
                     gemm_img(d_img, 1, d_img.ptr(), x_imgs[i], 1, x_imgs[i].ptr(), dW[:, off:], N, K, mrows, Ktot, beta=1.0, splitk=True,
                              rowmap=rowmap, compact=2)
-                    if rowmap is not None:
+                    if rowmap is not None and not ctx.shift:
                         _handoff_put_x(x, x_imgs[i])
                 else:
                     gemm_raw(dpre, x, dW[:, off:], N, K, rows, 1, N, K, 1, Ktot, mode=ctx.mode_dw, splitk=True)
@@ -599,6 +699,8 @@
     w_img = Bf16Image.of_weight(W, ctx.mode)
     if ctx.cat:
         return w_img, [Bf16Image.cat_rows([x.reshape(rows, x.shape[-1]) for x in xs], ctx.mode, ctx.rowmap)]
+    if getattr(ctx, "shift", False):
+        return w_img, [Bf16Image(xs[0].reshape(rows, Ktot), mode=ctx.mode, rowmap=ctx.rowmap, row_shift=ctx.rowmap.B)]
     return w_img, [shared_image(x, rows, x.shape[-1], ctx.mode, ctx.rowmap) for x in xs]
 
 
@@ -964,10 +1066,14 @@
 _BIAS_SUMS = {}
 
 
+_BIAS_SUMS_LAZY = _os.environ.get("FLOWTRON_BIAS_SUMS_LAZY", "1") != "0"
+
+
 class _BiasSumsFn(torch.autograd.Function):
     @staticmethod
     def forward(ctx, *flat):
         n = len(flat) // 2
+        ctx.set_materialize_grads(not _BIAS_SUMS_LAZY)
         return tuple(torch._foreach_add(list(flat[:n]), list(flat[n:])))
 
     @staticmethod
@@ -1052,10 +1158,24 @@
     return c
 
 
+_WFRAG_TABLE = _os.environ.get("FLOWTRON_WFRAG_TABLE", "1") != "0"
+
+
+def roles_wimg_bwd_pair(ws, mode):
+    if not _WFRAG_TABLE or _WIMG["plan_next"] is None:
+        return None
+    imgs = [(_wimg_request(w, mode, L.IMG_FRAG_ROLES_BWD) if _wfrag_ok(w) else None) for w in ws]
+    return imgs if all(i is not None for i in imgs) else None
+
+
 def roles_wimg(w_hh, mode, backward):
+    w = _c(w_hh)
+    if _WFRAG_TABLE and _wfrag_ok(w):
+        img = _wimg_request(w, mode, L.IMG_FRAG_ROLES_BWD if backward else L.IMG_FRAG_ROLES_FWD)
+        if img is not None:
+            return img
     img = torch.empty(L.lib().ft_lstm_roles_wimg_bytes(w_hh.shape[1]), device=w_hh.device, dtype=torch.uint8)
     fn = L.op16("ft_lstm_roles_prepare_bwd" if backward else "ft_lstm_roles_prepare_fwd", mode)
-    w = _c(w_hh)
     L.check(fn(L.ptr(w), L.ptr(img), w.shape[1], L.stream()), "ft_lstm_roles_prepare")
     return img
 
@@ -1123,6 +1243,9 @@
 
 
 def _chunk_rowmaps(lens, edges, B):
+    sm = _STEP_MAPS_LAST["sm"] if _STEP_MAPS else None
+    if sm is not None and sm.lens_ref() is lens and sm.version == lens._version and sm.B == B and tuple(edges) in sm.chunks:
+        return sm.chunks[tuple(edges)]
     key = (tuple(edges), lens.device)
     ev = _EDGE_CACHE.get(key)
     if ev is None:
@@ -1202,6 +1325,7 @@
         ctx.save_for_backward(w_hh0, w_ih1, w_hh1, lens, y0, g0, c0, y1, g1, c1)
         ctx.mode, ctx.rowmap, ctx.gx_private, ctx.nchunks = mode, rowmap, bool(gx_private), nchunks
         ctx.chunk_maps, ctx.w_img, ctx.gx_dtype = (edges, rms), w_img, gx0.dtype
+        ctx.wb = roles_wimg_bwd_pair((w_hh0, w_hh1), mode) if (_PAIR_CHUNKS_BWD != 0 and (ctx.needs_input_grad[0] or ctx.needs_input_grad[1])) else None
         return y1
 
     @staticmethod
@@ -1233,7 +1357,8 @@
         dgx0 = None if img_only else torch.empty(T, B, H4, **f)
         sb1 = (torch.zeros(B, H4, **f), torch.zeros(B, H, **f))
         sb0 = (torch.zeros(B, H4, **f), torch.zeros(B, H, **f))
-        wb0, wb1 = roles_wimg(w_hh0, mode, True), roles_wimg(w_hh1, mode, True)
+        wb0, wb1 = ctx.wb if ctx.wb is not None else (roles_wimg(w_hh0, mode, True), roles_wimg(w_hh1, mode, True))
+        ctx.wb = None
         for j in range(n + 1):
             c = n - 1 - j
             roles = []
@@ -1335,7 +1460,8 @@
     dy0 = torch.empty(T, B, H, **f)
     st = torch.empty(2, B * (H4 + H), **f)
     sb1, sb0 = (st[0, :B * H4], st[0, B * H4:]), (st[1, :B * H4], st[1, B * H4:])
-    wb0, wb1 = roles_wimg(w_hh0, mode, True), roles_wimg(w_hh1, mode, True)
+    wb0, wb1 = ctx.wb if ctx.wb is not None else (roles_wimg(w_hh0, mode, True), roles_wimg(w_hh1, mode, True))
+    ctx.wb = None
     for j in range(n + 1):
         c = n - 1 - j
         roles = []
@@ -1714,29 +1840,45 @@
         return dQ, dV, dtext, dwk, dv.reshape(1, -1), dw1, db1, dw2, db2, None, None, None
 
 
+_AFFINE_LOGS = _os.environ.get("FLOWTRON_AFFINE_LOGS", "1") != "0"
+
+
 class AffineFn(torch.autograd.Function):
     @staticmethod
-    def forward(ctx, out, x):
+    def forward(ctx, out, x, with_log_s=False, rev_lens=None):
         out, x = _c(out), _c(x)
-        L.require_cuda(out, x)
+        L.require_cuda(out, x, rev_lens)
         M = x.shape[-1]
         rows = x.numel() // M
         z = torch.empty_like(x)
-        L.check(L.lib().ft_affine_fwd(L.ptr(out), L.ptr(x), L.ptr(z), rows, M, L.stream()), "ft_affine_fwd")
-        ctx.save_for_backward(out, x)
-        return z
-
-    @staticmethod
-    def backward(ctx, dz):
-        out, x = ctx.saved_tensors
-        dz = _c(dz)
+        if rev_lens is not None:
+            T, B = x.shape[0], x.shape[1]
+            assert x.dim() == 3 and rev_lens.dtype == torch.int32 and rev_lens.numel() == B and rev_lens.is_contiguous()
+            L.check(L.lib().ft_affine_fwd_rev(L.ptr(out), L.ptr(x), L.ptr(z), L.ptr(rev_lens), T, B, M, L.stream()), "ft_affine_fwd_rev")
+        else:
+            L.check(L.lib().ft_affine_fwd(L.ptr(out), L.ptr(x), L.ptr(z), rows, M, L.stream()), "ft_affine_fwd")
+        ctx.save_for_backward(out, x, rev_lens)
+        return (z, out[..., :M]) if with_log_s else z
+
+    @staticmethod
+    def backward(ctx, dz, dls=None):
+        out, x, rev_lens = ctx.saved_tensors
         M = x.shape[-1]
         rows = x.numel() // M
+        dz = _c(dz) if dz is not None else torch.zeros_like(x)
+        dls = _c(dls) if dls is not None else None
         dout = torch.empty_like(out)
         dx = torch.empty_like(x)
-        L.check(L.lib().ft_affine_bwd(L.ptr(out), L.ptr(x), L.ptr(dz), None, L.ptr(dout), L.ptr(dx), rows, M, L.stream()),
-                "ft_affine_bwd")
-        return dout, dx
+        if rev_lens is not None:
+            L.check(L.lib().ft_affine_bwd_rev(L.ptr(out), L.ptr(x), L.ptr(dz), L.ptr(dls), L.ptr(dout), L.ptr(dx), L.ptr(rev_lens),
+                                              x.shape[0], x.shape[1], M, L.stream()), "ft_affine_bwd_rev")
+        else:
+            L.check(L.lib().ft_affine_bwd(L.ptr(out), L.ptr(x), L.ptr(dz), L.ptr(dls), L.ptr(dout), L.ptr(dx), rows, M, L.stream()),
+                    "ft_affine_bwd")
+        return dout, dx, None, None
+
+
+_AFFINE_REVERSE = _os.environ.get("FLOWTRON_AFFINE_REVERSE", "1") != "0"
 
 
 class ReverseByLengthFn(torch.autograd.Function):
diff --git a/include/flowtron_hip.h b/include/flowtron_hip.h
--- a/include/flowtron_hip.h
+++ b/include/flowtron_hip.h
@@ -68,10 +68,19 @@
 typedef struct { const float* src; int64_t ld; int64_t rows; int64_t cols; void* dst; int kind; } ft_img_desc;
 int ft_bf16_image_table(const ft_img_desc* descs, int n, void* stream);
 int ft_bf16_image_table_f16(const ft_img_desc* descs, int n, void* stream);
+int ft_bilstm_wimg_prepare(const float* w_hh, void* wimg, int H, int backward, void* stream);
+int ft_bilstm_wimg_prepare_f16(const float* w_hh, void* wimg, int H, int backward, void* stream);
 int ft_rowmap_build(const int32_t* lens, int32_t* rowmap, int32_t* rows_dev, int T, int B, void* stream);
 int ft_chunk_gather_rows(const int32_t* lens, int32_t* a_rows, int32_t* rowmap, int T, int B, int t0, int t1, void* stream);
+typedef struct { int32_t kind, t0, t1; } ft_step_map_job;
+int64_t ft_step_maps_plan(int T, int B, const ft_step_map_job* jobs, int n_jobs, int64_t* offsets);
+int ft_step_maps(const int32_t* lens, int32_t* out, int64_t out_ints, int T, int B, const ft_step_map_job* jobs, int n_jobs, void* stream);
 int ft_bf16_image_rows(const float* src, int64_t ld, int64_t cap_rows, int64_t cols, void* dst, float* colsum,
                        const int32_t* rowmap, const int32_t* rows_dev, void* stream);
+int ft_bf16_image_rows_shift(const float* src, int64_t ld, int64_t cap_rows, int64_t cols, void* dst,
+                             const int32_t* rowmap, const int32_t* rows_dev, int row_shift, void* stream);
+int ft_bf16_image_rows_shift_f16(const float* src, int64_t ld, int64_t cap_rows, int64_t cols, void* dst,
+                                 const int32_t* rowmap, const int32_t* rows_dev, int row_shift, void* stream);
 int ft_bf16_image_rows_act_bwd(const float* dy, int64_t ld, const float* y, int64_t ldy, int act, int64_t cap_rows, int64_t cols,
                                void* dst, float* colsum, const int32_t* rowmap, const int32_t* rows_dev, void* stream);
 int ft_bf16_image_rows_act_bwd_f16(const float* dy, int64_t ld, const float* y, int64_t ldy, int act, int64_t cap_rows, int64_t cols,
@@ -89,6 +98,7 @@
 int ft_img_gemv_rows_bwd_f16(const void* img, int64_t ld, int K, const float* dy, int64_t lddy, float* dw, float* db,
                              const int32_t* rowmap, const int32_t* rows_dev, int64_t cap_rows, void* stream);
 int ft_pad_rows_fill(float* y, int64_t ld, int cols, const int32_t* lens, int T, int B, int mode, void* stream);
+int ft_pad_rows_fill_tail(float* y, int64_t ld, int cols, const int32_t* lens, int T, int B, void* stream);
 
 int ft_embedding_fwd(const int64_t* ids, const float* W, float* out, int n, int dim, int64_t ld_out, void* stream);
 int ft_embedding_bwd(const int64_t* ids, const float* dout, float* dW, int n, int dim, int64_t ld_dout, void* stream);
@@ -184,6 +194,9 @@
 int ft_affine_fwd(const float* out, const float* x, float* z, int64_t n_rows, int M, void* stream);
 int ft_affine_bwd(const float* out, const float* x, const float* dz, const float* dlog_s_ext,
                   float* dout, float* dx, int64_t n_rows, int M, void* stream);
+int ft_affine_fwd_rev(const float* out, const float* x, float* z, const int32_t* lens, int T, int B, int M, void* stream);
+int ft_affine_bwd_rev(const float* out, const float* x, const float* dz, const float* dlog_s_ext, float* dout, float* dx,
+                      const int32_t* lens, int T, int B, int M, void* stream);
 int ft_affine_inv(const float* out, const float* z, float* x, int64_t n_rows, int M, void* stream);
 
 int ft_masked_sum(const float* x, int64_t ld, const int32_t* lens, float* acc, int square,
```

Measured after the change: 709,700 mel-frames/s, median of 6. About the same (+0.6%).
